# evanwang1990/FMwR

Hardware: AMD Instinct MI355X
Metric: training examples/sec, 10Mx1M sparse FM SGD (higher is better)
Workload: dtype f32

## Files before the change

### fmwr_amd/_lib.py

```python
import ctypes as C
import os

_PKG = os.path.dirname(os.path.abspath(__file__))
LIB_PATH = os.environ.get("FMX_LIB_PATH") or os.path.join(_PKG, "libfmx.so")

OK, ERR_INVALID, ERR_HIP, ERR_NOGPU, ERR_STATE = 0, 1, 2, 3, 4
TASK_CLASSIFICATION, TASK_REGRESSION, TASK_RANKING = 10, 20, 30
SOLVER_MCMC, SOLVER_ALS, SOLVER_SGD, SOLVER_FTRL, SOLVER_TDAP = 100, 200, 300, 500, 600
MODE_SEQUENTIAL, MODE_MINIBATCH = 0, 1
LINK_NONE, LINK_LOGISTIC, LINK_CLAMP, LINK_PROBIT = 0, 1, 2, 3
DIV_REL_SCORE, DIV_REL_MINMAX = 0, 1
SIM_COSINE, SIM_DOT = 0, 1
REDUCE_MEAN, REDUCE_SUM = 0, 1
COLUMNS_UNIFORM, COLUMNS_ZIPF = 1, 2
EVAL_LL, EVAL_AUC, EVAL_ACC, EVAL_RMSE, EVAL_MSE, EVAL_MAE = 0, 111, 222, 333, 444, 555
EVAL_PAIR_ACC, EVAL_BPR = 666, 777
KERNEL_ROWS_FORWARD, KERNEL_COLS_UPDATE, KERNEL_SCALAR, KERNEL_SEQ, KERNEL_ALS_SWEEP = 0, 1, 2, 3, 4

SYMBOLS = [
    "fmx_last_error", "fmx_device_count", "fmx_config_default", "fmx_engine_create", "fmx_engine_destroy", "fmx_set_params",
    "fmx_get_params", "fmx_engine_save", "fmx_engine_load", "fmx_matrix_from_rlist", "fmx_matrix_from_dgc", "fmx_matrix_from_csr", "fmx_matrix_synthetic", "fmx_matrix_synthetic_fields", "fmx_matrix_synthetic_iid", "fmx_matrix_synthetic_ragged", "fmx_matrix_synthetic_values", "fmx_train_stream", "fmx_matrix_set_labels", "fmx_matrix_set_fields", "fmx_matrix_destroy",
    "fmx_matrix_info", "fmx_matrix_export", "fmx_matrix_scales", "fmx_matrix_normalize", "fmx_predict", "fmx_train", "fmx_train_grid", "fmx_train_order", "fmx_num_batches",
    "fmx_step", "fmx_grad", "fmx_grad_buffer", "fmx_grad_elem_bytes", "fmx_grad_layout", "fmx_grad_begin", "fmx_grad_chunk", "fmx_apply_chunk", "fmx_apply", "fmx_sync", "fmx_stream", "fmx_predict_device",
    "fmx_als_plan_info", "fmx_als_tiled_info", "fmx_als_order_info", "fmx_als_carry_q", "fmx_als_vsweep", "fmx_mcmc_vsweep", "fmx_als_train", "fmx_mcmc_train", "fmx_mcmc_train_from", "fmx_mcmc_v_hyper", "fmx_evaluate", "fmx_train_tracked", "fmx_trace_size", "fmx_trace_get", "fmx_trace_params",
    "fmx_profile_enable", "fmx_profile_get", "fmx_profile_reset", "fmx_rows_tune_info", "fmx_matrix_rows_form", "fmx_measure_gather", "fmx_measure_gather_occ", "fmx_measure_gather_matrix", "fmx_rccl_selftest",
    "fmx_get_rows", "fmx_set_rows", "fmx_init_normal", "fmx_compact_info", "fmx_compact_count", "fmx_compact_reserve", "fmx_grad_compact", "fmx_compact_records", "fmx_apply_compact",
    "fmx_vsweep_device", "fmx_group_info", "fmx_source_open", "fmx_source_next", "fmx_source_close",
    "fmx_apply_compact_parts", "fmx_layout_info", "fmx_owner_configure", "fmx_owner_info", "fmx_rows_pack", "fmx_rows_unpack",
    "fmx_topk", "fmx_topk_device", "fmx_contrib", "fmx_contrib_device", "fmx_contrib_summary",
    "fmx_matrix_pairs", "fmx_matrix_pairs_hard",
    "fmx_heldout_rank", "fmx_heldout_rank_device", "fmx_heldout_metrics",
    "fmx_rank_lists", "fmx_rank_lists_device", "fmx_topk_lists", "fmx_topk_lists_device", "fmx_project", "fmx_project_device",
    "fmx_fold_in", "fmx_fold_in_pairs",
    "fmx_diversify", "fmx_diversify_device",
    "fmx_neighbors", "fmx_neighbors_device",
    "fmx_interactions", "fmx_interactions_device", "fmx_interactions_summary",
    "fmx_metrics", "fmx_metrics_device",
    "fmx_predict_calibrated", "fmx_predict_calibrated_device", "fmx_reliability", "fmx_reliability_device",
    "fmx_calibrate_platt", "fmx_calibrate_platt_device", "fmx_calibrate_isotonic", "fmx_calibrate_isotonic_device",
    "fmx_matrix_take", "fmx_matrix_take_device", "fmx_split_assign", "fmx_split_assign_device", "fmx_matrix_select", "fmx_matrix_select_device",
    "fmx_free_device", "fmx_matrix_split_entries", "fmx_row_permutation", "fmx_row_permutation_device",
]
SPLIT_ROWS, SPLIT_WITHIN_GROUPS, SPLIT_GROUPS = 0, 1, 2
SPLIT_ORDER_HASH, SPLIT_ORDER_TAIL = 0, 1
SPLIT_NO_PART = 0xFFFFFFFF
MET_VALUES, MET_COUNTS = 6, 4
MET_AUC, MET_LOGLOSS, MET_ACCURACY, MET_BRIER, MET_MEAN_PRED, MET_MEAN_LABEL = 0, 1, 2, 3, 4, 5
MET_MSE, MET_RMSE, MET_MAE, MET_MEAN_ERR = 0, 1, 2, 3
MET_ROWS, MET_POSITIVES, MET_PAIRS2, MET_CORRECT = 0, 1, 2, 3
CAL_NONE, CAL_PLATT, CAL_STEPS = 0, 1, 2
BINS_WIDTH, BINS_MASS = 0, 1
CAL_VALUES = 4
CAL_ECE, CAL_MCE, CAL_BRIER, CAL_LOGLOSS = 0, 1, 2, 3


TEST_HOOKS = ["fmx_debug_fail_next_plan_build", "fmx_debug_fail_next_comm_init", "fmx_debug_lose_next_seq_multiplier", "fmx_debug_stall_next_persistent_sweep",
              "fmx_debug_contrib_summary_chunk", "fmx_debug_foldin_slab", "fmx_debug_heldout_limits", "fmx_debug_pairs_hard_chunk", "fmx_debug_lists_limits", "fmx_debug_diversify_limits", "fmx_debug_neighbors_limits", "fmx_debug_interactions_limits", "fmx_debug_metrics_limits", "fmx_debug_take_limits", "fmx_debug_calibrate_limits", "fmx_debug_cols_launches",
              "fmx_debug_long_launches", "fmx_debug_rows_launches", "fmx_debug_rows_merged_launches",
              "fmx_debug_rows_sched_launches", "fmx_debug_rows_sched_id_limit", "fmx_debug_rows_sched_export"]


class Config(C.Structure):
    _fields_ = [
        ("struct_size", C.c_uint32), ("task", C.c_int32), ("solver", C.c_int32), ("num_factor", C.c_int32),
        ("keep_w0", C.c_int32), ("keep_w1", C.c_int32),
        ("l2_w0", C.c_double), ("l1_w1", C.c_double), ("l2_w1", C.c_double), ("l1_v", C.c_double), ("l2_v", C.c_double),
        ("learn_rate", C.c_double),
        ("alpha_w", C.c_double), ("alpha_v", C.c_double), ("beta_w", C.c_double), ("beta_v", C.c_double),
        ("random_step", C.c_int32), ("mode", C.c_int32), ("batch_rows", C.c_int64),
        ("min_target", C.c_double), ("max_target", C.c_double),
        ("device", C.c_int32), ("batch_reduce", C.c_int32), ("gamma", C.c_double), ("tile_rows", C.c_int64),
        ("state_fp64", C.c_int32), ("exchange_chunks", C.c_int32), ("n_gpus", C.c_int32), ("als_max_levels", C.c_int32), ("seq_reassociate", C.c_int32), ("gpus_share_device", C.c_int32),
    ]


class FieldsSpec(C.Structure):
    _fields_ = [("struct_size", C.c_uint32), ("n_dense", C.c_int32), ("n_fields", C.c_int32), ("reserved", C.c_int32),
                ("field_vocab", C.c_void_p), ("skew", C.c_double), ("seed", C.c_uint64)]


class TrackConfig(C.Structure):
    _fields_ = [("struct_size", C.c_uint32), ("metric", C.c_int32), ("step_size", C.c_int64), ("convergence", C.c_double),
                ("keep_params", C.c_int32), ("reserved", C.c_int32)]


class SplitSpec(C.Structure):
    _fields_ = [("struct_size", C.c_uint32), ("scope", C.c_int32), ("order", C.c_int32), ("n_folds", C.c_int32), ("hold_count", C.c_int64),
                ("hold_fraction", C.c_double), ("min_keep", C.c_int64), ("seed", C.c_uint64), ("salt", C.c_uint64)]


class Calibrator(C.Structure):
    _fields_ = [("struct_size", C.c_uint32), ("kind", C.c_int32), ("n_groups", C.c_int64), ("max_steps", C.c_int32), ("link", C.c_int32),
                ("platt", C.c_void_p), ("n_steps", C.c_void_p), ("thr", C.c_void_p), ("val", C.c_void_p)]


class FmxError(RuntimeError):
    def __init__(self, status, message):
        super().__init__(message)
        self.status = status


_lib = None


def lib():
    global _lib
    if _lib is None:
        if not os.path.exists(LIB_PATH):
            raise ImportError(f"{LIB_PATH} is missing: build the HIP library first (python -m fmwr_amd.build). "
                              "fmwr_amd has no CPU fallback.")
        L = C.CDLL(LIB_PATH)
        L.fmx_last_error.restype = C.c_char_p
        for name in SYMBOLS + TEST_HOOKS:
            if name != "fmx_last_error":
                getattr(L, name).restype = C.c_int
        L.fmx_matrix_pairs_hard.argtypes = [C.c_void_p, C.c_void_p, C.c_void_p, C.c_void_p, C.c_int32, C.c_int32, C.c_uint64, C.c_int64,
                                            C.POINTER(C.c_void_p)]
        L.fmx_fold_in.argtypes = [C.c_void_p, C.c_void_p, C.c_void_p, C.c_int64, C.c_double, C.c_double, C.c_int32, C.c_int32, C.c_void_p, C.c_void_p,
                                  C.c_void_p, C.c_void_p]
        L.fmx_fold_in_pairs.argtypes = L.fmx_fold_in.argtypes
        L.fmx_diversify.argtypes = [C.c_void_p, C.c_void_p, C.c_int64, C.c_int32, C.c_void_p, C.c_void_p, C.c_int32, C.c_double, C.c_int32, C.c_void_p,
                                    C.c_void_p, C.c_void_p]
        L.fmx_diversify_device.argtypes = L.fmx_diversify.argtypes
        L.fmx_neighbors.argtypes = [C.c_void_p, C.c_void_p, C.c_void_p, C.c_int32, C.c_int32, C.c_int32, C.c_void_p, C.c_void_p]
        L.fmx_neighbors_device.argtypes = [C.c_void_p, C.c_void_p, C.c_int64, C.c_int64, C.c_void_p, C.c_int32, C.c_int32, C.c_int32, C.c_void_p, C.c_void_p]
        L.fmx_debug_neighbors_limits.argtypes = [C.c_int64, C.c_int64]
        L.fmx_interactions.argtypes = [C.c_void_p, C.c_void_p, C.c_int32, C.c_void_p, C.c_void_p, C.c_void_p]
        L.fmx_interactions_device.argtypes = [C.c_void_p, C.c_void_p, C.c_int64, C.c_int64, C.c_int32, C.c_void_p, C.c_void_p, C.c_void_p]
        L.fmx_interactions_summary.argtypes = [C.c_void_p, C.c_void_p, C.c_void_p, C.c_int32, C.c_void_p, C.c_void_p, C.c_void_p]
        L.fmx_debug_interactions_limits.argtypes = [C.c_int32, C.c_int32, C.c_int64]
        L.fmx_metrics.argtypes = [C.c_void_p, C.c_void_p, C.c_void_p, C.c_int64, C.c_int, C.c_void_p, C.c_void_p]
        L.fmx_metrics_device.argtypes = [C.c_void_p, C.c_void_p, C.c_int64, C.c_int64, C.c_void_p, C.c_int64, C.c_int, C.c_void_p, C.c_void_p]
        L.fmx_debug_metrics_limits.argtypes = [C.c_int32, C.c_int32, C.c_int64]
        L.fmx_predict_calibrated.argtypes = [C.c_void_p, C.c_void_p, C.c_void_p, C.c_int64, C.POINTER(Calibrator), C.c_int, C.c_void_p]
        L.fmx_predict_calibrated_device.argtypes = [C.c_void_p, C.c_void_p, C.c_int64, C.c_int64, C.c_void_p, C.c_int64, C.POINTER(Calibrator), C.c_int, C.c_void_p]
        L.fmx_reliability.argtypes = [C.c_void_p, C.c_void_p, C.c_void_p, C.c_int64, C.c_int32, C.c_int32, C.POINTER(Calibrator), C.c_int] + [C.c_void_p] * 6
        L.fmx_reliability_device.argtypes = [C.c_void_p, C.c_void_p, C.c_int64, C.c_int64, C.c_void_p, C.c_int64, C.c_int32, C.c_int32, C.POINTER(Calibrator),
                                             C.c_int] + [C.c_void_p] * 6
        L.fmx_calibrate_platt.argtypes = [C.c_void_p, C.c_void_p, C.c_void_p, C.c_int64, C.c_double, C.c_int32, C.c_void_p, C.c_void_p, C.c_void_p]
        L.fmx_calibrate_platt_device.argtypes = [C.c_void_p, C.c_void_p, C.c_int64, C.c_int64, C.c_void_p, C.c_int64, C.c_double, C.c_int32, C.c_void_p, C.c_void_p,
                                                 C.c_void_p]
        L.fmx_calibrate_isotonic.argtypes = [C.c_void_p, C.c_void_p, C.c_void_p, C.c_int64, C.c_int32, C.c_void_p, C.c_void_p, C.c_void_p]
        L.fmx_calibrate_isotonic_device.argtypes = [C.c_void_p, C.c_void_p, C.c_int64, C.c_int64, C.c_void_p, C.c_int64, C.c_int32, C.c_void_p, C.c_void_p, C.c_void_p]
        L.fmx_debug_calibrate_limits.argtypes = [C.c_int64]
        L.fmx_matrix_take.argtypes = [C.c_void_p, C.c_void_p, C.c_int64, C.POINTER(C.c_void_p)]
        L.fmx_matrix_take_device.argtypes = L.fmx_matrix_take.argtypes
        L.fmx_split_assign.argtypes = [C.c_int, C.c_int64, C.c_void_p, C.c_int64, C.POINTER(SplitSpec), C.c_void_p]
        L.fmx_split_assign_device.argtypes = L.fmx_split_assign.argtypes
        L.fmx_matrix_select.argtypes = [C.c_void_p, C.c_void_p, C.c_uint32, C.c_int32, C.POINTER(C.c_void_p), C.c_void_p]
        L.fmx_matrix_select_device.argtypes = [C.c_void_p, C.c_void_p, C.c_uint32, C.c_int32, C.POINTER(C.c_void_p), C.POINTER(C.c_void_p)]
        L.fmx_free_device.argtypes = [C.c_void_p]
        L.fmx_matrix_split_entries.argtypes = [C.c_void_p, C.c_int32, C.c_int64, C.c_double, C.c_int64, C.c_uint64, C.c_uint64, C.POINTER(C.c_void_p),
                                               C.POINTER(C.c_void_p)]
        L.fmx_row_permutation.argtypes = [C.c_int, C.c_int64, C.c_uint64, C.c_uint64, C.c_void_p]
        L.fmx_row_permutation_device.argtypes = L.fmx_row_permutation.argtypes
        L.fmx_debug_take_limits.argtypes = [C.c_int32, C.c_int32, C.c_int64]
        _lib = L
    return _lib


def check(status):
    if status != OK:
        raise FmxError(status, lib().fmx_last_error().decode("utf-8", "replace"))


def default_config():
    cfg = Config()
    check(lib().fmx_config_default(C.byref(cfg)))
    return cfg
```

### fmwr_amd/csrc/fm_batch_kernels.hip

```cpp
#include <atomic>
#include <mutex>
#include <utility>
#include <vector>

#include "fmx_internal.h"
#include "fm_probit.h"
#include "fmx_test_hooks.h"

#ifndef FMX_U
#define FMX_U 4
#endif
#ifndef FMX_SPARSE_WAVES
#define FMX_SPARSE_WAVES 4
#endif
#ifndef FMX_DENSE_WAVES
#define FMX_DENSE_WAVES 4
#endif
#ifndef FMX_U_LARGE
#define FMX_U_LARGE 4
#endif
#ifndef FMX_U_SMALL
#define FMX_U_SMALL 8
#endif

// ... 331 lines not shown
  constexpr int PER = MERGE_STAGE / WG_THREADS;
  constexpr uint32_t DONE = 0xFFFFFFFFu;
  __shared__ uint32_t stage[MERGE_STAGE];
  __shared__ double red[TRAIN ? MERGE_RPW : 1];

  const int tid = threadIdx.x;
  const int gid = tid / LPR;
  const int lig = tid % LPR;
  const int64_t R0 = (int64_t)blockIdx.x * MERGE_RPW;
  const int64_t R1 = (R0 + MERGE_RPW < a.nrows) ? R0 + MERGE_RPW : a.nrows;
  const int64_t lo = a.row_ptr[a.r0 + R0];
  const int64_t hi = a.row_ptr[a.r0 + R1];
  const int cnt = (hi - lo < MERGE_STAGE) ? (int)(hi - lo) : MERGE_STAGE;
  uint32_t pe[MERGE_SLOTS];
#pragma unroll
  for (int s = 0; s < MERGE_SLOTS; ++s) {
    const int64_t row = R0 + s * NG + gid;
    const int64_t ra = row < a.nrows ? row : a.nrows, rb = row + 1 < a.nrows ? row + 1 : a.nrows;
    const int64_t ta = a.row_ptr[a.r0 + ra] - lo, tb = a.row_ptr[a.r0 + rb] - lo;
    pe[s] = (uint32_t)(ta < cnt ? ta : cnt) | ((uint32_t)(tb < cnt ? tb : cnt) << 16);
  }
  {
    uint32_t id[PER];
#pragma unroll
    for (int u = 0; u < PER; ++u) {
      const int i = tid + u * WG_THREADS;
      id[u] = i < cnt ? a.col[lo + i] : 0u;
    }
#pragma unroll
    for (int u = 0; u < PER; ++u) {
      const int i = tid + u * WG_THREADS;
      if (i < cnt) stage[i] = id[u];
    }
  }
  __syncthreads();

  const T* __restrict__ Vt = reinterpret_cast<const T*>(a.V) + lig * VEC;
  const T* __restrict__ wt = a.w ? reinterpret_cast<const T*>(a.w) : reinterpret_cast<const T*>(a.V);
  const bool k1 = h.k1 != 0;
  const int last = cnt > 0 ? cnt - 1 : 0;
  static_assert(MERGE_STAGE < (1 << 16), "positions are kept in 16 bits");
  uint32_t hd[MERGE_SLOTS];
  int left = 0;
#pragma unroll
  for (int s = 0; s < MERGE_SLOTS; ++s) {
    const int p0 = (int)(pe[s] & 0xFFFFu), p1 = (int)(pe[s] >> 16);
    const uint32_t v = stage[p0 < last ? p0 : last];
    hd[s] = p0 < p1 ? v : DONE;
    left += p1 - p0;
  }
  double sm[MERGE_SLOTS][VEC], qm[MERGE_SLOTS][VEC], lin[MERGE_SLOTS];
#pragma unroll
  for (int s = 0; s < MERGE_SLOTS; ++s) {
#pragma unroll
    for (int i = 0; i < VEC; ++i) { sm[s][i] = 0.0; qm[s][i] = 0.0; }
    lin[s] = h.k0 ? a.scal[SC_W0] : 0.0;
  }

  uint32_t safe = 0u;
  for (; left > 0; left -= U) {
    uint32_t eid[U];
    int esl[U];
#pragma unroll
    for (int u = 0; u < U; ++u) {
      uint32_t best = hd[0];
      int sel = 0;
#pragma unroll
      for (int s = 1; s < MERGE_SLOTS; ++s)
        if (hd[s] < best) { best = hd[s]; sel = s; }
      const bool live = best != DONE;
      eid[u] = live ? best : safe;
      esl[u] = live ? sel : MERGE_SLOTS;
      safe = eid[u];
      uint32_t nxt = 0u;
#pragma unroll
      for (int s = 0; s < MERGE_SLOTS; ++s)
        if (esl[u] == s) { pe[s] += 1u; nxt = pe[s]; }
      const int np = (int)(nxt & 0xFFFFu), ne = (int)(nxt >> 16);
      const uint32_t nx = stage[np < last ? np : last];
      const uint32_t nh = np < ne ? nx : DONE;
#pragma unroll
      for (int s = 0; s < MERGE_SLOTS; ++s)
        if (esl[u] == s) hd[s] = nh;
    }
    float4 vv[U];
    T wv[U];
#pragma unroll
    for (int u = 0; u < U; ++u) {
      vv[u] = gather_row(Vt + ((size_t)eid[u] << RowStride<T, LPR>::v(a.vsh)));
      wv[u] = wt[(size_t)eid[u] << RowStride<T, LPR>::w(a.wsh)];
    }
#pragma unroll
    for (int u = 0; u < U; ++u) {
      const double x = 1.0;
      const double wx = (double)wv[u] * x;
      double tmp[VEC], tsq[VEC];
      slice_get(vv[u], tmp);
#pragma unroll
      for (int i = 0; i < VEC; ++i) { tmp[i] = tmp[i] * x; tsq[i] = tmp[i] * tmp[i]; }
#pragma unroll
      for (int s = 0; s < MERGE_SLOTS; ++s) {
        if (esl[u] == s) {
          if (k1) lin[s] += wx;
#pragma unroll
          for (int i = 0; i < VEC; ++i) {
            sm[s][i] += tmp[i];
            if constexpr (U == 1) qm[s][i] += tsq[i]; else qm[s][i] += tmp[i] * tmp[i];
          }
        }
      }
    }
  }

  int eg = tid / LPR;
  asm volatile("" : "+v"(eg));
#pragma unroll
  for (int s = 0; s < MERGE_SLOTS; ++s) {
    const int64_t row = R0 + s * NG + eg;
    const bool have = row < a.nrows;
    double pair = 0.0;
#pragma unroll
    for (int i = 0; i < VEC; ++i) pair += 0.5 * (sm[s][i] * sm[s][i] - qm[s][i]);
#pragma unroll
    for (int off = LPR / 2; off > 0; off >>= 1) pair += __shfl_xor(pair, off);
    const double y_hat = lin[s] + pair;
    if constexpr (TRAIN) {
      double mult = 0.0;
      if (have) {
        mult = grad_mult(h, y_hat, a.y[a.r0 + row]);
        float4 srow = slice_make(sm[s], T());
        srow = embed_store<LPR>(srow, lig, (float)mult, a.embed);
        *reinterpret_cast<float4*>(reinterpret_cast<T*>(a.S) + (size_t)row * KP + lig * VEC) = srow;
        if (lig == 0) reinterpret_cast<T*>(a.amul)[row] = (T)mult;
      }
      if (lig == 0) red[s * NG + eg] = mult;
    } else {
      if (have && lig == 0 && a.yhat) a.yhat[row] = link_apply(h, y_hat, a.link, a.pn_y);
    }
  }
  if constexpr (TRAIN) {
    __syncthreads();
    if (tid % 64 == 0) {
      const int s = tid / 64;
      if (R0 + (int64_t)s * NG < a.nrows) {
        double g0 = 0.0, q0 = 0.0;
        for (int i = 0; i < NG; ++i) { const double m = red[s * NG + i]; g0 += m; q0 += m * m; }
        a.partials[2 * ((size_t)blockIdx.x * MERGE_SLOTS + s)] = g0;
        a.partials[2 * ((size_t)blockIdx.x * MERGE_SLOTS + s) + 1] = q0;
      }
    }
  }
}

template <bool UNIFORM, bool PIPE, bool DEAL = false>
__global__ __launch_bounds__(WG_THREADS, 4) void fm_rows_sched_k(RowsArgs a, Hyper h) {
  using T = float;
  constexpr int LPR = 4, VEC = 4, KP = LPR * VEC;
  constexpr int NG = WG_THREADS / LPR;
  constexpr int PER = MERGE_STAGE / WG_THREADS;
  static_assert(MERGE_STAGE == SCHED_STAGE_STEPS * NG && MERGE_SLOTS == 4, "the stage holds SCHED_STAGE_STEPS steps of one word per lane group");
  static_assert(UNIFORM || !PIPE, "only the unrolled walk has a round to request together");
  static_assert(!(UNIFORM && DEAL), "a DEAL schedule is walked as a MERGE one");
  __shared__ uint32_t stage[MERGE_STAGE];
  __shared__ double red[MERGE_RPW];
  __shared__ uint32_t places[DEAL ? NG : 1];

  const int tid = threadIdx.x;
  const int gid = tid / LPR;
  const int lig = tid % LPR;
  const int64_t R0 = (int64_t)blockIdx.x * MERGE_RPW;
  const uint32_t w_hi = a.sched_dir[blockIdx.x + 1];
  uint32_t w_lo = a.sched_dir[blockIdx.x];
  if constexpr (DEAL) {
    const bool hdr = w_hi - w_lo >= (uint32_t)NG;
    if (tid < NG) places[tid] = hdr ? a.sched[(size_t)w_lo + tid] : 0u;
    w_lo += hdr ? (uint32_t)NG : 0u;
  }
  const int cnt = (w_hi - w_lo < (uint32_t)MERGE_STAGE) ? (int)(w_hi - w_lo) : MERGE_STAGE;
  const int steps = UNIFORM ? (cnt / NG) & ~3 : cnt / NG;
  {
    uint32_t id[PER];
#pragma unroll
    for (int u = 0; u < PER; ++u) {
      const int i = tid + u * WG_THREADS;
      id[u] = i < cnt ? a.sched[(size_t)w_lo + i] : SCHED_BUBBLE;
    }
#pragma unroll
    for (int u = 0; u < PER; ++u) {
      const int i = tid + u * WG_THREADS;
      if (i < cnt) stage[i] = id[u];
    }
  }
  __syncthreads();

  const __amdgpu_buffer_rsrc_t v_rsrc = table_rsrc(a.V, a.sched_vbytes);
  const __amdgpu_buffer_rsrc_t w_rsrc = table_rsrc(a.w ? a.w : a.V, a.w ? a.sched_wbytes : a.sched_vbytes);
  const bool k1 = h.k1 != 0;
  const int vsh = RowStride<T, LPR>::v(a.vsh) + 2, wsh = RowStride<T, LPR>::w(a.wsh) + 2;
  const uint32_t lane_off = (uint32_t)(lig * VEC * sizeof(T));
  double sm[MERGE_SLOTS][VEC], qm[MERGE_SLOTS][VEC], lin[MERGE_SLOTS];
#pragma unroll
  for (int s = 0; s < MERGE_SLOTS; ++s) {
#pragma unroll
    for (int i = 0; i < VEC; ++i) { sm[s][i] = 0.0; qm[s][i] = 0.0; }
    lin[s] = h.k0 ? a.scal[SC_W0] : 0.0;
  }
  const uint32_t* __restrict__ mine = stage + gid;

  if constexpr (UNIFORM) {
    for (int t = 0; t < steps; t += MERGE_SLOTS) {
      uint32_t wd[MERGE_SLOTS];
#pragma unroll
      for (int j = 0; j < MERGE_SLOTS; ++j) wd[j] = mine[(t + j) * NG];
      float4 vv[MERGE_SLOTS];
      T wv[MERGE_SLOTS];
      if constexpr (PIPE) {
#pragma unroll
        for (int j = 0; j < MERGE_SLOTS; ++j) {
          const bool live = wd[j] != SCHED_BUBBLE;
          const uint32_t c = wd[j] & SCHED_MAX_P;
          vv[j] = buf_row(v_rsrc, live ? (c << vsh) + lane_off : BUF_SKIP, T());
          wv[j] = buf_elem(w_rsrc, live ? c << wsh : BUF_SKIP, T());
        }
      }
#pragma unroll
      for (int j = 0; j < MERGE_SLOTS; ++j) {
        if constexpr (!PIPE) {
          const bool live = wd[j] != SCHED_BUBBLE;
          const uint32_t c = wd[j] & SCHED_MAX_P;
          vv[j] = buf_row(v_rsrc, live ? (c << vsh) + lane_off : BUF_SKIP, T());
          wv[j] = buf_elem(w_rsrc, live ? c << wsh : BUF_SKIP, T());
          asm volatile("s_waitcnt vmcnt(0)" ::: "memory");
        }
        const double x = 1.0;
        const double wx = (double)wv[j] * x;
        double tmp[VEC], tsq[VEC];
        slice_get(vv[j], tmp);
#pragma unroll
        for (int i = 0; i < VEC; ++i) { tmp[i] = tmp[i] * x; tsq[i] = tmp[i] * tmp[i]; }
        if (k1) lin[j] += wx;
#pragma unroll
        for (int i = 0; i < VEC; ++i) { sm[j][i] += tmp[i]; qm[j][i] += tsq[i]; }
      }
    }
  } else {
    for (int t = 0; t < steps; ++t) {
      const uint32_t wd = mine[t * NG];
      const bool live = wd != SCHED_BUBBLE;
      const uint32_t c = wd & SCHED_MAX_P;
      const int esl = live ? (int)(wd >> 30) : MERGE_SLOTS;
      const float4 vv = buf_row(v_rsrc, live ? (c << vsh) + lane_off : BUF_SKIP, T());
      const T wv = buf_elem(w_rsrc, live ? c << wsh : BUF_SKIP, T());
      const double x = 1.0;
      const double wx = (double)wv * x;
      double tmp[VEC], tsq[VEC];
      slice_get(vv, tmp);
#pragma unroll
      for (int i = 0; i < VEC; ++i) { tmp[i] = tmp[i] * x; tsq[i] = tmp[i] * tmp[i]; }
#pragma unroll
      for (int s = 0; s < MERGE_SLOTS; ++s) {
        if (esl == s) {
          if (k1) lin[s] += wx;
#pragma unroll
          for (int i = 0; i < VEC; ++i) { sm[s][i] += tmp[i]; qm[s][i] += tsq[i]; }
        }
      }
    }
  }

  int eg = tid / LPR;
  asm volatile("" : "+v"(eg));
  uint32_t place = 0;
  if constexpr (DEAL) place = places[eg];
#pragma unroll
  for (int s = 0; s < MERGE_SLOTS; ++s) {
    const int at = DEAL ? (int)((place >> (8 * s)) & 255u) : s * NG + eg;
    const int64_t row = R0 + at;
    const bool have = row < a.nrows;
    double pair = 0.0;
#pragma unroll
    for (int i = 0; i < VEC; ++i) pair += 0.5 * (sm[s][i] * sm[s][i] - qm[s][i]);
#pragma unroll
    for (int off = LPR / 2; off > 0; off >>= 1) pair += __shfl_xor(pair, off);
    const double y_hat = lin[s] + pair;
    double mult = 0.0;
    if (have) {
      mult = grad_mult(h, y_hat, a.y[a.r0 + row]);
      float4 srow = slice_make(sm[s], T());
      srow = embed_store<LPR>(srow, lig, (float)mult, a.embed);
      *reinterpret_cast<float4*>(reinterpret_cast<T*>(a.S) + (size_t)row * KP + lig * VEC) = srow;
      if (lig == 0) reinterpret_cast<T*>(a.amul)[row] = (T)mult;
    }
    if (lig == 0) red[at] = mult;
  }
  __syncthreads();
  if (tid % 64 == 0) {
    const int s = tid / 64;
    if (R0 + (int64_t)s * NG < a.nrows) {
      double g0 = 0.0, q0 = 0.0;
      for (int i = 0; i < NG; ++i) { const double m = red[s * NG + i]; g0 += m; q0 += m * m; }
      a.partials[2 * ((size_t)blockIdx.x * MERGE_SLOTS + s)] = g0;
      a.partials[2 * ((size_t)blockIdx.x * MERGE_SLOTS + s) + 1] = q0;
    }
  }
}

template <typename T, int LPR, bool TRAIN>
__global__ __launch_bounds__(WG_THREADS) void fm_rows_forward_dyn_k(RowsArgs a, Hyper h) {
  using vec_t = typename Slice<T>::vec;
  constexpr int VEC = Slice<T>::N;
  constexpr int KP = LPR * VEC;
  constexpr int GROUPS = WG_THREADS / LPR;
  constexpr int RPW = 4 * GROUPS;
  constexpr int RU = FMX_U_LARGE;
  constexpr int PER = (RU + LPR - 1) / LPR;
  __shared__ int next_row;
  __shared__ double red[TRAIN ? RPW : 1];
  const int tid = threadIdx.x;
  const int grp = tid / LPR, lig = tid % LPR;
  const int lane0 = (tid & 63) - lig;
  const int64_t R0 = (int64_t)blockIdx.x * RPW;
  const int rows_here = (int)((R0 + RPW < a.nrows ? R0 + RPW : a.nrows) - R0);
  if (tid == 0) next_row = GROUPS;
  if (TRAIN) for (int i = tid; i < RPW; i += WG_THREADS) red[i] = 0.0;
  __syncthreads();
  const T* __restrict__ Vt = reinterpret_cast<const T*>(a.V) + lig * VEC;
  const T* __restrict__ wt = a.w ? reinterpret_cast<const T*>(a.w) : reinterpret_cast<const T*>(a.V);
  const bool k1 = h.k1 != 0;
  const int64_t last = a.row_ptr[a.r0 + R0 + rows_here] - 1;
  int r = grp;
  while (r < rows_here) {
    const int64_t ta = a.row_ptr[a.r0 + R0 + r], tb = a.row_ptr[a.r0 + R0 + r + 1];
    double s[VEC], q[VEC];
#pragma unroll
    for (int i = 0; i < VEC; ++i) { s[i] = 0.0; q[i] = 0.0; }
    double lin = h.k0 ? a.scal[SC_W0] : 0.0;
    auto load_round = [&](int64_t t, uint32_t* id, uint32_t* xb) {
#pragma unroll
      for (int v = 0; v < PER; ++v) {
        const int64_t at = t + lig + v * LPR;
        const int64_t ac = at <= last ? (at >= 0 ? at : 0) : (last >= 0 ? last : 0);
        id[v] = a.col[ac];
        xb[v] = a.unit ? 0x3f800000u : __float_as_uint(a.val[ac]);
      }
    };
    uint32_t cid[PER], cxb[PER], nid[PER], nxb[PER];
    load_round(ta, cid, cxb);
    for (int64_t t = ta; t < tb; t += RU) {
      load_round(t + RU, nid, nxb);
      uint2 en[RU];
#pragma unroll
      for (int u = 0; u < RU; ++u) {
        en[u].x = (uint32_t)__shfl((int)cid[u / LPR], lane0 + (u % LPR));
        en[u].y = (uint32_t)__shfl((int)cxb[u / LPR], lane0 + (u % LPR));
      }
#pragma unroll
      for (int u = 1; u < RU; ++u)
        if (t + u >= tb) en[u] = make_uint2(en[0].x, 0u);
      vec_t vv[RU];
      T wv[RU];
#pragma unroll
      for (int u = 0; u < RU; ++u) {
        vv[u] = gather_row(Vt + ((size_t)en[u].x << RowStride<T, LPR>::v(a.vsh)));
        wv[u] = wt[(size_t)en[u].x << RowStride<T, LPR>::w(a.wsh)];
        if (a.serial) asm volatile("s_waitcnt vmcnt(0)" ::: "memory");
      }
#pragma unroll
      for (int u = 0; u < RU; ++u) {
        const double x = (double)__uint_as_float(en[u].y);
        if (k1) lin += (double)wv[u] * x;
        double vf[VEC];
        slice_get(vv[u], vf);
#pragma unroll
        for (int i = 0; i < VEC; ++i) {
          const double tmp = vf[i] * x;
          s[i] += tmp;
          q[i] += tmp * tmp;
        }
      }
#pragma unroll
      for (int v = 0; v < PER; ++v) { cid[v] = nid[v]; cxb[v] = nxb[v]; }
    }
    double pair = 0.0;
#pragma unroll
    for (int i = 0; i < VEC; ++i) pair += 0.5 * (s[i] * s[i] - q[i]);
#pragma unroll
    for (int off = LPR / 2; off > 0; off >>= 1) pair += __shfl_xor(pair, off);
    const double y_hat = lin + pair;
    const int64_t row = R0 + r;
    if constexpr (TRAIN) {
      const double mult = grad_mult(h, y_hat, a.y[a.r0 + row]);
      vec_t srow = slice_make(s, T());
      if constexpr (sizeof(T) == 4) srow = embed_store<LPR>(srow, lig, (float)mult, a.embed);
      *reinterpret_cast<vec_t*>(reinterpret_cast<T*>(a.S) + (size_t)row * KP + lig * VEC) = srow;
      if (lig == 0) { reinterpret_cast<T*>(a.amul)[row] = (T)mult; red[r] = mult; }
    } else {
      if (lig == 0 && a.yhat) a.yhat[row] = link_apply(h, y_hat, a.link, a.pn_y);
      if constexpr (sizeof(T) == 8) {
        if (a.qout) {
          if (a.qout_t > 0) { a.qout[(size_t)(lig * VEC) * a.qout_t + row] = s[0]; a.qout[(size_t)(lig * VEC + 1) * a.qout_t + row] = s[1]; }
          else *reinterpret_cast<double2*>(a.qout + (size_t)row * KP + lig * VEC) = make_double2(s[0], s[1]);
        }
      } else if (a.qout) {
        double2* q2 = reinterpret_cast<double2*>(a.qout + (size_t)row * KP + lig * VEC);
        q2[0] = make_double2(s[0], s[1]);
        q2[1] = make_double2(s[2], s[3]);
      }
    }
    int nr = 0;
    if (lig == 0) nr = atomicAdd(&next_row, 1);
    r = __shfl(nr, lane0);
  }
  if constexpr (TRAIN) {
    __syncthreads();
    if (tid < RPW / GROUPS && tid * GROUPS < rows_here) {
      double g0 = 0.0, q0 = 0.0;
      for (int i = tid * GROUPS; i < (tid + 1) * GROUPS; ++i) { g0 += red[i]; q0 += red[i] * red[i]; }
      const size_t at = (size_t)blockIdx.x * (RPW / GROUPS) + tid;
// ... 254 lines not shown
    if (a.wg_threads == 64 && 64 / lpr >= 2) { count_rows_launch(counted, ROWS_NARROW1); return launch_rows_t<T, TRAIN, 64, 1, true>(e, a, kp); }
    count_rows_launch(counted, wide_form);
    return launch_rows_t<T, TRAIN, WG_THREADS, 1, true>(e, a, kp);
  }
  if (a.sort_rows && a.wg_threads != 64) { count_rows_launch(counted, ROWS_PULL); return launch_rows_dyn<T, TRAIN>(e, a, kp); }
  if (a.flat == 1 && a.wg_threads != 64) { count_rows_launch(counted, ROWS_FLAT); return launch_rows_flat<T, TRAIN>(e, a, kp); }
  if (a.wg_threads == 64) {
    count_rows_launch(counted, a.split == 4 ? ROWS_NARROW4 : ROWS_NARROW1);
    return a.split == 4 ? launch_rows_t<T, TRAIN, 64, 4>(e, a, kp) : launch_rows_t<T, TRAIN, 64, 1>(e, a, kp);
  }
  count_rows_launch(counted, wide_form);
  return launch_rows_t<T, TRAIN, WG_THREADS, 1>(e, a, kp);
}

static std::atomic<int64_t> g_rows_merged[2];
void debug_rows_merged_launches(int64_t out[2]) {
  for (int i = 0; i < 2; ++i) out[i] = g_rows_merged[i].load();
}
#ifndef FMX_ROWS_MERGE_U_DEFAULT
#define FMX_ROWS_MERGE_U_DEFAULT 1
#endif
static int rows_merge_mode() { static const int v = [] { const char* s = getenv("FMX_ROWS_MERGE"); return s ? atoi(s) : 1; }(); return v; }
static int rows_merge_u() {
  static const int v = [] { const char* s = getenv("FMX_ROWS_MERGE_U"); const int u = s ? atoi(s) : FMX_ROWS_MERGE_U_DEFAULT; return (u == 1 || u == 2) ? u : FMX_ROWS_MERGE_U_DEFAULT; }();
  return v;
}

template <bool TRAIN, int U>
static int64_t rows_merged_fill(const fmx_engine* e) {
  constexpr int MAX_DEV = 64;
  static std::atomic<int64_t> fill_dev[MAX_DEV];
  std::atomic<int64_t>& fill = fill_dev[(e->cfg.device >= 0 && e->cfg.device < MAX_DEV) ? e->cfg.device : 0];
  int64_t v = fill.load();
  if (v == 0) {
    hipDeviceProp_t pr{};
    const int cus = (hipGetDeviceProperties(&pr, e->cfg.device) == hipSuccess && pr.multiProcessorCount > 0) ? pr.multiProcessorCount : 256;
    int per = 0;
    if (hipOccupancyMaxActiveBlocksPerMultiprocessor(&per, fm_rows_merged_k<float, 4, TRAIN, U>, WG_THREADS, 0) != hipSuccess || per <= 0) per = 4;
    v = (int64_t)per * cus * MERGE_RPW;
    fill.store(v);
  }
  return v;
}

__global__ __launch_bounds__(WG_THREADS) void rows_block_max_k(const int64_t* __restrict__ row_ptr, int64_t r0, int64_t nrows, int64_t* __restrict__ out) {
  __shared__ int64_t part[WG_THREADS];
  const int64_t blocks = (nrows + MERGE_RPW - 1) / MERGE_RPW;
  int64_t m = 0;
  for (int64_t b = threadIdx.x; b < blocks; b += WG_THREADS) {
    const int64_t r1 = (b + 1) * MERGE_RPW < nrows ? (b + 1) * MERGE_RPW : nrows;
    const int64_t c = row_ptr[r0 + r1] - row_ptr[r0 + b * MERGE_RPW];
    m = c > m ? c : m;
  }
  part[threadIdx.x] = m;
  __syncthreads();
  if (threadIdx.x == 0) {
    for (int i = 1; i < WG_THREADS; ++i) m = part[i] > m ? part[i] : m;
    out[0] = m;
  }
}

static int rows_merged_fits(fmx_engine* e, const RowsArgs& a, bool* fits) {
  if ((int64_t)a.max_row_len * MERGE_RPW <= MERGE_STAGE) { *fits = true; return FMX_OK; }
  struct Key { uint64_t uid; int64_t r0, nrows; };
  static std::mutex mu;
  static std::vector<std::pair<Key, bool>> known;
  {
    std::lock_guard<std::mutex> g(mu);
    for (const auto& k : known)
      if (k.first.uid == a.mat_uid && k.first.r0 == a.r0 && k.first.nrows == a.nrows) { *fits = k.second; return FMX_OK; }
  }
  int64_t* d = nullptr;
  int64_t most = 0;
  FMX_HIP(hipMalloc(&d, sizeof(int64_t)));
  hipLaunchKernelGGL(rows_block_max_k, dim3(1), dim3(WG_THREADS), 0, e->stream, a.row_ptr, a.r0, a.nrows, d);
  hipError_t err = hipGetLastError();
  if (err == hipSuccess) err = hipMemcpyAsync(&most, d, sizeof(int64_t), hipMemcpyDeviceToHost, e->stream);
  if (err == hipSuccess) err = hipStreamSynchronize(e->stream);
  (void)hipFree(d);
  FMX_HIP(err);
  *fits = most <= MERGE_STAGE;
  std::lock_guard<std::mutex> g(mu);
  if (known.size() >= 4096) known.clear();
  known.push_back({Key{a.mat_uid, a.r0, a.nrows}, *fits});
  return FMX_OK;
}

template <bool TRAIN, int U>
static int launch_rows_merged_u(fmx_engine* e, const RowsArgs& a, int mode, bool* ran) {
  const size_t v_bytes = ((size_t)e->p << a.vsh) * sizeof(float);
  if (mode != 2 && (a.nrows < rows_merged_fill<TRAIN, U>(e) || a.col_skew != 1 || v_bytes <= MERGE_MIN_TABLE)) return FMX_OK;
  bool fits = false;
  FMX_TRY(rows_merged_fits(e, a, &fits));
  if (!fits) { g_rows_merged[1]++; return FMX_OK; }
  const int64_t grid = (a.nrows + MERGE_RPW - 1) / MERGE_RPW;
  FMX_CHECK(grid < (1LL << 31), FMX_ERR_INVALID, "rows_forward: grid too large (%lld)", (long long)grid);
  hipLaunchKernelGGL((fm_rows_merged_k<float, 4, TRAIN, U>), dim3((unsigned)grid), dim3(WG_THREADS), 0, e->stream, a, e->hyper);
  FMX_HIP(hipGetLastError());
  g_rows_merged[0]++;
  *ran = true;
  return FMX_OK;
}

template <bool TRAIN>
static int launch_rows_merged(fmx_engine* e, const RowsArgs& a, bool fp64_tables, bool* ran) {
  *ran = false;
  const int mode = rows_merge_mode();
  if (mode == 0 || fp64_tables || e->kp32 != 16 || !a.unit || a.qout || a.no_w || a.wg_threads == 64 || a.sort_rows || a.flat == 1) return FMX_OK;
  if (TRAIN && e->cfg.task == FMX_TASK_RANKING) return FMX_OK;
  if (a.nrows <= 0 || a.max_row_len <= 0 || a.mat_uid == 0) return FMX_OK;
  switch (rows_merge_u()) {
    case 2: return launch_rows_merged_u<TRAIN, 2>(e, a, mode, ran);
    default: return launch_rows_merged_u<TRAIN, 1>(e, a, mode, ran);
  }
}

#ifndef FMX_ROWS_SCHED_DEFAULT
#define FMX_ROWS_SCHED_DEFAULT 1
#endif
#ifndef FMX_ROWS_SCHED_POLICY_DEFAULT
#define FMX_ROWS_SCHED_POLICY_DEFAULT SCHED_DEAL
#endif
#ifndef FMX_ROWS_SCHED_RHO_DEFAULT
#define FMX_ROWS_SCHED_RHO_DEFAULT 1024
#endif
static std::atomic<int64_t> g_rows_sched[3];
void debug_rows_sched_launches(int64_t out[3]) {
  for (int i = 0; i < 3; ++i) out[i] = g_rows_sched[i].load();
}
void rows_sched_count_build() { g_rows_sched[2]++; }
static int rows_sched_mode() {
  static const int v = [] { const char* s = getenv("FMX_ROWS_SCHED"); return s ? atoi(s) : (getenv("FMX_ROWS_MERGE") ? 0 : FMX_ROWS_SCHED_DEFAULT); }();
  return v;
}
static int rows_sched_policy() {
  static const int v = [] {
    const char* s = getenv("FMX_ROWS_SCHED_POLICY");
    if (!s) return (int)FMX_ROWS_SCHED_POLICY_DEFAULT;
    return s[0] == 'm' ? (int)SCHED_MERGE : s[0] == 'f' ? (int)SCHED_FRONT : s[0] == 'r' ? (int)SCHED_ROUND : s[0] == 'd' ? (int)SCHED_DEAL : (int)FMX_ROWS_SCHED_POLICY_DEFAULT;
  }();
  return v;
}
static int rows_sched_rho_q() {
  static const int v = [] {
    const char* s = getenv("FMX_ROWS_SCHED_RHO");
    if (!s) return (int)FMX_ROWS_SCHED_RHO_DEFAULT;
    const double r = atof(s);
    return r <= 0.0 ? 0 : r >= 1.0 ? 1024 : (int)(r * 1024.0 + 0.5);
  }();
  return v;
}
static int rows_sched_u() { static const int v = [] { const char* s = getenv("FMX_ROWS_SCHED_U"); return (s && atoi(s) == 4) ? 4 : 1; }(); return v; }

bool rows_sched_wanted(fmx_engine* e, const RowsArgs& a, int* policy, int* rho_q) {
  const int mode = rows_sched_mode();
  if (mode == 0 || mb_wide(e) || e->kp32 != 16 || !a.unit || a.qout || a.no_w || a.wg_threads == 64 || a.sort_rows || a.flat == 1) return false;
  if (e->cfg.task == FMX_TASK_RANKING || a.nrows <= 0 || a.max_row_len <= 0 || a.mat_uid == 0 || !a.w) return false;
  const uint64_t v_bytes = (uint64_t)e->p * (uint64_t)a.vs * sizeof(float), w_bytes = (uint64_t)e->p * (uint64_t)a.ws * sizeof(float);
  if (v_bytes >= BUF_SKIP || w_bytes >= BUF_SKIP || e->p > SCHED_MAX_P) return false;
  if (mode != 2 && (a.nrows < rows_merged_fill<true, 1>(e) || a.col_skew != 1 || v_bytes <= MERGE_MIN_TABLE)) return false;
  *policy = rows_sched_policy();
  *rho_q = (*policy == SCHED_MERGE || *policy == SCHED_DEAL) ? 0 : rows_sched_rho_q();
  return true;
}

static int launch_rows_sched(fmx_engine* e, const RowsArgs& a_in, bool* ran) {
  *ran = false;
  if (a_in.sched_state == 0) return FMX_OK;
  int policy = 0, rho_q = 0;
  if (!rows_sched_wanted(e, a_in, &policy, &rho_q)) return FMX_OK;
  if (a_in.sched_state != 1 || !a_in.sched || !a_in.sched_dir) { g_rows_sched[1]++; return FMX_OK; }
  RowsArgs a = a_in;
  a.sched_vbytes = (uint32_t)((uint64_t)e->p * (uint64_t)a.vs * sizeof(float));
  a.sched_wbytes = (uint32_t)((((uint64_t)e->p - 1) * (uint64_t)a.ws + 1) * sizeof(float));
  const int64_t grid = (a.nrows + MERGE_RPW - 1) / MERGE_RPW;
  FMX_CHECK(grid < (1LL << 31), FMX_ERR_INVALID, "rows_forward: grid too large (%lld)", (long long)grid);
  if (a.sched_deal) hipLaunchKernelGGL((fm_rows_sched_k<false, false, true>), dim3((unsigned)grid), dim3(WG_THREADS), 0, e->stream, a, e->hyper);
  else if (!a.sched_uniform) hipLaunchKernelGGL((fm_rows_sched_k<false, false>), dim3((unsigned)grid), dim3(WG_THREADS), 0, e->stream, a, e->hyper);
  else if (rows_sched_u() == 4) hipLaunchKernelGGL((fm_rows_sched_k<true, true>), dim3((unsigned)grid), dim3(WG_THREADS), 0, e->stream, a, e->hyper);
  else hipLaunchKernelGGL((fm_rows_sched_k<true, false>), dim3((unsigned)grid), dim3(WG_THREADS), 0, e->stream, a, e->hyper);
  FMX_HIP(hipGetLastError());
  g_rows_sched[0]++;
  *ran = true;
  return FMX_OK;
}

int launch_rows_forward(fmx_engine* e, const RowsArgs& a_in, bool train, bool fp64_tables) {
  RowsArgs a = a_in;
  FMX_CHECK(a.vs >= (fp64_tables ? e->kp64 : e->kp32) && a.ws >= 1 && (a.vs & (a.vs - 1)) == 0 && (a.ws & (a.ws - 1)) == 0, FMX_ERR_STATE,
            "rows_forward: table strides not set (%d, %d)", a.vs, a.ws);
  {
    const int kp = fp64_tables ? e->kp64 : e->kp32;
    FMX_CHECK((!fp64_tables && kp <= WIR_MAX_KP) || (a.vs == kp && a.ws == 1), FMX_ERR_STATE, "rows_forward: strides (%d, %d) on a table of compiled strides (%d, 1)",
              a.vs, a.ws, kp);
  }
  a.vsh = __builtin_ctz((unsigned)a.vs); a.wsh = __builtin_ctz((unsigned)a.ws);
  static const bool embed_ok = [] { const char* v = getenv("FMX_EMBED_MULT"); return !(v && v[0] == '0'); }();
  static const int force = [] { const char* v = getenv("FMX_ROWS_SERIAL"); return v ? atoi(v) : -1; }();
  RowsTune& tu = e->rows_tune;
  auto pick = [&](const RowsArgs& r, int* serial, int* trial) -> int {
    *trial = -1;
    *serial = 1;
    if (force >= 0) { *serial = force; return FMX_OK; }
    const bool timed = r.wg_threads != 64 && r.nrows >= RowsTune::MIN_ROWS;
    const int64_t key = r.unit ? 1 : 0;
    if (timed && key != tu.key) {
      if (tu.events && tu.launches > 0 && tu.decided < 0) FMX_HIP(hipStreamSynchronize(e->stream));
      tu.key = key; tu.decided = -1; tu.launches = 0;
    }
    if (tu.decided >= 0) { *serial = tu.decided; return FMX_OK; }
    if (!timed) return FMX_OK;
    if (!tu.events) {
      bool ok = true;
      for (auto& ev : tu.ev) ok = ok && hipEventCreate(&ev) == hipSuccess;
      FMX_CHECK(ok, FMX_ERR_HIP, "rows_forward: could not create the tuning events");
      tu.events = true;
    }
    if (tu.launches >= RowsTune::TRIALS) {
      tu.decided = 1;
      return FMX_OK;
    }
    *trial = tu.launches++;
    *serial = *trial % 2 == 0 ? 1 : 0;
    FMX_HIP(hipEventRecord(tu.ev[2 * *trial], e->stream));
    return FMX_OK;
  };
  auto done = [&](int trial) -> int {
    if (trial < 0) return FMX_OK;
    FMX_HIP(hipEventRecord(tu.ev[2 * trial + 1], e->stream));
    if (tu.launches >= RowsTune::TRIALS && tu.decided < 0) {
      FMX_HIP(hipEventSynchronize(tu.ev[2 * trial + 1]));
      double ms[2] = {0.0, 0.0};
      for (int i = 2; i < RowsTune::TRIALS; ++i) {
        float t = 0.f;
        FMX_HIP(hipEventElapsedTime(&t, tu.ev[2 * i], tu.ev[2 * i + 1]));
        ms[i % 2 == 0 ? 1 : 0] += t;
      }
      tu.ms[0] = ms[0]; tu.ms[1] = ms[1];
      tu.decided = ms[1] <= ms[0] ? 1 : 0;
    }
    return FMX_OK;
  };
  a.embed = (train && embed_ok) ? embed_mode(e->k, fp64_tables ? e->kp64 : e->kp32, !fp64_tables) : EMBED_NONE;
  prof_begin(e, FMX_KERNEL_ROWS_FORWARD);
  int st = FMX_OK;
  bool merged = false;
  if (train) {
    st = launch_rows_sched(e, a, &merged);
    if (st == FMX_OK && !merged) st = launch_rows_merged<true>(e, a, fp64_tables, &merged);
    if (st == FMX_OK && !merged) {
      int trial;
      FMX_TRY(pick(a, &a.serial, &trial));
      st = fp64_tables ? launch_rows_w<double, true>(e, a, e->kp64) : launch_rows_w<float, true>(e, a, e->kp32);
      { const int st2 = done(trial); if (st == FMX_OK) st = st2; }
    }
  } else {
    const int64_t SLAB = 1 << 18;
    const int kp = fp64_tables ? e->kp64 : e->kp32;
    for (int64_t off = 0; off < a.nrows && st == FMX_OK; off += SLAB) {
      RowsArgs s = a;
      s.r0 = a.r0 + off;
      s.nrows = a.nrows - off < SLAB ? a.nrows - off : SLAB;
      if (a.yhat) s.yhat = a.yhat + off;
      if (a.qout) s.qout = a.qout_t > 0 ? a.qout + off : a.qout + (size_t)off * kp;
      s.wg_threads = a.fixed_schedule ? WG_THREADS : rows_wg_threads(a.nrows, kp / (fp64_tables ? 2 : 4));
      s.split = a.fixed_schedule ? 1 : rows_split(a.nrows, kp / (fp64_tables ? 2 : 4));
      st = launch_rows_merged<false>(e, s, fp64_tables, &merged);
      if (st != FMX_OK || merged) continue;
      int trial;
      FMX_TRY(pick(s, &s.serial, &trial));
      st = fp64_tables ? launch_rows_w<double, false>(e, s, kp) : launch_rows_w<float, false>(e, s, kp);
      { const int st2 = done(trial); if (st == FMX_OK) st = st2; }
    }
  }
  prof_end(e);
  return st;
}

template <typename ST>
__device__ __forceinline__ void tail_put_rows(ST* gtail, double rows) {
  const double hi = floor(rows / 4096.0);
  gtail[2] = (ST)hi;
  gtail[3] = (ST)(rows - hi * 4096.0);
}
template <typename ST>
__device__ __forceinline__ double tail_get_rows(const ST* gtail) { return (double)gtail[2] * 4096.0 + (double)gtail[3]; }

template <typename ST>
__device__ __forceinline__ void scalar_update(const double* __restrict__ partials, int64_t n_partials, const double* sin,
                                              double* sout, ST* gtail, const Hyper& h, double rows, int mode,
                                              double* sg, double* sq) {
  const int phase = (mode == SCALAR_PUBLISH) ? 1 : (mode == SCALAR_FROM_TAIL) ? 2 : 0;
  double g0 = 0.0, q0 = 0.0;
  if (phase != 2) {
    for (int64_t i = threadIdx.x; i < n_partials; i += WG_THREADS) { g0 += partials[2 * i]; q0 += partials[2 * i + 1]; }
  }
  sg[threadIdx.x] = g0; sq[threadIdx.x] = q0;
  __syncthreads();
  for (int off = WG_THREADS / 2; off > 0; off >>= 1) {
    if ((int)threadIdx.x < off) { sg[threadIdx.x] += sg[threadIdx.x + off]; sq[threadIdx.x] += sq[threadIdx.x + off]; }
    __syncthreads();
  }
  if (threadIdx.x != 0) return;
  g0 = sg[0]; q0 = sq[0];
  if (phase == 1) { gtail[0] = (ST)g0; gtail[1] = (ST)q0; tail_put_rows(gtail, rows); return; }
  if (phase == 2) { g0 = gtail[0]; q0 = gtail[1]; if (rows <= 0.0) rows = tail_get_rows(gtail); }
  for (int i = 0; i < SC_COUNT; ++i) sout[i] = sin[i];
  if (h.task == FMX_TASK_RANKING) {
    sout[SC_G0] = 0.0; sout[SC_Q0] = 0.0;
    if (h.kind == UPD_SGD_L1) {
      const double steps = (h.mean && rows > 0.0) ? 1.0 : rows;
      sout[SC_UW] = sin[SC_UW] + steps * (h.lr * h.regw);
      sout[SC_UV] = sin[SC_UV] + steps * (h.lr * h.regv);
    }
    return;
  }
  sout[SC_G0] = g0; sout[SC_Q0] = q0;
  if (h.mean && rows > 0.0) {
    g0 /= rows;
    q0 = g0 * g0;
    rows = 1.0;
  }
  const double w0 = sin[SC_W0];
  if (h.kind == UPD_TDAP) {
    double u = sin[SC_N0], nu = sin[SC_T_NU], dl = sin[SC_T_DELTA], hh = sin[SC_T_H], z0 = sin[SC_Z0];
    if (h.k0) {
      const double u_new = u + q0;
      nu += g0;
      const double sigma = (sqrt(u_new) - sqrt(u)) / h.alpha_w;
      const double age = rows == 1.0 ? h.egamma : exp(-h.gamma * rows);
      dl = age * (dl + sigma);
      hh = age * (hh + sigma * w0);
      u = u_new;
      z0 = nu - hh;
// ... 1148 lines not shown
```

### fmwr_amd/csrc/fm_group.hip

```cpp
#include <dlfcn.h>

#include <atomic>

#include <hip/hip_runtime.h>

#include "fmx_internal.h"

namespace fmx {

typedef void* rcclComm_t;
struct Rccl {
  void* lib = nullptr;
  int (*CommInitAll)(rcclComm_t*, int, const int*) = nullptr;
  int (*CommDestroy)(rcclComm_t) = nullptr;
  int (*AllReduce)(const void*, void*, size_t, int, int, rcclComm_t, hipStream_t) = nullptr;
  int (*AllGather)(const void*, void*, size_t, int, rcclComm_t, hipStream_t) = nullptr;
  int (*GroupStart)() = nullptr;
  int (*GroupEnd)() = nullptr;
  const char* (*GetErrorString)(int) = nullptr;
};
constexpr int RCCL_SUM = 0, RCCL_FLOAT32 = 7, RCCL_FLOAT64 = 8;

static Rccl* rccl() {
  static Rccl r;
  static bool tried = false;
  if (tried) return r.lib ? &r : nullptr;
  tried = true;
  for (const char* name : {"librccl.so.1", "librccl.so", "/opt/rocm/lib/librccl.so.1"}) {
    r.lib = dlopen(name, RTLD_NOW | RTLD_GLOBAL);
    if (r.lib) break;
  }
  if (!r.lib) return nullptr;
  r.CommInitAll = (decltype(r.CommInitAll))dlsym(r.lib, "ncclCommInitAll");
  r.CommDestroy = (decltype(r.CommDestroy))dlsym(r.lib, "ncclCommDestroy");
  r.AllReduce = (decltype(r.AllReduce))dlsym(r.lib, "ncclAllReduce");
  r.AllGather = (decltype(r.AllGather))dlsym(r.lib, "ncclAllGather");
  r.GroupStart = (decltype(r.GroupStart))dlsym(r.lib, "ncclGroupStart");
  r.GroupEnd = (decltype(r.GroupEnd))dlsym(r.lib, "ncclGroupEnd");
  r.GetErrorString = (decltype(r.GetErrorString))dlsym(r.lib, "ncclGetErrorString");
  if (!r.CommInitAll || !r.CommDestroy || !r.AllReduce || !r.AllGather || !r.GroupStart || !r.GroupEnd) { dlclose(r.lib); r.lib = nullptr; return nullptr; }
  return &r;
}

#define FMX_RCCL(call)                                                                                               \
  do {                                                                                                               \
    const int _r = (call);                                                                                           \
    if (_r != 0) {                                                                                                   \
      Rccl* _l = rccl();                                                                                             \
      fmx::set_error("%s failed: %s", #call, _l && _l->GetErrorString ? _l->GetErrorString(_r) : "rccl error");       \
      return FMX_ERR_HIP;                                                                                            \
    }                                                                                                                \
  } while (0)

constexpr int GROUP_MAX = 16;
struct BufList { void* b[GROUP_MAX]; int n; };

template <typename ST>
__global__ void sum_buffers_k(BufList bl, int64_t count) {
  const int64_t i = (int64_t)blockIdx.x * blockDim.x + threadIdx.x;
  if (i >= count) return;
  ST acc = reinterpret_cast<const ST*>(bl.b[0])[i];
  for (int r = 1; r < bl.n; ++r) acc = acc + reinterpret_cast<const ST*>(bl.b[r])[i];
  for (int r = 0; r < bl.n; ++r) reinterpret_cast<ST*>(bl.b[r])[i] = acc;
}

__global__ void rebase_rows_k(const int64_t* __restrict__ src, int64_t r0, int64_t n, int64_t base, int64_t* __restrict__ dst) {
  const int64_t i = (int64_t)blockIdx.x * blockDim.x + threadIdx.x;
  if (i <= n) dst[i] = src[r0 + i] - base;
}

struct Group {
  int n = 0;
  std::vector<fmx_engine*> rep;
  std::vector<int> dev;
  bool shared = false;
  std::vector<rcclComm_t> comm;
  hipStream_t xs = nullptr;
  std::vector<hipEvent_t> ready;
  hipEvent_t summed = nullptr;
  uint64_t src_uid = 0;
  uint64_t src_values = 0;
  std::vector<fmx_matrix*> shard;
  std::vector<void*> gath;
  int64_t gath_records = 0;
  bool busy = false;
  struct OwnerBuf {
    void *req = nullptr, *rows_out = nullptr, *rows_in = nullptr, *parts = nullptr;
    int64_t req_cap = 0, out_cap = 0, in_cap = 0, parts_cap = 0;
  };
  std::vector<OwnerBuf> ox;
  std::vector<hipEvent_t> ev_ids, ev_packed, ev_grad, ev_done;
  int peer_pairs = 0, peer_direct = 0;
  bool owners_on = false;
  bool owner_dirty = false;
};

bool group_outside(const fmx_engine* e) { return e->group != nullptr && !e->group->busy; }

static void free_shards(Group* g) {
  for (size_t r = 0; r < g->shard.size(); ++r)
    if (g->shard[r]) { (void)hipSetDevice(g->dev[r]); fmx_matrix_destroy(g->shard[r]); }
  g->shard.clear();
  g->src_uid = 0;
}

void group_destroy(fmx_engine* e) {
  Group* g = e->group;
  if (!g) return;
  free_shards(g);
  for (size_t r = 0; r < g->gath.size(); ++r) if (g->gath[r]) { (void)hipSetDevice(g->dev[r]); (void)hipFree(g->gath[r]); }
  for (size_t r = 0; r < g->ox.size(); ++r) {
    (void)hipSetDevice(g->dev[r]);
    (void)hipFree(g->ox[r].req); (void)hipFree(g->ox[r].rows_out); (void)hipFree(g->ox[r].rows_in); (void)hipFree(g->ox[r].parts);
  }
  for (auto* v : {&g->ev_ids, &g->ev_packed, &g->ev_grad, &g->ev_done})
    for (size_t r = 0; r < v->size(); ++r) if ((*v)[r]) { (void)hipSetDevice(g->dev[r]); (void)hipEventDestroy((*v)[r]); }
  Rccl* l = rccl();
  for (rcclComm_t c : g->comm) if (c && l) (void)l->CommDestroy(c);
  (void)hipSetDevice(e->cfg.device);
  for (hipEvent_t ev : g->ready) if (ev) (void)hipEventDestroy(ev);
  if (g->summed) (void)hipEventDestroy(g->summed);
  if (g->xs) (void)hipStreamDestroy(g->xs);
  for (int r = 1; r < g->n; ++r) fmx_engine_destroy(g->rep[(size_t)r]);
  delete g;
  e->group = nullptr;
}

static std::atomic<int> g_fail_next_comm_init{0};
void debug_fail_next_comm_init() { g_fail_next_comm_init.store(1); }

int group_create(fmx_engine* e) {
  const int n = e->cfg.n_gpus;
  FMX_CHECK(n >= 2 && n <= GROUP_MAX, FMX_ERR_INVALID, "n_gpus must be in 1..%d", GROUP_MAX);
  FMX_CHECK(e->cfg.mode == FMX_MODE_MINIBATCH, FMX_ERR_INVALID,
            "n_gpus > 1 needs FMX_MODE_MINIBATCH: the reference's per-example algorithm does not shard (every example depends on the one before)");
  FMX_CHECK(e->cfg.solver == FMX_SOLVER_SGD || e->cfg.solver == FMX_SOLVER_FTRL || e->cfg.solver == FMX_SOLVER_TDAP, FMX_ERR_INVALID,
            "n_gpus > 1 trains SGD / FTRL / TDAP engines (the ALS / MCMC sweeps run as replicas only)");
  Group* g = new Group();
  e->group = g;
  g->n = n;
  g->shared = e->cfg.gpus_share_device != 0;
  g->rep.assign((size_t)n, nullptr);
  g->rep[0] = e;
  int count = 0;
  FMX_HIP(hipGetDeviceCount(&count));
  for (int r = 0; r < n; ++r) g->dev.push_back(g->shared ? e->cfg.device : e->cfg.device + r);
  FMX_CHECK(g->dev.back() < count, FMX_ERR_INVALID, "n_gpus = %d starting at device %d, but only %d devices are visible", n, e->cfg.device, count);
  for (int r = 1; r < n; ++r) {
    fmx_config c = e->cfg;
    c.n_gpus = 1;
    c.device = g->dev[(size_t)r];
    FMX_TRY(fmx_engine_create(&c, e->p, &g->rep[(size_t)r]));
  }
  g->ready.assign((size_t)n, nullptr);
  if (g_fail_next_comm_init.exchange(0) > 0) {
    set_error("ncclCommInitAll failed on device %d (forced: fmx_debug_fail_next_comm_init)", g->dev[(size_t)n - 1]);
    return FMX_ERR_HIP;
  }
  if (g->shared) {
    FMX_HIP(hipSetDevice(e->cfg.device));
    FMX_HIP(hipStreamCreateWithFlags(&g->xs, hipStreamNonBlocking));
    FMX_HIP(hipEventCreateWithFlags(&g->summed, hipEventDisableTiming));
    for (int r = 0; r < n; ++r) FMX_HIP(hipEventCreateWithFlags(&g->ready[(size_t)r], hipEventDisableTiming));
  } else {
    Rccl* l = rccl();
    FMX_CHECK(l != nullptr, FMX_ERR_STATE, "n_gpus > 1 on distinct devices needs librccl.so (not found by dlopen)");
    g->comm.assign((size_t)n, nullptr);
    FMX_RCCL(l->CommInitAll(g->comm.data(), n, g->dev.data()));
    for (int a = 0; a < n; ++a) {
      FMX_HIP(hipSetDevice(g->dev[(size_t)a]));
      for (int b = 0; b < n; ++b) {
        if (a == b) continue;
        ++g->peer_pairs;
        int can = 0;
        if (hipDeviceCanAccessPeer(&can, g->dev[(size_t)a], g->dev[(size_t)b]) != hipSuccess) { (void)hipGetLastError(); can = 0; }
        if (!can) continue;
        const hipError_t pe = hipDeviceEnablePeerAccess(g->dev[(size_t)b], 0);
        if (pe == hipSuccess || pe == hipErrorPeerAccessAlreadyEnabled) ++g->peer_direct;
        (void)hipGetLastError();
      }
    }
  }
  FMX_HIP(hipSetDevice(e->cfg.device));
  return FMX_OK;
}

int group_load(fmx_engine* e, const char* path) {
  Group* g = e->group;
  for (int r = 1; r < g->n; ++r) FMX_TRY(fmx_engine_load(g->rep[(size_t)r], path));
  g->owner_dirty = false;
  return use_device(e->cfg.device);
}

int group_set_params(fmx_engine* e, double w0, const double* w, const double* v) {
  (void)w; (void)v;
  Group* g = e->group;
  std::vector<std::pair<void*, size_t>> src;
  engine_tables(e, &src, true);
  FMX_HIP(hipSetDevice(e->cfg.device));
  FMX_HIP(hipStreamSynchronize(e->stream));
  for (int r = 1; r < g->n; ++r) {
    FMX_TRY(fmx_set_params(g->rep[(size_t)r], w0, nullptr, nullptr));
    std::vector<std::pair<void*, size_t>> dst;
    engine_tables(g->rep[(size_t)r], &dst, true);
    FMX_CHECK(dst.size() == src.size(), FMX_ERR_STATE, "replica %d has another table layout", r);
    for (size_t t = 0; t < src.size(); ++t) {
      FMX_CHECK(dst[t].second == src[t].second, FMX_ERR_STATE, "replica %d has another table layout", r);
      const size_t bytes = src[t].second * (size_t)e->p;
      if (g->dev[(size_t)r] == g->dev[0]) FMX_HIP(hipMemcpy(dst[t].first, src[t].first, bytes, hipMemcpyDeviceToDevice));
      else FMX_HIP(hipMemcpyPeer(dst[t].first, g->dev[(size_t)r], src[t].first, g->dev[0], bytes));
    }
  }
  FMX_HIP(hipDeviceSynchronize());
  g->owner_dirty = false;
  return use_device(e->cfg.device);
}

int group_init_normal(fmx_engine* e, uint64_t seed, double mean, double stdev) {
  Group* g = e->group;
  for (int r = 1; r < g->n; ++r) FMX_TRY(fmx_init_normal(g->rep[(size_t)r], seed, mean, stdev));
  return use_device(e->cfg.device);
}

int group_set_rows(fmx_engine* e, const uint32_t* ids, int64_t n, const double* w, const double* v) {
  Group* g = e->group;
  for (int r = 1; r < g->n; ++r) FMX_TRY(fmx_set_rows(g->rep[(size_t)r], ids, n, w, v));
  return use_device(e->cfg.device);
}

static int cut_shard(const fmx_matrix* src, int64_t r0, int64_t r1, int dev, fmx_matrix** out) {
  FMX_HIP(hipSetDevice(src->device));
  int64_t ends[2] = {0, 0};
  FMX_HIP(hipMemcpy(&ends[0], src->row_ptr + r0, sizeof(int64_t), hipMemcpyDeviceToHost));
  FMX_HIP(hipMemcpy(&ends[1], src->row_ptr + r1, sizeof(int64_t), hipMemcpyDeviceToHost));
  const int64_t base = ends[0], cnt = ends[1] - ends[0], n = r1 - r0;
  fmx_matrix* m = nullptr;
  FMX_TRY(alloc_matrix(dev, n, src->p, cnt, src->has_labels != 0, &m));
  auto body = [&]() -> int {
    FMX_HIP(hipSetDevice(dev));
    if (dev == src->device) {
      hipLaunchKernelGGL(rebase_rows_k, dim3((unsigned)((n + 1 + 255) / 256)), dim3(256), 0, nullptr, src->row_ptr, r0, n, base, m->row_ptr);
    } else {
      FMX_HIP(hipMemcpyPeer(m->row_ptr, dev, src->row_ptr + r0, src->device, ((size_t)n + 1) * sizeof(int64_t)));
      hipLaunchKernelGGL(rebase_rows_k, dim3((unsigned)((n + 1 + 255) / 256)), dim3(256), 0, nullptr, m->row_ptr, (int64_t)0, n, base, m->row_ptr);
    }
    if (cnt > 0) {
      FMX_HIP(hipMemcpyPeer(m->col, dev, src->col + base, src->device, (size_t)cnt * sizeof(uint32_t)));
      FMX_HIP(hipMemcpyPeer(m->val, dev, src->val + base, src->device, (size_t)cnt * sizeof(float)));
    }
    if (n > 0) FMX_HIP(hipMemcpyPeer(m->y, dev, src->y + r0, src->device, (size_t)n * sizeof(float)));
// ... 615 lines not shown
```

### fmwr_amd/csrc/fmx_api.hip

```cpp
#include <algorithm>
#include <cmath>
#include <cstdlib>
#include <cstring>
#include <ctime>
#include <atomic>
#include <memory>

#include "fmx_internal.h"
#include "fmx_test_hooks.h"
#include "fm_probit.h"

namespace fmx {

static thread_local std::string g_error;

void set_error(const char* fmt, ...) {
  char buf[1024];
  va_list ap;
  va_start(ap, fmt);
  vsnprintf(buf, sizeof(buf), fmt, ap);
  va_end(ap);
  g_error = buf;
}

void prof_begin(fmx_engine* e, int kernel) {
  e->prof_open = 0;
  if (!e->profile) return;
  if ((e->prof_seen[kernel]++ % e->profile) != 0) return;
  hipEvent_t a, b;
  if (hipEventCreate(&a) != hipSuccess || hipEventCreate(&b) != hipSuccess) return;
  (void)hipEventRecord(a, e->stream);
  e->prof_pending.push_back({kernel, {a, b}});
  e->prof_open = 1;
}

void prof_end(fmx_engine* e) {
  if (!e->prof_open || e->prof_pending.empty()) return;
  e->prof_open = 0;
  (void)hipEventRecord(e->prof_pending.back().second.second, e->stream);
}

static int prof_collect(fmx_engine* e) {
  if (e->prof_pending.empty()) return FMX_OK;
  FMX_HIP(hipStreamSynchronize(e->stream));
  for (auto& pr : e->prof_pending) {
    float ms = 0.f;
    if (hipEventElapsedTime(&ms, pr.second.first, pr.second.second) == hipSuccess) {
      e->prof_ms[pr.first] += ms;
      e->prof_n[pr.first] += 1;
    }
    (void)hipEventDestroy(pr.second.first);
    (void)hipEventDestroy(pr.second.second);
  }
  e->prof_pending.clear();
  return FMX_OK;
}

int use_device(int device) {
  int count = 0;
  hipError_t err = hipGetDeviceCount(&count);
  if (err != hipSuccess || count <= 0) {
    set_error("no HIP device available (%s); libfmx has no CPU fallback", err == hipSuccess ? "device count 0" : hipGetErrorString(err));
    return FMX_ERR_NOGPU;
  }
  FMX_CHECK(device >= 0 && device < count, FMX_ERR_INVALID, "device %d out of range (0..%d)", device, count - 1);
  FMX_HIP(hipSetDevice(device));
  return FMX_OK;
}

int seq_abort_check(fmx_engine* e) {
  if (!e->cfg.seq_reassociate && !getenv("FMX_SEQ_REASSOC")) return FMX_OK;
  double flag = 0.0;
  FMX_HIP(hipMemcpy(&flag, e->scal + SC_SEQ_ABORT, sizeof(double), hipMemcpyDeviceToHost));
  FMX_CHECK(flag == 0.0, FMX_ERR_HIP, "the reassociated sequential learner gave up waiting inside a launch (its workgroup's waves did not all run?): the parameters are not a valid state");
  return FMX_OK;
}

template <typename T>
static int dev_alloc_zero(T** ptr, size_t count) {
  const size_t bytes = (count ? count : 1) * sizeof(T);
  FMX_HIP(hipMalloc(ptr, bytes));
  FMX_HIP(hipMemset(*ptr, 0, bytes));
  return FMX_OK;
}

static int make_hyper(const fmx_config& c, Hyper* h) {
  h->task = c.task;
  h->k0 = c.keep_w0 != 0;
  h->k1 = c.keep_w1 != 0;
  h->lr = c.learn_rate;
  h->reg0 = c.l2_w0;
  h->l1w = c.l1_w1; h->l1v = c.l1_v; h->l2w = c.l2_w1; h->l2v = c.l2_v;
  h->alpha_w = c.alpha_w; h->alpha_v = c.alpha_v; h->beta_w = c.beta_w; h->beta_v = c.beta_v;
  h->min_t = c.min_target; h->max_t = c.max_target;
  h->mean = (c.batch_reduce == FMX_REDUCE_MEAN);
  h->egamma = std::exp(-c.gamma);
  h->gamma = c.gamma;
  if (c.solver == FMX_SOLVER_FTRL || c.solver == FMX_SOLVER_TDAP) {
    h->kind = c.solver == FMX_SOLVER_FTRL ? UPD_FTRL : UPD_TDAP;
    h->regw = 0; h->regv = 0;
  } else {
    bool l1 = false;
    if (c.l1_w1 > 0 || c.l1_v > 0) {
      l1 = true;
      h->regw = c.l1_w1; h->regv = c.l1_v;
    } else {
      h->regw = c.l2_w1; h->regv = c.l2_v;
    }
    if (c.task == FMX_TASK_REGRESSION) l1 = false;
    h->kind = l1 ? UPD_SGD_L1 : UPD_SGD_L2;
  }
  h->decay_w = 1.0 - h->lr * h->regw;
  h->decay_v = 1.0 - h->lr * h->regv;
  h->log_decay_w = h->decay_w > 0 ? std::log(h->decay_w) : 0.0;
  h->log_decay_v = h->decay_v > 0 ? std::log(h->decay_v) : 0.0;
  return FMX_OK;
}

static bool seq_mode(const fmx_engine* e) { return e->cfg.mode == FMX_MODE_SEQUENTIAL; }
static bool ranking(const fmx_engine* e) { return e->cfg.task == FMX_TASK_RANKING; }

static int check_pairs(const fmx_engine* e, const fmx_matrix* m, int64_t rows, const char* what) {
  if (!ranking(e)) return FMX_OK;
  FMX_CHECK(m->n % 2 == 0, FMX_ERR_INVALID, "a ranking engine trains on pair matrices (rows 2t, 2t + 1): this matrix has an odd row count (%lld)", (long long)m->n);
  FMX_CHECK(rows % 2 == 0, FMX_ERR_INVALID, "a ranking engine needs an even %s (got %lld): a step may not split a pair", what, (long long)rows);
  return FMX_OK;
}

static int reset_optimizer_state(fmx_engine* e) {
  const size_t p = e->p;
  double zeros[SC_COUNT] = {0};
  double w0 = 0;
  FMX_HIP(hipMemcpy(&w0, e->scal + SC_W0, sizeof(double), hipMemcpyDeviceToHost));
  zeros[SC_W0] = w0;
  FMX_HIP(hipMemcpy(e->scal, zeros, sizeof(zeros), hipMemcpyHostToDevice));
  if (e->sV) FMX_HIP(hipMemset(e->sV, 0, p * e->kp32 * sizeof(float)));
  if (e->sw) FMX_HIP(hipMemset(e->sw, 0, p * sizeof(float)));
  if (e->nV) FMX_HIP(hipMemset(e->nV, 0, p * e->kp32 * sizeof(float)));
  if (e->nw) FMX_HIP(hipMemset(e->nw, 0, p * sizeof(float)));
  for (float* t : {e->t1V, e->t2V, e->t3V}) if (t) FMX_HIP(hipMemset(t, 0, p * e->kp32 * sizeof(float)));
  for (float* t : {e->t1w, e->t2w, e->t3w}) if (t) FMX_HIP(hipMemset(t, 0, p * sizeof(float)));
  if (e->dsV) FMX_HIP(hipMemset(e->dsV, 0, p * e->kp64 * sizeof(double)));
  if (e->dsw) FMX_HIP(hipMemset(e->dsw, 0, p * sizeof(double)));
  if (e->dnV) FMX_HIP(hipMemset(e->dnV, 0, p * e->kp64 * sizeof(double)));
  if (e->dnw) FMX_HIP(hipMemset(e->dnw, 0, p * sizeof(double)));
  for (double* t : {e->dt1V, e->dt2V, e->dt3V}) if (t) FMX_HIP(hipMemset(t, 0, p * e->kp64 * sizeof(double)));
  for (double* t : {e->dt1w, e->dt2w, e->dt3w}) if (t) FMX_HIP(hipMemset(t, 0, p * sizeof(double)));
  return FMX_OK;
}

static int ensure_workspace(fmx_engine* e, int64_t s_rows, int64_t step_rows, int64_t tiles_per_step) {
  const int rpw = WG_THREADS / mb_lpr(e);
  const int64_t partials = (step_rows + rpw - 1) / rpw + (tiles_per_step > 0 ? tiles_per_step : 1) + 8 + 4096;
  if (s_rows <= e->ws_rows && partials <= e->ws_partials) return FMX_OK;
  FMX_HIP(hipStreamSynchronize(e->stream));
  (void)hipFree(e->S); (void)hipFree(e->amul); (void)hipFree(e->partials);
  e->S = nullptr; e->amul = nullptr; e->partials = nullptr; e->ws_rows = 0; e->ws_partials = 0;
  FMX_HIP(hipMalloc(&e->S, (size_t)s_rows * mb_kp(e) * mb_elem(e)));
  FMX_HIP(hipMalloc(&e->amul, (size_t)s_rows * mb_elem(e)));
  FMX_HIP(hipMalloc(&e->partials, (size_t)partials * 2 * sizeof(double)));
  e->ws_rows = s_rows;
  e->ws_partials = partials;
  return FMX_OK;
}

static int ensure_gbuf(fmx_engine* e) {
  if (e->gbuf) return FMX_OK;
  const bool has_q = exchange_has_q(e);
  const int64_t chunks = e->cfg.exchange_chunks > 1 ? e->cfg.exchange_chunks : 1;
  const int64_t per = ((int64_t)e->p + chunks - 1) / chunks;
  e->gb_feats = chunks > 1 ? (per + 63) / 64 * 64 : ((int64_t)e->p + 3) / 4 * 4;
  e->gb_blocks = ((int64_t)e->p + e->gb_feats - 1) / e->gb_feats;
  e->gb_block_elems = e->gb_feats * mb_kp(e) * (has_q ? 2 : 1) + e->gb_feats * (has_q ? 3 : 2);
  e->gbuf_floats = e->gb_blocks * e->gb_block_elems + 4;
  FMX_HIP(hipMalloc(&e->gbuf, (size_t)e->gbuf_floats * mb_elem(e)));
  FMX_HIP(hipMemset(e->gbuf, 0, (size_t)e->gbuf_floats * mb_elem(e)));
  FMX_HIP(hipDeviceSynchronize());
  return FMX_OK;
}

static uint32_t random_select(int n) {
  if (n == 1) return 1;
  return (uint32_t)((rand() / ((double)RAND_MAX + 1)) * n + 1);
}

struct VisitOrder {
  int64_t n;
  int step;
  uint64_t i = 0;
  bool in_pass = false;
  int idle = 0;
  VisitOrder(int64_t n_, int step_) : n(n_), step(step_) {}
  bool pending = false;
  bool next(int64_t count, std::vector<int64_t>* out) {
    out->clear();
    out->reserve((size_t)count);
    size_t pass_start = 0;
    while ((int64_t)out->size() < count) {
      if (!in_pass) { i = random_select(step); in_pass = true; pending = false; pass_start = out->size(); }
      else if (pending) { i += random_select(step); pending = false; }
      if (i < (uint64_t)n) {
        out->push_back((int64_t)i);
        pending = true;
        idle = 0;
      } else {
        in_pass = false;
        if (out->size() == pass_start && ++idle > 1000) return false;
      }
    }
    return true;
  }
};

void free_matrix(fmx_matrix* m) {
  if (!m) return;
  (void)hipFree(m->row_ptr); (void)hipFree(m->col); (void)hipFree(m->val); (void)hipFree(m->y);
  drop_plans(m);
  (void)hipFree(m->col_ptr); (void)hipFree(m->crow); (void)hipFree(m->cval); (void)hipFree(m->als_feats); (void)hipFree(m->als_heavy); (void)hipFree(m->als_level_ptr_dev); (void)hipFree(m->als_rank);
  (void)hipFree(m->als_vh); (void)hipFree(m->als_vh_seg0); (void)hipFree(m->als_vseg_feat); (void)hipFree(m->als_vseg_b); (void)hipFree(m->als_vseg_e); (void)hipFree(m->als_vh_work);
  als_tiled_free(m);
  delete m;
}

int alloc_matrix(int device, int64_t n, uint32_t p, int64_t nnz, bool labels, fmx_matrix** out) {
  FMX_CHECK(out != nullptr, FMX_ERR_INVALID, "out is NULL");
  *out = nullptr;
  FMX_CHECK(n >= 0 && nnz >= 0, FMX_ERR_INVALID, "negative size");
  FMX_TRY(use_device(device));
  std::unique_ptr<fmx_matrix, void (*)(fmx_matrix*)> m(new fmx_matrix(), free_matrix);
  static std::atomic<uint64_t> next_uid{1};
  m->uid = next_uid.fetch_add(1);
  m->device = device; m->n = n; m->p = p; m->nnz = nnz; m->has_labels = labels;
  FMX_HIP(hipMalloc(&m->row_ptr, ((size_t)n + 1) * sizeof(int64_t)));
  FMX_HIP(hipMalloc(&m->col, ((size_t)nnz + 1) * sizeof(uint32_t)));
  FMX_HIP(hipMalloc(&m->val, ((size_t)nnz + 1) * sizeof(float)));
  FMX_HIP(hipMalloc(&m->y, ((size_t)n + 1) * sizeof(float)));
  FMX_HIP(hipMemset(m->y, 0, ((size_t)n + 1) * sizeof(float)));
  *out = m.release();
  return FMX_OK;
}

int check_pair(const fmx_engine* e, const fmx_matrix* m) {
  FMX_CHECK(e && m, FMX_ERR_INVALID, "NULL handle");
  FMX_CHECK((uint64_t)m->p == e->p, FMX_ERR_INVALID, "number of input's features is not correct...");
  FMX_CHECK(m->device == e->cfg.device, FMX_ERR_INVALID, "matrix lives on device %d, engine on %d", m->device, e->cfg.device);
  return FMX_OK;
}

int forward_rows(fmx_engine* e, const fmx_matrix* m, int64_t r0, int64_t r1, double* d_out, int link) {
  FMX_CHECK(link >= FMX_LINK_NONE && link <= FMX_LINK_PROBIT, FMX_ERR_INVALID, "unknown link %d", link);
  if (link == FMX_LINK_PROBIT) FMX_TRY(ensure_probit(e));
  RowsArgs a{};
  a.row_ptr = m->row_ptr; a.col = m->col; a.val = m->val; a.y = nullptr;
  a.r0 = r0; a.nrows = r1 - r0;
  if (wide_state(e)) { a.V = e->dV; a.w = e->dw; a.vs = e->kp64; a.ws = 1; }
  else { a.V = e->V; a.w = mb_wbase(e); a.vs = e->vstride32; a.ws = mb_wstride(e); }
  a.scal = e->scal;
  a.yhat = d_out;
  a.link = link;
  a.pn_y = e->probit;
  a.unit = m->unit_values;
  a.sort_rows = rows_ragged(m);
  a.flat = rows_flat(m); a.nmat = m->n;
  a.mat_uid = m->uid; a.max_row_len = m->max_row_len;
  for (const auto& pl : m->plans) { const int s = rows_col_skew(m, pl); a.col_skew = s > a.col_skew ? s : a.col_skew; }
  FMX_TRY(launch_rows_forward(e, a, false, wide_state(e)));
  return FMX_OK;
}

int ensure_probit(fmx_engine* e) {
  if (e->probit) return FMX_OK;
  std::vector<double> t((size_t)PN_POINTS + 1 + DP_POINTS + 1);
  for (int i = 0; i < PN_POINTS; ++i) t[(size_t)i] = 0.5 * std::erfc(-pn_x(i) / std::sqrt(2.0));
  t[PN_POINTS] = t[PN_POINTS - 1];
  double* dp = t.data() + PN_POINTS + 1;
  for (int i = 0; i < DP_POINTS; ++i) {
    const double x = dp_x(i);
    const double r = std::exp(-0.5 * x * x) / std::sqrt(2.0 * 3.14159265358979323846) / (1.0 - 0.5 * std::erfc(-x / std::sqrt(2.0)));
    dp[i] = std::round(r * 1e12) / 1e12;
  }
  dp[DP_POINTS] = dp[DP_POINTS - 1];
  FMX_HIP(hipMalloc(&e->probit, t.size() * sizeof(double)));
  FMX_HIP(hipMemcpy(e->probit, t.data(), t.size() * sizeof(double), hipMemcpyHostToDevice));
  return FMX_OK;
}

static int64_t effective_tile_rows(const fmx_engine* e) {
  const int64_t want = e->cfg.tile_rows > 0 ? e->cfg.tile_rows : (e->kp32 >= 16 ? 524288 : 262144);
  if (e->cfg.batch_rows <= want) return e->cfg.batch_rows;
  const int64_t tiles = (e->cfg.batch_rows + want - 1) / want;
  const int64_t rows = (e->cfg.batch_rows + tiles - 1) / tiles;
  return (ranking(e) && rows % 2 != 0) ? rows + 1 : rows;
}

struct TileRun {
  int64_t tile;
  int64_t r0;
  int64_t nrows;
};

static int step_tiles(fmx_engine* e, fmx_matrix* m, int64_t batch, int64_t rows_limit, std::vector<TileRun>* out, int64_t* step_rows) {
  FMX_CHECK(!seq_mode(e), FMX_ERR_STATE, "step interface needs FMX_MODE_MINIBATCH");
  FMX_CHECK(m->has_labels || ranking(e), FMX_ERR_STATE, "there are no labels in data");
  FMX_TRY(check_pairs(e, m, rows_limit, "rows_limit"));
  const int64_t tile = effective_tile_rows(e);
  FMX_TRY(build_batch_csc(m, e->cfg.batch_rows, tile, e->stream));
// ... 237 lines not shown
  if (tiles.empty()) tiles.push_back({m->step_first_tile[(size_t)batch], 0, 0});
  const auto& pl = m->plans[(size_t)tiles[0].tile];
  FMX_CHECK(pl.feat != nullptr, FMX_ERR_STATE, "the compact exchange needs sparse tiles (fewer entries than features per tile); use fmx_grad for dense ones");
  FMX_TRY(ensure_compact(e, (int64_t)pl.n_lists > 0 ? (int64_t)pl.n_lists : 1));
  int64_t np = 0;
  FMX_TRY(rows_phase(e, m, tiles[0], step_rows, 0, &np));
  ColsArgs c{};
  FMX_TRY(cols_args(e, m, tiles[0], true, &c));
  c.store_compact = 1;
  c.compact_tail = 1;
  c.scalar = SCALAR_PUBLISH;
  c.n_partials = np;
  c.global_rows = (double)step_rows;
  if (e->owner_parts > 1) {
    FMX_TRY(ensure_owner_plan(e, m, tiles[0].tile));
    c.rec_pos = m->plans[(size_t)tiles[0].tile].own_pos;
  }
  LongArgs la{};
  FMX_TRY(long_args(e, m, tiles[0].tile, &la, &c));
  e->crec_count = pl.dcounts;
  e->crec_n = (int64_t)pl.n_lists;
  return launch_cols_update(e, c, la);
}

int group_grad_empty(fmx_engine* e, fmx_matrix* m, int64_t batch) { return run_step(e, m, batch, 0, false, true); }
int group_grad_compact(fmx_engine* e, fmx_matrix* m, int64_t batch, int64_t rows) { return grad_compact(e, m, batch, rows, rows <= 0); }

}

using namespace fmx;

extern "C" {

const char* fmx_last_error(void) { return g_error.c_str(); }

int fmx_device_count(int32_t* count) {
  FMX_CHECK(count != nullptr, FMX_ERR_INVALID, "count is NULL");
  int c = 0;
  const hipError_t err = hipGetDeviceCount(&c);
  *count = (err == hipSuccess) ? c : 0;
  if (err != hipSuccess || c <= 0) { set_error("no HIP device available (%s); libfmx has no CPU fallback", err == hipSuccess ? "device count 0" : hipGetErrorString(err)); return FMX_ERR_NOGPU; }
  return FMX_OK;
}

int fmx_config_default(fmx_config* cfg) {
  FMX_CHECK(cfg != nullptr, FMX_ERR_INVALID, "cfg is NULL");
  memset(cfg, 0, sizeof(*cfg));
  cfg->struct_size = sizeof(fmx_config);
  cfg->task = FMX_TASK_CLASSIFICATION;
  cfg->solver = FMX_SOLVER_SGD;
  cfg->num_factor = 2;
  cfg->keep_w0 = 1; cfg->keep_w1 = 1;
  cfg->learn_rate = 0.01;
  cfg->alpha_w = 0.1; cfg->alpha_v = 0.1; cfg->beta_w = 1.0; cfg->beta_v = 1.0;
  cfg->random_step = 1;
  cfg->mode = FMX_MODE_SEQUENTIAL;
  cfg->batch_rows = 65536;
  cfg->min_target = -1.0; cfg->max_target = 1.0;
  cfg->device = 0;
  cfg->batch_reduce = FMX_REDUCE_MEAN;
  cfg->gamma = 1e-4;
  cfg->n_gpus = 1;
  return FMX_OK;
}

int fmx_engine_create(const fmx_config* cfg, uint64_t num_features, fmx_engine** out) {
  FMX_CHECK(out != nullptr, FMX_ERR_INVALID, "out is NULL");
  *out = nullptr;
  FMX_CHECK(cfg != nullptr, FMX_ERR_INVALID, "cfg is NULL");
  FMX_CHECK(cfg->struct_size == sizeof(fmx_config), FMX_ERR_INVALID, "fmx_config size mismatch (%u vs %zu): header/library skew",
            cfg->struct_size, sizeof(fmx_config));
  FMX_CHECK(cfg->task == FMX_TASK_CLASSIFICATION || cfg->task == FMX_TASK_REGRESSION || cfg->task == FMX_TASK_RANKING, FMX_ERR_INVALID, "unknown task...");
  if (cfg->task == FMX_TASK_RANKING) {
    FMX_CHECK(cfg->mode == FMX_MODE_MINIBATCH && (cfg->solver == FMX_SOLVER_SGD || cfg->solver == FMX_SOLVER_FTRL), FMX_ERR_INVALID,
              "FMX_TASK_RANKING runs in FMX_MODE_MINIBATCH with FMX_SOLVER_SGD or FMX_SOLVER_FTRL only (got mode %d, solver %d)", cfg->mode, cfg->solver);
    FMX_CHECK(cfg->batch_rows % 2 == 0 && cfg->tile_rows % 2 == 0, FMX_ERR_INVALID,
              "FMX_TASK_RANKING needs an even batch_rows and an even (or 0) tile_rows: a step or tile may not split a pair (got %lld, %lld)",
              (long long)cfg->batch_rows, (long long)cfg->tile_rows);
  }
  FMX_CHECK(cfg->solver == FMX_SOLVER_SGD || cfg->solver == FMX_SOLVER_FTRL || cfg->solver == FMX_SOLVER_ALS || cfg->solver == FMX_SOLVER_TDAP ||
                cfg->solver == FMX_SOLVER_MCMC,
            FMX_ERR_INVALID, "Unknown solver...");
  FMX_CHECK(cfg->num_factor >= 0 && cfg->num_factor <= 128, FMX_ERR_INVALID, "factor.number must be in 0..128 (got %d)", cfg->num_factor);
  FMX_CHECK(cfg->mode == FMX_MODE_SEQUENTIAL || cfg->mode == FMX_MODE_MINIBATCH, FMX_ERR_INVALID, "unknown mode %d", cfg->mode);
  FMX_CHECK(cfg->random_step >= 1, FMX_ERR_INVALID, "random_step must be >= 1");
  FMX_CHECK(cfg->n_gpus >= 0, FMX_ERR_INVALID, "n_gpus must be >= 0");
  FMX_CHECK(cfg->als_max_levels >= -2, FMX_ERR_INVALID, "als_max_levels must be >= 0, or -1 / -2 (the coloured orders)");
  FMX_CHECK(cfg->batch_reduce == FMX_REDUCE_MEAN || cfg->batch_reduce == FMX_REDUCE_SUM, FMX_ERR_INVALID, "unknown batch_reduce %d", cfg->batch_reduce);
  FMX_CHECK(num_features > 0 && num_features < (1ull << 32), FMX_ERR_INVALID, "number of features must be in 1..2^32-1");
  if (cfg->mode == FMX_MODE_MINIBATCH) FMX_CHECK(cfg->batch_rows >= 1 && cfg->tile_rows >= 0, FMX_ERR_INVALID, "batch_rows must be >= 1 and tile_rows >= 0");
  FMX_TRY(use_device(cfg->device));

  std::unique_ptr<fmx_engine, int (*)(fmx_engine*)> e(new fmx_engine(), fmx_engine_destroy);
  e->cfg = *cfg;
  e->p = num_features;
  e->k = cfg->num_factor;
  e->kp32 = pad_factor(e->k, 4);
  e->kp64 = pad_factor(e->k, 2);
  FMX_TRY(make_hyper(*cfg, &e->hyper));
  FMX_HIP(hipStreamCreateWithFlags(&e->stream, hipStreamNonBlocking));
  FMX_TRY(dev_alloc_zero(&e->scal_base, (size_t)2 * SC_COUNT));
  e->scal = e->scal_base;
  e->scal_next = e->scal_base + SC_COUNT;
  const size_t p = (size_t)e->p;
  if (cfg->mode == FMX_MODE_MINIBATCH && !cfg->state_fp64) {
    {
      const char* v = getenv("FMX_W_IN_ROW");
      const bool want = v ? v[0] == '1' : num_features >= 3000000ull;
      e->w_in_row = (want && e->kp32 <= WIR_MAX_KP && e->k > 0) ? 1 : 0;
      e->vstride32 = e->w_in_row ? 2 * e->kp32 : e->kp32;
    }
    FMX_TRY(dev_alloc_zero(&e->V, p * e->vstride32));
    if (!e->w_in_row) FMX_TRY(dev_alloc_zero(&e->w, p));
    if (e->hyper.kind != UPD_SGD_L2) { FMX_TRY(dev_alloc_zero(&e->sV, p * e->kp32)); FMX_TRY(dev_alloc_zero(&e->sw, p)); }
    if (e->hyper.kind == UPD_FTRL || e->hyper.kind == UPD_TDAP) { FMX_TRY(dev_alloc_zero(&e->nV, p * e->kp32)); FMX_TRY(dev_alloc_zero(&e->nw, p)); }
    if (e->hyper.kind == UPD_TDAP) {
      FMX_TRY(dev_alloc_zero(&e->t1V, p * e->kp32)); FMX_TRY(dev_alloc_zero(&e->t1w, p));
      FMX_TRY(dev_alloc_zero(&e->t2V, p * e->kp32)); FMX_TRY(dev_alloc_zero(&e->t2w, p));
      FMX_TRY(dev_alloc_zero(&e->t3V, p * e->kp32)); FMX_TRY(dev_alloc_zero(&e->t3w, p));
    }
  } else {
    FMX_TRY(dev_alloc_zero(&e->dV, p * e->kp64));
    FMX_TRY(dev_alloc_zero(&e->dw, p));
    if (e->hyper.kind != UPD_SGD_L2) { FMX_TRY(dev_alloc_zero(&e->dsV, p * e->kp64)); FMX_TRY(dev_alloc_zero(&e->dsw, p)); }
    if (e->hyper.kind == UPD_FTRL || e->hyper.kind == UPD_TDAP) { FMX_TRY(dev_alloc_zero(&e->dnV, p * e->kp64)); FMX_TRY(dev_alloc_zero(&e->dnw, p)); }
    if (e->hyper.kind == UPD_TDAP) {
      FMX_TRY(dev_alloc_zero(&e->dt1V, p * e->kp64)); FMX_TRY(dev_alloc_zero(&e->dt1w, p));
      FMX_TRY(dev_alloc_zero(&e->dt2V, p * e->kp64)); FMX_TRY(dev_alloc_zero(&e->dt2w, p));
      FMX_TRY(dev_alloc_zero(&e->dt3V, p * e->kp64)); FMX_TRY(dev_alloc_zero(&e->dt3w, p));
    }
  }
  FMX_HIP(hipDeviceSynchronize());
  if (cfg->n_gpus > 1) FMX_TRY(group_create(e.get()));
  *out = e.release();
  return FMX_OK;
}

int fmx_engine_destroy(fmx_engine* e) {
  if (!e) return FMX_OK;
  group_destroy(e);
  (void)hipSetDevice(e->cfg.device);
  if (e->stream) (void)hipStreamSynchronize(e->stream);
  for (auto& pr : e->prof_pending) { (void)hipEventDestroy(pr.second.first); (void)hipEventDestroy(pr.second.second); }
  if (e->rows_tune.events) for (auto& ev : e->rows_tune.ev) (void)hipEventDestroy(ev);
  (void)hipFree(e->scal_base);
  (void)hipFree(e->V); (void)hipFree(e->w); (void)hipFree(e->sV); (void)hipFree(e->sw); (void)hipFree(e->nV); (void)hipFree(e->nw);
  (void)hipFree(e->t1V); (void)hipFree(e->t1w); (void)hipFree(e->t2V); (void)hipFree(e->t2w); (void)hipFree(e->t3V); (void)hipFree(e->t3w);
  (void)hipFree(e->dV); (void)hipFree(e->dw); (void)hipFree(e->dsV); (void)hipFree(e->dsw); (void)hipFree(e->dnV); (void)hipFree(e->dnw);
  (void)hipFree(e->dt1V); (void)hipFree(e->dt1w); (void)hipFree(e->dt2V); (void)hipFree(e->dt2w); (void)hipFree(e->dt3V); (void)hipFree(e->dt3w);
  (void)hipFree(e->seq_b); (void)hipFree(e->seq_len); (void)hipFree(e->seq_y);
  (void)hipFree(e->seq_packed); (void)hipFree(e->seq_conf); (void)hipFree(e->seq_keys); (void)hipFree(e->seq_sort_tmp);
  (void)hipFree(e->long_partial); (void)hipFree(e->probit);
  (void)hipFree(e->S); (void)hipFree(e->amul); (void)hipFree(e->partials); (void)hipFree(e->gbuf);
  (void)hipFree(e->crec); (void)hipFree(e->ctail); merge_ws_free(e->merge); (void)hipFree(e->als_qe_new); (void)hipFree(e->als_Q); (void)hipFree(e->als_qe); (void)hipFree(e->als_dyn); (void)hipFree(e->als_backup); (void)hipFree(e->als_tile_ws); (void)hipFree(e->als_lo[0]); (void)hipFree(e->als_lo[1]); (void)hipFree(e->als_hash_word); (void)hipFree(e->als_lam_mu); (void)hipFree(e->als_persist_ctl); (void)hipFree(e->als_rec);
  als_graph_free(e->als_graph_w); als_graph_free(e->als_graph_v);
  if (e->side_fork) (void)hipEventDestroy(e->side_fork);
  if (e->side_join) (void)hipEventDestroy(e->side_join);
  if (e->side) (void)hipStreamDestroy(e->side);
  if (e->stream) (void)hipStreamDestroy(e->stream);
  delete e;
  return FMX_OK;
}

int fmx_set_params(fmx_engine* e, double w0, const double* w, const double* v) {
  FMX_CHECK(e != nullptr, FMX_ERR_INVALID, "NULL engine");
  FMX_TRY(use_device(e->cfg.device));
  FMX_HIP(hipStreamSynchronize(e->stream));
  FMX_HIP(hipMemcpy(e->scal + SC_W0, &w0, sizeof(double), hipMemcpyHostToDevice));
  e->als_q_invalidate();
  FMX_TRY(params_to_device(e, w, v));
  e->trace_iters.clear(); e->trace_evals.clear(); e->trace_params.clear();
  FMX_TRY(reset_optimizer_state(e));
  FMX_HIP(hipDeviceSynchronize());
  if (e->group) FMX_TRY(group_set_params(e, w0, w, v));
  return FMX_OK;
}

int fmx_get_params(fmx_engine* e, double* w0, double* w, double* v) {
  FMX_CHECK(e != nullptr, FMX_ERR_INVALID, "NULL engine");
  FMX_TRY(use_device(e->cfg.device));
  FMX_HIP(hipStreamSynchronize(e->stream));
  FMX_TRY(seq_abort_check(e));
  if (w0) FMX_HIP(hipMemcpy(w0, e->scal + SC_W0, sizeof(double), hipMemcpyDeviceToHost));
  FMX_TRY(params_from_device(e, w, v));
  return FMX_OK;
}

int fmx_init_normal(fmx_engine* e, uint64_t seed, double mean, double stdev) {
  FMX_CHECK(e != nullptr, FMX_ERR_INVALID, "NULL engine");
  FMX_TRY(use_device(e->cfg.device));
  FMX_TRY(fmx_set_params(e, 0.0, nullptr, nullptr));
  FMX_TRY(init_normal(e, seed, mean, stdev));
  FMX_HIP(hipStreamSynchronize(e->stream));
  if (e->group) FMX_TRY(group_init_normal(e, seed, mean, stdev));
  return FMX_OK;
}

static int rows_io(fmx_engine* e, const uint32_t* ids, int64_t n, double* w, double* v, bool set) {
  FMX_CHECK(e != nullptr && n >= 0 && (n == 0 || ids), FMX_ERR_INVALID, "bad argument");
  for (int64_t i = 0; i < n; ++i) FMX_CHECK((uint64_t)ids[i] < e->p, FMX_ERR_INVALID, "feature id %u out of range", ids[i]);
  FMX_TRY(use_device(e->cfg.device));
  if (n == 0) return FMX_OK;
  uint32_t* d_ids = nullptr; double *d_w = nullptr, *d_v = nullptr;
  const size_t kk = (size_t)(e->k > 0 ? e->k : 1);
  int st = FMX_OK;
  auto body = [&]() -> int {
    FMX_HIP(hipMalloc(&d_ids, (size_t)n * sizeof(uint32_t)));
    FMX_HIP(hipMalloc(&d_w, (size_t)n * sizeof(double)));
    FMX_HIP(hipMalloc(&d_v, (size_t)n * kk * sizeof(double)));
    FMX_HIP(hipMemcpy(d_ids, ids, (size_t)n * sizeof(uint32_t), hipMemcpyHostToDevice));
    if (set) {
      FMX_TRY(rows_copy(e, d_ids, n, d_w, d_v, false));
      FMX_HIP(hipStreamSynchronize(e->stream));
      if (w) FMX_HIP(hipMemcpy(d_w, w, (size_t)n * sizeof(double), hipMemcpyHostToDevice));
      if (v && e->k > 0) FMX_HIP(hipMemcpy(d_v, v, (size_t)n * kk * sizeof(double), hipMemcpyHostToDevice));
    }
    FMX_TRY(rows_copy(e, d_ids, n, d_w, d_v, set));
    FMX_HIP(hipStreamSynchronize(e->stream));
    if (!set) {
      if (w) FMX_HIP(hipMemcpy(w, d_w, (size_t)n * sizeof(double), hipMemcpyDeviceToHost));
      if (v && e->k > 0) FMX_HIP(hipMemcpy(v, d_v, (size_t)n * kk * sizeof(double), hipMemcpyDeviceToHost));
    }
    return FMX_OK;
  };
  st = body();
  (void)hipFree(d_ids); (void)hipFree(d_w); (void)hipFree(d_v);
  return st;
}

int fmx_get_rows(fmx_engine* e, const uint32_t* ids, int64_t n, double* w, double* v) { return rows_io(e, ids, n, w, v, false); }
int fmx_set_rows(fmx_engine* e, const uint32_t* ids, int64_t n, const double* w, const double* v) {
  if (e) e->als_q_invalidate();
  FMX_TRY(rows_io(e, ids, n, const_cast<double*>(w), const_cast<double*>(v), true));
  if (e->group) FMX_TRY(group_set_rows(e, ids, n, w, v));
  return FMX_OK;
}

namespace fmx {

struct CkptHeader {
  char magic[4];
  uint32_t version;
  uint64_t p;
  int32_t k, kp, mode, kind;
  uint32_t scalars;
  uint32_t reserved[7];
};
static_assert(sizeof(CkptHeader) == 64, "checkpoint header is 64 bytes");

static void ckpt_tables(fmx_engine* e, std::vector<std::pair<void*, size_t>>* out) {
  const size_t p = (size_t)e->p;
  auto add = [&](void* ptr, size_t bytes) { if (ptr) out->push_back({ptr, bytes}); };
  add(e->V, p * (e->vstride32 ? e->vstride32 : e->kp32) * sizeof(float)); add(e->w, p * sizeof(float));
  add(e->sV, p * e->kp32 * sizeof(float)); add(e->sw, p * sizeof(float));
  add(e->nV, p * e->kp32 * sizeof(float)); add(e->nw, p * sizeof(float));
  add(e->t1V, p * e->kp32 * sizeof(float)); add(e->t1w, p * sizeof(float));
  add(e->t2V, p * e->kp32 * sizeof(float)); add(e->t2w, p * sizeof(float));
  add(e->t3V, p * e->kp32 * sizeof(float)); add(e->t3w, p * sizeof(float));
  add(e->dV, p * e->kp64 * sizeof(double)); add(e->dw, p * sizeof(double));
  add(e->dsV, p * e->kp64 * sizeof(double)); add(e->dsw, p * sizeof(double));
  add(e->dnV, p * e->kp64 * sizeof(double)); add(e->dnw, p * sizeof(double));
  add(e->dt1V, p * e->kp64 * sizeof(double)); add(e->dt1w, p * sizeof(double));
  add(e->dt2V, p * e->kp64 * sizeof(double)); add(e->dt2w, p * sizeof(double));
  add(e->dt3V, p * e->kp64 * sizeof(double)); add(e->dt3w, p * sizeof(double));
}

extern "C++" void engine_tables(fmx_engine* e, std::vector<std::pair<void*, size_t>>* out, bool params_only) {
  std::vector<std::pair<void*, size_t>> all;
  ckpt_tables(e, &all);
  for (auto& t : all) {
    const bool param = t.first == (void*)e->V || t.first == (void*)e->w || t.first == (void*)e->dV || t.first == (void*)e->dw;
    if (!params_only || param) out->push_back({t.first, t.second / (size_t)(e->p ? e->p : 1)});
  }
}

static CkptHeader ckpt_header(const fmx_engine* e) {
  CkptHeader h{};
  memcpy(h.magic, "FMX1", 4);
  h.version = 1; h.p = e->p; h.k = e->k; h.kp = wide_state(e) ? e->kp64 : e->kp32; h.mode = e->cfg.mode; h.kind = e->hyper.kind;
  h.scalars = SC_COUNT;
  h.reserved[0] = mb_wide(e) ? 1u : 0u;
  h.reserved[1] = 0u;
  return h;
}

constexpr size_t CKPT_PIECE = 1u << 18;
static bool ckpt_save_params32(fmx_engine* e, FILE* f) {
  const size_t p = (size_t)e->p, kp = (size_t)e->kp32, ds = (size_t)e->vstride32;
  std::vector<float> dev(CKPT_PIECE * ds), rows(CKPT_PIECE * kp), w(p);
  for (size_t j0 = 0; j0 < p; j0 += CKPT_PIECE) {
    const size_t c = p - j0 < CKPT_PIECE ? p - j0 : CKPT_PIECE;
    if (hipMemcpy(dev.data(), e->V + j0 * ds, c * ds * sizeof(float), hipMemcpyDeviceToHost) != hipSuccess) return false;
    for (size_t j = 0; j < c; ++j) {
      memcpy(&rows[j * kp], &dev[j * ds], kp * sizeof(float));
      w[j0 + j] = dev[j * ds + kp];
    }
    if (fwrite(rows.data(), sizeof(float), c * kp, f) != c * kp) return false;
  }
  return fwrite(w.data(), sizeof(float), p, f) == p;
}
static bool ckpt_load_params32(fmx_engine* e, FILE* f, bool file_wir) {
  const size_t p = (size_t)e->p, kp = (size_t)e->kp32, ds = (size_t)e->vstride32, fs = file_wir ? 2 * kp : kp;
  std::vector<float> dev(CKPT_PIECE * ds), rows(CKPT_PIECE * fs), w(p, 0.f);
  if (!file_wir && e->w_in_row) {
    const long at = ftell(f);
    if (at < 0 || fseek(f, (long)(p * kp * sizeof(float)), SEEK_CUR) != 0 || fread(w.data(), sizeof(float), p, f) != p || fseek(f, at, SEEK_SET) != 0) return false;
// ... 1027 lines not shown
  const size_t bytes = (size_t)m->n * sizeof(double);
  const size_t zbytes = (size_t)e->k * (size_t)e->p * sizeof(double);
  FMX_HIP(hipMalloc(&d_err, bytes));
  if (std_normals && hipMalloc(&d_z, zbytes) != hipSuccess) {
    (void)hipFree(d_err);
    set_error("out of device memory");
    return FMX_ERR_HIP;
  }
  int st = FMX_OK;
  if (hipMemcpy(d_err, error, bytes, hipMemcpyHostToDevice) != hipSuccess) { set_error("upload of the residual failed"); st = FMX_ERR_HIP; }
  if (st == FMX_OK && std_normals && hipMemcpy(d_z, std_normals, zbytes, hipMemcpyHostToDevice) != hipSuccess) { set_error("upload of the normal draws failed"); st = FMX_ERR_HIP; }
  if (st == FMX_OK) st = launch_als_vsweep_device(e, m, d_err, alpha, v_lambda, v_mu, d_z);
  if (st == FMX_OK && hipMemcpy(error, d_err, bytes, hipMemcpyDeviceToHost) != hipSuccess) { set_error("download of the residual failed"); st = FMX_ERR_HIP; }
  (void)hipFree(d_err); (void)hipFree(d_z);
  return st;
}

int fmx_als_vsweep(fmx_engine* e, fmx_matrix* m, double* error, double alpha, const double* v_lambda, const double* v_mu) {
  return vsweep_impl(e, m, error, alpha, v_lambda, v_mu, nullptr);
}

int fmx_mcmc_vsweep(fmx_engine* e, fmx_matrix* m, double* error, double alpha, const double* v_lambda, const double* v_mu,
                    const double* std_normals) {
  FMX_CHECK(std_normals != nullptr, FMX_ERR_INVALID, "std_normals is NULL (use fmx_als_vsweep for the ALS form)");
  return vsweep_impl(e, m, error, alpha, v_lambda, v_mu, std_normals);
}

int fmx_vsweep_device(fmx_engine* e, fmx_matrix* m, void* dev_error_f64, double alpha, const double* v_lambda, const double* v_mu, const void* dev_std_normals_f64) {
  FMX_TRY(check_pair(e, m));
  FMX_CHECK(seq_mode(e), FMX_ERR_STATE, "the ALS sweep runs on the fp64 tables: create the engine with FMX_MODE_SEQUENTIAL");
  FMX_CHECK(dev_error_f64 != nullptr || m->n == 0, FMX_ERR_INVALID, "dev_error_f64 is NULL");
  FMX_TRY(use_device(e->cfg.device));
  if (m->n == 0 || e->k == 0) return FMX_OK;
  return launch_als_vsweep_device(e, m, (double*)dev_error_f64, alpha, v_lambda, v_mu, (const double*)dev_std_normals_f64);
}

int fmx_als_plan_info(fmx_engine* e, fmx_matrix* m, int64_t* levels, int64_t* largest_level, int32_t* approximate, int32_t* level_of_feature) {
  FMX_TRY(check_pair(e, m));
  FMX_CHECK(seq_mode(e), FMX_ERR_STATE, "the ALS sweeps run on the fp64 tables: create the engine with FMX_MODE_SEQUENTIAL");
  FMX_TRY(use_device(e->cfg.device));
  return als_plan_info(e, m, levels, largest_level, approximate, level_of_feature);
}

int fmx_als_tiled_info(fmx_engine* e, fmx_matrix* m, int32_t* levels_tiled, int64_t* tile_rows, int32_t* n_tiles) {
  FMX_TRY(check_pair(e, m));
  FMX_CHECK(seq_mode(e), FMX_ERR_STATE, "the ALS sweeps run on the fp64 tables: create the engine with FMX_MODE_SEQUENTIAL");
  FMX_TRY(use_device(e->cfg.device));
  FMX_TRY(als_plan_info(e, m, nullptr, nullptr, nullptr, nullptr));
  return als_tiled_info(m, levels_tiled, tile_rows, n_tiles);
}

int fmx_als_order_info(fmx_engine* e, fmx_matrix* m, int32_t* level_order) {
  FMX_TRY(check_pair(e, m));
  FMX_CHECK(seq_mode(e), FMX_ERR_STATE, "the ALS sweeps run on the fp64 tables: create the engine with FMX_MODE_SEQUENTIAL");
  FMX_CHECK(level_order != nullptr, FMX_ERR_INVALID, "NULL argument");
  FMX_TRY(use_device(e->cfg.device));
  FMX_TRY(als_plan_info(e, m, nullptr, nullptr, nullptr, nullptr));
  *level_order = als_order_form(m);
  return FMX_OK;
}

int fmx_als_carry_q(fmx_engine* e, int32_t on) {
  FMX_CHECK(e != nullptr, FMX_ERR_INVALID, "NULL engine");
  e->als_carry_q = on ? 1 : 0;
  e->als_q_have = 0;
  return FMX_OK;
}

int fmx_als_train(fmx_engine* e, fmx_matrix* m, int32_t max_iter, int32_t with_v) {
  FMX_TRY(check_pair(e, m));
  FMX_CHECK(seq_mode(e), FMX_ERR_STATE, "ALS runs on the fp64 tables: create the engine with FMX_MODE_SEQUENTIAL");
  FMX_CHECK(max_iter >= 0, FMX_ERR_INVALID, "max_iter must be >= 0");
  FMX_CHECK(m->has_labels, FMX_ERR_STATE, "there are no labels in data");
  FMX_TRY(use_device(e->cfg.device));
  if (m->n == 0 || max_iter == 0) return FMX_OK;
  return launch_als_train(e, m, max_iter, with_v);
}

int fmx_mcmc_train(fmx_engine* e, fmx_matrix* m, int32_t max_iter, const double* std_gammas, const double* std_normals, double* state_out) {
  FMX_TRY(check_pair(e, m));
  FMX_CHECK(seq_mode(e), FMX_ERR_STATE, "MCMC runs on the fp64 tables: create the engine with FMX_MODE_SEQUENTIAL");
  FMX_CHECK(max_iter >= 0, FMX_ERR_INVALID, "max_iter must be >= 0");
  FMX_CHECK(m->has_labels, FMX_ERR_STATE, "there are no labels in data");
  FMX_CHECK(max_iter == 0 || (std_gammas != nullptr && std_normals != nullptr), FMX_ERR_INVALID, "the pre-drawn variates are NULL");
  FMX_TRY(use_device(e->cfg.device));
  if (m->n == 0 || max_iter == 0) return FMX_OK;
  return launch_mcmc_train(e, m, max_iter, std_gammas, std_normals, state_out);
}

int fmx_mcmc_train_from(fmx_engine* e, fmx_matrix* m, int32_t max_iter, const double* std_gammas, const double* std_normals, double* state_io) {
  FMX_TRY(check_pair(e, m));
  FMX_CHECK(seq_mode(e), FMX_ERR_STATE, "MCMC runs on the fp64 tables: create the engine with FMX_MODE_SEQUENTIAL");
  FMX_CHECK(state_io != nullptr, FMX_ERR_INVALID, "state_io is NULL (use fmx_mcmc_train to start a chain)");
  FMX_CHECK(max_iter >= 0, FMX_ERR_INVALID, "max_iter must be >= 0");
  FMX_CHECK(m->has_labels, FMX_ERR_STATE, "there are no labels in data");
  FMX_CHECK(max_iter == 0 || (std_gammas != nullptr && std_normals != nullptr), FMX_ERR_INVALID, "the pre-drawn variates are NULL");
  FMX_TRY(use_device(e->cfg.device));
  if (m->n == 0 || max_iter == 0) return FMX_OK;
  const double in[3] = {state_io[0], state_io[1], state_io[2]};
  return launch_mcmc_train(e, m, max_iter, std_gammas, std_normals, state_io, in);
}

int fmx_mcmc_v_hyper(fmx_engine* e, const double* std_gammas, const double* std_normals, double* v_lambda, double* v_mu, int32_t sample) {
  FMX_CHECK(e != nullptr && v_lambda != nullptr && v_mu != nullptr, FMX_ERR_INVALID, "NULL argument");
  FMX_CHECK(seq_mode(e), FMX_ERR_STATE, "MCMC / ALS run on the fp64 tables: create the engine with FMX_MODE_SEQUENTIAL");
  FMX_CHECK(!sample || (std_gammas != nullptr && std_normals != nullptr), FMX_ERR_INVALID, "the pre-drawn variates are NULL");
  FMX_TRY(use_device(e->cfg.device));
  return launch_mcmc_v_hyper(e, std_gammas, std_normals, v_lambda, v_mu, sample);
}

int fmx_rccl_selftest(int32_t n, double* max_err) { return group_rccl_selftest(n, max_err); }

int fmx_debug_fail_next_plan_build(void) { debug_fail_next_plan_build(); return FMX_OK; }
int fmx_debug_fail_next_comm_init(void) { debug_fail_next_comm_init(); return FMX_OK; }
int fmx_debug_lose_next_seq_multiplier(void) { debug_lose_next_seq_multiplier(); return FMX_OK; }
int fmx_debug_stall_next_persistent_sweep(void) { debug_stall_next_persistent_sweep(); return FMX_OK; }
int fmx_debug_contrib_summary_chunk(int64_t entries) { debug_contrib_summary_chunk(entries); return FMX_OK; }
int fmx_debug_foldin_slab(int64_t rows, int64_t groups) { debug_foldin_slab(rows, groups); return FMX_OK; }
int fmx_debug_heldout_limits(int32_t window, int64_t chunk) { debug_heldout_limits(window, chunk); return FMX_OK; }
int fmx_debug_pairs_hard_chunk(int64_t contexts) { debug_pairs_hard_chunk(contexts); return FMX_OK; }
int fmx_debug_lists_limits(int32_t lds_entries, int64_t chunk) { debug_lists_limits(lds_entries, chunk); return FMX_OK; }
int fmx_debug_diversify_limits(int32_t lds_rows, int64_t chunk) { debug_diversify_limits(lds_rows, chunk); return FMX_OK; }
int fmx_debug_neighbors_limits(int64_t slice_items, int64_t chunk_rows) { debug_neighbors_limits(slice_items, chunk_rows); return FMX_OK; }
int fmx_debug_interactions_limits(int32_t wave_entries, int32_t tile_entries, int64_t summary_rows_per_group) {
  debug_interactions_limits(wave_entries, tile_entries, summary_rows_per_group);
  return FMX_OK;
}
int fmx_debug_metrics_limits(int32_t wave_rows, int32_t lds_rows, int64_t chunk_rows) { debug_metrics_limits(wave_rows, lds_rows, chunk_rows); return FMX_OK; }
int fmx_debug_calibrate_limits(int64_t chunk_rows) { debug_calibrate_limits(chunk_rows); return FMX_OK; }
int fmx_debug_take_limits(int32_t fixed_entries, int32_t group_entries, int64_t rows_per_launch) {
  debug_take_limits(fixed_entries, group_entries, rows_per_launch);
  return FMX_OK;
}
int fmx_debug_long_launches(int64_t* out) {
  FMX_CHECK(out != nullptr, FMX_ERR_INVALID, "out is NULL");
  debug_long_launches(out);
  return FMX_OK;
}
int fmx_debug_rows_launches(int64_t* out) {
  FMX_CHECK(out != nullptr, FMX_ERR_INVALID, "out is NULL");
  debug_rows_launches(out);
  return FMX_OK;
}
int fmx_debug_rows_merged_launches(int64_t* out) {
  FMX_CHECK(out != nullptr, FMX_ERR_INVALID, "out is NULL");
  debug_rows_merged_launches(out);
  return FMX_OK;
}
int fmx_debug_rows_sched_launches(int64_t* out) {
  FMX_CHECK(out != nullptr, FMX_ERR_INVALID, "out is NULL");
  debug_rows_sched_launches(out);
  return FMX_OK;
}
int fmx_debug_rows_sched_id_limit(uint32_t limit) { debug_rows_sched_id_limit(limit); return FMX_OK; }
int fmx_debug_rows_sched_export(const fmx_matrix* m, int64_t tile, int64_t block, uint32_t* out, int64_t cap_words, int64_t* steps, int64_t* info) {
  FMX_CHECK(m != nullptr, FMX_ERR_INVALID, "NULL matrix");
  if (info) { info[0] = (int64_t)m->rows_sched.bytes; info[1] = (int64_t)(m->rows_sched.build_ms * 1e3); info[2] = m->rows_sched.policy; info[3] = m->rows_sched.rho_q; }
  return debug_rows_sched_export(m, tile, block, out, cap_words, steps);
}
int fmx_group_info(fmx_engine* e, int32_t* n_replicas, int32_t* share_device, int32_t* peer_pairs, int32_t* peer_pairs_direct, int32_t* sparse_exchange) {
  FMX_CHECK(e != nullptr, FMX_ERR_INVALID, "NULL engine");
  return group_info(e, n_replicas, share_device, peer_pairs, peer_pairs_direct, sparse_exchange);
}

int fmx_profile_enable(fmx_engine* e, int on) {
  FMX_CHECK(e != nullptr, FMX_ERR_INVALID, "NULL engine");
  FMX_TRY(prof_collect(e));
  e->profile = on > 0 ? on : 0;
  for (int i = 0; i < FMX_KERNEL_COUNT; ++i) e->prof_seen[i] = 0;
  return FMX_OK;
}

int fmx_profile_get(fmx_engine* e, int kernel, double* total_ms, int64_t* launches) {
  FMX_CHECK(e != nullptr && kernel >= 0 && kernel < FMX_KERNEL_COUNT, FMX_ERR_INVALID, "bad kernel id");
  FMX_TRY(prof_collect(e));
  if (total_ms) *total_ms = e->prof_ms[kernel];
  if (launches) *launches = e->prof_n[kernel];
  return FMX_OK;
}

int fmx_rows_tune_info(fmx_engine* e, int32_t* serial, double* ms_serial, double* ms_pipelined) {
  FMX_CHECK(e != nullptr, FMX_ERR_INVALID, "NULL engine");
  if (serial) *serial = e->rows_tune.decided;
  if (ms_serial) *ms_serial = e->rows_tune.ms[1];
  if (ms_pipelined) *ms_pipelined = e->rows_tune.ms[0];
  return FMX_OK;
}

int fmx_matrix_rows_form(const fmx_matrix* m, int32_t* form) {
  FMX_CHECK(m != nullptr && form != nullptr, FMX_ERR_INVALID, "NULL matrix or output");
  *form = rows_ragged(m) ? 2 : (rows_flat(m) ? 1 : 0);
  return FMX_OK;
}

int fmx_layout_info(fmx_engine* e, int32_t* v_row_stride, int32_t* w_in_row) {
  FMX_CHECK(e != nullptr, FMX_ERR_INVALID, "NULL engine");
  if (v_row_stride) *v_row_stride = wide_state(e) ? e->kp64 : e->vstride32;
  if (w_in_row) *w_in_row = (!wide_state(e) && e->w_in_row) ? 1 : 0;
  return FMX_OK;
}

int fmx_profile_reset(fmx_engine* e) {
  FMX_CHECK(e != nullptr, FMX_ERR_INVALID, "NULL engine");
  FMX_TRY(prof_collect(e));
  for (int i = 0; i < FMX_KERNEL_COUNT; ++i) { e->prof_ms[i] = 0; e->prof_n[i] = 0; }
  return FMX_OK;
}

}
```

### fmwr_amd/csrc/fmx_internal.h

```cpp
#pragma once
#include <hip/hip_runtime.h>

#include <cstdarg>
#include <cstdint>
#include <cstdio>
#include <cstdlib>
#include <functional>
#include <string>
#include <utility>
#include <vector>

#include "../../include/fmx.h"

namespace fmx {

void set_error(const char* fmt, ...);

#define FMX_HIP(call)                                                                         \
  do {                                                                                        \
    hipError_t _e = (call);                                                                   \
    if (_e != hipSuccess) {                                                                   \
      fmx::set_error("%s failed: %s (%s:%d)", #call, hipGetErrorString(_e), __FILE__, __LINE__); \
      return FMX_ERR_HIP;                                                                     \
    }                                                                                         \
// ... 63 lines not shown

namespace fmx { struct MergeWs; struct Group; }

struct fmx_matrix {
  uint64_t uid = 0;
  int device = 0;
  int64_t n = 0;
  uint32_t p = 0;
  int64_t nnz = 0;
  int64_t* row_ptr = nullptr;
  uint32_t* col = nullptr;
  float* val = nullptr;
  float* y = nullptr;
  int has_labels = 0;
  int rows_sorted = 0;
  int fixed_row_len = 0;
  int unit_values = 0;
  int dense_prefix = 0;
  std::vector<uint32_t> field_base;
  int max_row_len = 0;
  int64_t batch_rows = 0;
  int64_t tile_rows = 0;
  int64_t n_batches = 0;
  std::vector<int64_t> step_first_tile;
  struct TilePlan {
    int64_t r0 = 0, nrows = 0;
    int64_t base = 0, cnt = 0;
    uint32_t* off = nullptr;
    uint32_t* feat = nullptr;
    uint32_t* soff = nullptr;
    uint32_t* row0 = nullptr;
    uint32_t* val0 = nullptr;
    uint32_t n_lists = 0;
    uint32_t cap_lists = 0;
    uint32_t* lfeat = nullptr;
    uint32_t* lpos = nullptr;
    uint32_t* lseg_ptr = nullptr;
    uint32_t* seg_list = nullptr;
    uint32_t* seg_begin = nullptr;
    uint32_t* seg_end = nullptr;
    uint32_t n_long = 0, n_seg = 0, cap_long = 0, cap_seg = 0;
    uint32_t* dcounts = nullptr;
    void* pool = nullptr;
    int off_in_pool = 0;
    int own_n = 0;
    uint32_t* own_pos = nullptr;
    uint32_t* own_ids = nullptr;
    uint32_t* own_counts = nullptr;
    int64_t own_counts_h[17] = {0};
    void* own_pool = nullptr;
    uint32_t own_cap = 0;
  };
  std::vector<TilePlan> plans;
  uint64_t value_generation = 0;
  uint64_t plan_generation = 0;
  int64_t max_long_seg = 0;
  int64_t max_tile_cnt = 0;
  uint32_t* brow = nullptr;
  float* bval = nullptr;
  struct RowsSched {
    uint32_t* words = nullptr;
    uint32_t* dir = nullptr;
    std::vector<int64_t> tile_words;
    std::vector<int64_t> tile_dir;
    int policy = -1, rho_q = 0;
    uint64_t generation = 0;
    int tried = 0;
    size_t bytes = 0;
    double build_ms = 0.0;
  } rows_sched;
  int refilled_in_place = 0;
  int64_t* col_ptr = nullptr;
  uint32_t* crow = nullptr;
  float* cval = nullptr;
  uint32_t* als_feats = nullptr;
  std::vector<int64_t> als_level_ptr;
  uint32_t* als_heavy = nullptr;
  std::vector<int64_t> als_heavy_ptr;
  uint32_t* als_vh = nullptr;
  uint32_t* als_vh_seg0 = nullptr;
  uint32_t* als_vseg_feat = nullptr;
  int64_t* als_vseg_b = nullptr;
  int64_t* als_vseg_e = nullptr;
  double* als_vh_work = nullptr;
  int64_t als_n_vh = 0, als_n_vseg = 0;
  std::vector<int64_t> als_vh_ptr, als_vseg_ptr;
  std::vector<int32_t> als_level_of;
  int als_approx = 0;
  int als_coloured = 0;
  std::vector<int64_t> als_level_maxlen;
  int als_force_exact = 0;
  int als_plan_cap = -1;
  int64_t* als_level_ptr_dev = nullptr;
  uint16_t* als_rank = nullptr;
  int als_rank_state = 0;
  void* als_tiled = nullptr;
  int als_tiled_tried = 0;
};

struct RowsTune {
  static constexpr int TRIALS = 14;
  static constexpr int64_t MIN_ROWS = 65536;
  int decided = -1;
  int launches = 0;
  int64_t key = -1;
  hipEvent_t ev[2 * TRIALS] = {};
  bool events = false;
  double ms[2] = {0, 0};
};

struct fmx_engine {
  fmx_config cfg{};
  fmx::Hyper hyper{};
  uint64_t p = 0;
  int k = 0;
  int kp32 = 0;
  int vstride32 = 0;
  int w_in_row = 0;
  int kp64 = 0;
  hipStream_t stream = nullptr;
  hipStream_t side = nullptr;
  hipEvent_t side_fork = nullptr, side_join = nullptr;
  double* scal = nullptr;
  double* scal_next = nullptr;
  double* scal_base = nullptr;
  float *V = nullptr, *w = nullptr;
  float *sV = nullptr, *sw = nullptr;
  float *nV = nullptr, *nw = nullptr;
  float *t1V = nullptr, *t1w = nullptr;
  float *t2V = nullptr, *t2w = nullptr;
  float *t3V = nullptr, *t3w = nullptr;
  double *dV = nullptr, *dw = nullptr;
  double *dsV = nullptr, *dsw = nullptr;
  double *dnV = nullptr, *dnw = nullptr;
  double *dt1V = nullptr, *dt1w = nullptr;
  double *dt2V = nullptr, *dt2w = nullptr;
  double *dt3V = nullptr, *dt3w = nullptr;
  int64_t* seq_b = nullptr;
  int* seq_len = nullptr;
  float* seq_y = nullptr;
  int64_t seq_cap = 0;
  void* seq_packed = nullptr;
  int32_t* seq_conf = nullptr;
  uint32_t* seq_keys = nullptr;
  void* seq_sort_tmp = nullptr;
  size_t seq_sort_tmp_bytes = 0;
  int64_t seq_wcap = 0;
  int64_t ws_rows = 0;
  int64_t tile_rows = 0;
  void* S = nullptr;
  void* amul = nullptr;
  double* partials = nullptr;
  int64_t ws_partials = 0;
  double* probit = nullptr;
  double* long_partial = nullptr;
  int64_t long_partial_cap = 0;
  void* crec = nullptr;
  int64_t crec_cap = 0;
  int rec_elems = 0;
  void* ctail = nullptr;
  uint32_t* crec_count = nullptr;
  int64_t crec_n = 0;
  int owner_parts = 0;
  int owner_rank = 0;
  fmx::MergeWs* merge = nullptr;
  void* als_qe_new = nullptr;
  int64_t als_qe_new_rows = 0;
  double* als_Q = nullptr;
  size_t als_Q_elems = 0;
  void* als_qe = nullptr;
  int64_t als_qe_rows = 0;
  void* als_dyn = nullptr;
  void* als_tile_ws = nullptr;
  size_t als_tile_ws_bytes = 0;
  void* als_lo[2] = {nullptr, nullptr};
  int64_t als_lo_rows = 0;
  int als_lo_cur = 0;
  int als_q_level0 = 0;
  int als_carry_q = 0;
  int als_q_have = 0, als_q_age = 0;
  uint64_t als_q_trusted = 0;
  uint64_t als_q_hash = 0, als_q_plan = 0;
  void* als_hash_word = nullptr;
  double* als_lam_mu = nullptr;
  void als_q_invalidate() { als_q_have = 0; als_q_trusted = 0; }
  uint32_t* als_rec = nullptr;
  int64_t als_rec_rows = 0;
  unsigned int* als_persist_ctl = nullptr;
  const double* als_qnext = nullptr;
  int als_vf_slot = -1, als_vf_buf = 0;
  void *als_graph_w = nullptr, *als_graph_v = nullptr;
  double* als_backup = nullptr;
  size_t als_backup_elems = 0;
  fmx::Group* group = nullptr;
  void* gbuf = nullptr;
  int64_t gbuf_floats = 0;
  int64_t gb_feats = 0, gb_blocks = 0, gb_block_elems = 0;
  struct OpenTile { int64_t tile, r0, nrows, s_row0; };
  std::vector<OpenTile> open_tiles;
  int64_t open_rows = 0;
  int64_t open_partials = 0;
  fmx_matrix* open_matrix = nullptr;
  uint64_t open_generation = 0;
  struct Snapshot { double w0; std::vector<double> w, v; };
  std::vector<int64_t> trace_iters;
  std::vector<double> trace_evals;
  std::vector<Snapshot> trace_params;
  int profile = 0;
  int64_t prof_seen[FMX_KERNEL_COUNT] = {0};
  int prof_open = 0;
  double prof_ms[FMX_KERNEL_COUNT] = {0};
  int64_t prof_n[FMX_KERNEL_COUNT] = {0};
  std::vector<std::pair<int, std::pair<hipEvent_t, hipEvent_t>>> prof_pending;
  RowsTune rows_tune;
};

namespace fmx {

inline bool mb_wide(const fmx_engine* e) { return e->cfg.mode == FMX_MODE_MINIBATCH && e->cfg.state_fp64 != 0; }
inline bool wide_state(const fmx_engine* e) { return e->cfg.mode == FMX_MODE_SEQUENTIAL || e->cfg.state_fp64 != 0; }
inline int mb_kp(const fmx_engine* e) { return mb_wide(e) ? e->kp64 : e->kp32; }
inline int mb_lpr(const fmx_engine* e) { return mb_wide(e) ? e->kp64 / 2 : e->kp32 / 4; }
inline size_t mb_elem(const fmx_engine* e) { return mb_wide(e) ? sizeof(double) : sizeof(float); }
inline int mb_vstride(const fmx_engine* e) { return mb_wide(e) ? e->kp64 : e->vstride32; }
inline void* mb_vbase(const fmx_engine* e) { return mb_wide(e) ? (void*)e->dV : (void*)e->V; }
inline void* mb_wbase(const fmx_engine* e) { return mb_wide(e) ? (void*)e->dw : (e->w_in_row ? (void*)(e->V + e->kp32) : (void*)e->w); }
inline int mb_wstride(const fmx_engine* e) { return (!mb_wide(e) && e->w_in_row) ? e->vstride32 : 1; }
inline bool exchange_has_q(const fmx_engine* e) { return (e->hyper.kind == UPD_FTRL || e->hyper.kind == UPD_TDAP) && !e->hyper.mean; }

struct RowsArgs {
  const int64_t* row_ptr;
  const uint32_t* col;
  const float* val;
  const float* y;
  int64_t r0;
  int64_t nrows;
  const void* V;
  const void* w;
  int vs, ws;
  int vsh, wsh;
  const double* scal;
  void* S;
  void* amul;
  double* partials;
  double* yhat;
  double* qout;
  int64_t qout_t;
  const double* pn_y;
  int link;
  int unit;
  int no_w;
  int embed;
  int wg_threads;
  int split;
  int serial;
  int flat;
  int64_t nmat;
  int sort_rows;
  uint64_t mat_uid;
  int max_row_len;
  int col_skew;
  const uint32_t* sched;
  const uint32_t* sched_dir;
  int sched_state;
  uint32_t sched_vbytes, sched_wbytes;
  int sched_uniform;
  int sched_deal;
  int fixed_schedule;
};
constexpr size_t FMX_SERIAL_TABLE_MAX = 1ull << 30;
inline int rows_wg_threads(int64_t step_rows, int lpr) { return step_rows * lpr < 512LL * WG_THREADS ? 64 : WG_THREADS; }
inline int rows_split(int64_t step_rows, int lpr) { return (lpr <= 16 && step_rows * lpr < 1024LL * 64) ? 4 : 1; }
inline int rows_ragged(const fmx_matrix* m) {
  const char* s = getenv("FMX_ROWS_PULL");
  return (s && s[0] == '1' && m->fixed_row_len == 0 && m->n > 0) ? 1 : 0;
}
inline int rows_flat(const fmx_matrix* m) {
  if (m->fixed_row_len != 0 || m->n <= 0 || m->nnz <= 0) return 0;
  if ((int64_t)m->max_row_len * WG_THREADS >= (1LL << 31)) return 0;
  const char* s = getenv("FMX_ROWS_FLAT");
  return (s && s[0] == '1') ? 1 : 0;
}
inline int64_t rows_flat_blocks(int64_t r0, int64_t nrows, int g) { return nrows > 0 ? (r0 + nrows - 1) / g - r0 / g + 1 : 0; }
inline int rows_col_skew(const fmx_matrix* m, const fmx_matrix::TilePlan& pl) {
  const uint64_t lists = pl.feat ? pl.n_lists : m->p;
  if (lists == 0 || pl.n_long == 0) return 1;
  return ((uint64_t)pl.cnt <= 32ull * lists && (uint64_t)pl.n_long * 1024ull >= lists) ? 2 : 1;
}
int launch_rows_forward(fmx_engine* e, const RowsArgs& a, bool train, bool fp64_tables);
enum RowsSchedPolicy : int { SCHED_MERGE = 0, SCHED_FRONT = 1, SCHED_ROUND = 2, SCHED_DEAL = 3 };
constexpr int SCHED_STAGE_STEPS = 144;
constexpr uint32_t SCHED_BUBBLE = 0xFFFFFFFFu;
constexpr uint32_t SCHED_MAX_P = (1u << 30) - 1;
bool rows_sched_wanted(fmx_engine* e, const RowsArgs& a, int* policy, int* rho_q);
void rows_sched_count_build();
void debug_rows_sched_launches(int64_t out[3]);
int rows_sched_build(fmx_matrix* m, int policy, int rho_q, hipStream_t stream);
void rows_sched_free(fmx_matrix* m);
void debug_rows_sched_id_limit(uint32_t limit);
int debug_rows_sched_export(const fmx_matrix* m, int64_t tile, int64_t block, uint32_t* out, int64_t cap_words, int64_t* steps);
int ensure_probit(fmx_engine* e);
int topk_run(fmx_engine* e, const fmx_matrix* C, int64_t r0, int64_t r1, const fmx_matrix* I, const fmx_matrix* X, int K, int link, int64_t* d_index,
             double* d_score);
int heldout_run(fmx_engine* e, const fmx_matrix* C, int64_t r0, int64_t r1, const fmx_matrix* I, const fmx_matrix* H, const fmx_matrix* X, int64_t* d_rank,
                double* d_score, const int32_t* ks, int n_ks, double* pc);
int heldout_means(fmx_engine* e, const double* pc, int64_t n, int cols, double* out, int64_t* counted);
void debug_heldout_limits(int window, int64_t chunk);
int lists_run(fmx_engine* e, const fmx_matrix* C, int64_t r0, int64_t r1, const fmx_matrix* I, const fmx_matrix* Lm, int link, int K, double* d_score,
              int64_t* d_pos, int64_t* d_index, double* d_tscore);
int project_run(fmx_engine* e, const fmx_matrix* m, int64_t r0, int64_t r1, bool with_w0, double* d_base, double* d_s);
void debug_lists_limits(int lds_entries, int64_t chunk);
int diversify_run(fmx_engine* e, const fmx_matrix* I, int64_t n, int P, const int64_t* index, const double* score, int K, double lambda, int relevance,
                  int64_t* oi, double* os, double* om, bool host);
void debug_diversify_limits(int lds_rows, int64_t chunk);
int neighbors_run(fmx_engine* e, const fmx_matrix* Q, int64_t r0, int64_t r1, const fmx_matrix* I, int K, int metric, bool skip_self, int64_t* d_index,
                  double* d_score);
void debug_neighbors_limits(int64_t slice_items, int64_t chunk_rows);
int contrib_run(fmx_engine* e, const fmx_matrix* m, int64_t r0, int64_t r1, double* d_out);
int pairs_build(const fmx_matrix* C, const fmx_matrix* I, const fmx_matrix* X, int n_neg, uint64_t seed, int64_t epoch, fmx_matrix** out,
                fmx_engine* e = nullptr, int n_cand = 1);
void debug_pairs_hard_chunk(int64_t contexts);
int contrib_summary_run(fmx_engine* e, const fmx_matrix* m, double* sum, double* abs_sum, int64_t* count);
int foldin_run(fmx_engine* e, const fmx_matrix* m, const uint32_t* ids, int64_t n_ids, double lw, double lv, int n_newton, bool pairs,
               std::vector<double>* theta, std::vector<int64_t>* rows, std::vector<int32_t>* status);
void debug_foldin_slab(int64_t rows, int64_t groups);
void debug_contrib_summary_chunk(int64_t entries);
struct InterLimits {
  int wave_entries = 0;
  int tile_entries = 0;
  int64_t summary_rows = 0;
};
InterLimits interactions_take_limits();
int interactions_run(fmx_engine* e, const fmx_matrix* m, int64_t r0, int64_t r1, int top_m, const InterLimits& lim, int64_t* d_a, int64_t* d_b, double* d_v);
int interactions_summary_run(fmx_engine* e, const fmx_matrix* m, const uint32_t* groups, int G, const InterLimits& lim, double* sum, double* abs_sum,
                             int64_t* count);
void debug_interactions_limits(int wave_entries, int tile_entries, int64_t summary_rows);
struct MetLimits {
  int wave_rows = 0;
  int lds_rows = 0;
  int64_t chunk_rows = 0;
};
MetLimits metrics_limits();
int metrics_run(fmx_engine* e, const fmx_matrix* m, int64_t r0, int64_t r1, const uint32_t* d_group, int64_t G, int link, const MetLimits& lim, double* d_value,
                int64_t* d_count);
void debug_metrics_limits(int wave_rows, int lds_rows, int64_t chunk_rows);
int predict_calibrated_run(fmx_engine* e, const fmx_matrix* m, int64_t r0, int64_t r1, const uint32_t* d_group, int64_t G, const fmx_calibrator* cal, int link,
                           double* d_out);
int reliability_run(fmx_engine* e, const fmx_matrix* m, int64_t r0, int64_t r1, const uint32_t* d_group, int64_t G, int B, int binning, const fmx_calibrator* cal,
                    int link, int64_t* d_count, double* d_sum_p, double* d_lo_z, double* d_hi_z, int64_t* d_nan_rows, double* d_value);
int platt_run(fmx_engine* e, const fmx_matrix* m, int64_t r0, int64_t r1, const uint32_t* d_group, int64_t G, double lambda, int n_newton, double* d_ab,
              int64_t* d_rows, int32_t* d_status);
int isotonic_run(fmx_engine* e, const fmx_matrix* m, int64_t r0, int64_t r1, const uint32_t* d_group, int64_t G, int B, int32_t* d_n_steps, double* d_thr,
                 double* d_val);
void debug_calibrate_limits(int64_t chunk_rows);
void debug_take_limits(int fixed_entries, int group_entries, int64_t rows_per_launch);
void debug_long_launches(int64_t out[2]);
void debug_rows_launches(int64_t out[6]);
void debug_rows_merged_launches(int64_t out[2]);

enum ScalarMode : int { SCALAR_NONE = 0, SCALAR_FUSED = 1, SCALAR_PUBLISH = 2, SCALAR_FROM_TAIL = 3 };

struct ColsArgs {
  const uint32_t* bptr;
  const uint32_t* brow;
  const float* bval;
  uint32_t rows_active;
  uint32_t long_min;
  const uint32_t* tfeat;
  const uint32_t* toff;
  uint32_t n_tfeat;
  const uint32_t* trow0;
  const uint32_t* tval0;
  int inline0;
  int walk;
  int load_gbuf;
  int store_gbuf;
  int apply;
  int scalar;
  int64_t n_partials;
  double global_rows;
  uint32_t f0, f1;
  int64_t s_row0;
  int store_compact;
  const uint32_t* rec_pos;
  int compact_tail;
  int unit;
  int direct;
  int64_t list_entries;
  int embed;
  int buf_gather;
};
struct LongArgs {
  const uint32_t* lfeat;
  const uint32_t* lpos;
  const uint32_t* lseg_ptr;
  const uint32_t* seg_feat;
  const uint32_t* seg_begin;
  const uint32_t* seg_end;
  double* partial;
  int64_t n_long, n_seg;
};
inline uint32_t list_long_min() {
  static const uint32_t v = [] { const char* s = getenv("FMX_LONG_MIN"); const long x = s ? atol(s) : 0; return x > 0 ? (uint32_t)x : 64u; }();
  return v;
}
constexpr int WIR_MAX_KP = 16;
constexpr uint32_t LIST_SEG = 1024;
int launch_cols_update(fmx_engine* e, const ColsArgs& a, const LongArgs& la);
constexpr int REC_PARTS_MAX = 64;
struct RecParts { int n; int64_t prefix[REC_PARTS_MAX + 1]; int64_t start[REC_PARTS_MAX]; };
int launch_record_keys(fmx_engine* e, const void* recs, const RecParts& parts, int64_t total, uint32_t* keys, uint32_t* pos);
int launch_apply_records(fmx_engine* e, const void* recs, const uint32_t* pos, const uint32_t* roff, const uint32_t* rfeat, const uint32_t* d_n,
                         int64_t max_lists, int64_t global_rows);
struct MergeWs;
int merge_records(fmx_engine* e, const void* recs, const int64_t* counts, const int64_t* starts, int n_parts, int64_t stride, int64_t* total_out);
void merge_ws_free(MergeWs* w);
void merge_result(const fmx_engine* e, const uint32_t** pos, const uint32_t** roff, const uint32_t** rfeat, const uint32_t** d_n);

int launch_seq_learn(fmx_engine* e, const fmx_matrix* m, const int64_t* d_order, int64_t count);
int launch_seq_learn_grid(fmx_engine* const* es, int n, const fmx_matrix* m, const int64_t* d_order, int64_t count);

struct PlanWorkspace {
  int64_t max_cnt = 0;
  uint32_t p = 0;
  int bits = 0;
  uint32_t* keys_out = nullptr;
  uint64_t *vals_in = nullptr, *vals_out = nullptr;
  void* sort_temp = nullptr;
  size_t sort_bytes = 0;
  uint8_t* flags = nullptr;
  uint32_t* nseg = nullptr;
  uint32_t* blk = nullptr;
  void* prim_temp = nullptr;
  size_t prim_bytes = 0;
  uint32_t *fq_counts = nullptr, *fq_totals = nullptr;
  int reserve(int64_t cnt, uint32_t p, hipStream_t stream);
  PlanWorkspace() = default;
  PlanWorkspace(const PlanWorkspace&) = delete;
  PlanWorkspace& operator=(const PlanWorkspace&) = delete;
  ~PlanWorkspace();
};
int plan_alloc(fmx_matrix::TilePlan& t, uint32_t p, int64_t cap_cnt, bool dense);
void plan_free(fmx_matrix::TilePlan& t);
int plan_build(fmx_matrix::TilePlan& t, PlanWorkspace& ws, uint32_t p, const int64_t* row_ptr, const uint32_t* col, const float* val,
               uint32_t* brow, float* bval, hipStream_t stream, int unit_values, int fixed_row_len, int dense_prefix = 0,
               const std::vector<uint32_t>* field_base = nullptr, bool presplit = false);
bool plan_fields_split_applies(const PlanWorkspace& ws, int unit_values, int fixed_row_len, int dense_prefix, const std::vector<uint32_t>* field_base);
void plan_set_counts(fmx_matrix::TilePlan& t, uint32_t p, const uint32_t* h);
int plan_ensure_dense(fmx_matrix* m, int64_t tile, hipStream_t stream);
struct OwnerWorkspace {
  uint32_t cap = 0;
  uint32_t *keys_in = nullptr, *keys_out = nullptr, *idx_in = nullptr, *idx_out = nullptr;
  void* temp = nullptr;
  size_t temp_bytes = 0;
  int reserve(uint32_t n, hipStream_t stream);
  OwnerWorkspace() = default;
  OwnerWorkspace(const OwnerWorkspace&) = delete;
  OwnerWorkspace& operator=(const OwnerWorkspace&) = delete;
  ~OwnerWorkspace();
};
int plan_owner_alloc(fmx_matrix::TilePlan& t, uint32_t cap_lists);
int plan_owner_build(fmx_matrix::TilePlan& t, OwnerWorkspace& ws, int n_owners, uint32_t n_sort, hipStream_t stream);
int rows_pack(fmx_engine* e, const uint32_t* d_ids, int64_t n, void* d_rows, bool unpack);
void drop_plans(fmx_matrix* m);
int build_batch_csc(fmx_matrix* m, int64_t batch_rows, int64_t tile_rows, hipStream_t stream);
void debug_fail_next_plan_build();
void debug_lose_next_seq_multiplier();
void debug_stall_next_persistent_sweep();
int build_full_csc(fmx_matrix* m, hipStream_t stream);
int generate_synthetic(fmx_matrix* m, int32_t nnz_per_row, uint64_t seed, int64_t row_offset);
int generate_synthetic_async(fmx_matrix* m, int64_t n, int32_t z, uint64_t seed, int64_t row_offset, hipStream_t stream);
void strata_bounds(uint32_t p, int32_t z, std::vector<uint32_t>* out);
int generate_ragged(int device, int64_t n, uint32_t p, double mean, int lo, int hi, uint64_t seed, int64_t row_offset, fmx_matrix** out);
int matrix_values_uniform(fmx_matrix* m, uint64_t seed, int64_t row_offset);
int generate_iid_async(fmx_matrix* m, int64_t n, int32_t z, uint64_t seed, int64_t row_offset, int kind, double s_exp, hipStream_t stream);
constexpr int FMX_MAX_FIELDS = 64;
struct FieldSpec {
  int n_dense, n_fields;
  double skew;
  uint32_t base[FMX_MAX_FIELDS], vocab[FMX_MAX_FIELDS];
};
int generate_fields_async(fmx_matrix* m, int64_t n, const FieldSpec& fs, uint64_t seed, int64_t row_offset, hipStream_t stream);
int generate_fields_split_async(fmx_matrix* m, int64_t n, const FieldSpec& fs, uint64_t seed, int64_t row_offset, hipStream_t stream, uint32_t* keys_sorted, uint32_t* brow,
                                float* bval, uint32_t* keys_in);
int check_rows_sorted(fmx_matrix* m);
int params_to_device(fmx_engine* e, const double* w, const double* v);
int params_from_device(fmx_engine* e, double* w, double* v);
int ingest_host_arrays(fmx_matrix* m, const void* values, bool values_f64, const void* cols, bool cols_signed, const int32_t* row_size, const int64_t* row_ptr,
                       const void* labels, bool labels_f64, uint64_t bad[2], int64_t* total);
int matrix_set_fields(fmx_matrix* m, int n_dense, int n_fields, const uint32_t* base);
int init_normal(fmx_engine* e, uint64_t seed, double mean, double stdev);
int rows_copy(fmx_engine* e, const uint32_t* d_ids, int64_t n, double* d_w, double* d_v, bool set);
int matrix_scales(fmx_matrix* m, const uint8_t* h_listed, double* h_mean, double* h_std);
int matrix_normalize(fmx_matrix* m, const double* h_mean, const double* h_std);

int launch_als_train(fmx_engine* e, fmx_matrix* m, int max_iter, int with_v);
int als_plan_info(fmx_engine* e, fmx_matrix* m, int64_t* levels, int64_t* largest, int32_t* approx, int32_t* level_of);
int launch_mcmc_train(fmx_engine* e, fmx_matrix* m, int max_iter, const double* h_gammas, const double* h_normals, double* h_state, const double* h_state_in = nullptr);
int launch_mcmc_v_hyper(fmx_engine* e, const double* h_gammas, const double* h_normals, double* v_lambda, double* v_mu, int sample);
int launch_als_vsweep(fmx_engine* e, fmx_matrix* m, double* d_error, double* d_q, double alpha, const double* h_lambda, const double* h_mu,
                      const double* d_znorm);
void als_graph_free(void* g);
struct SweepDyn {
  int f, pad;
  double alpha, lambda, mu;
  const double* znorm;
};
int als_tiled_build(fmx_matrix* m, hipStream_t stream);
void als_tiled_free(fmx_matrix* m);
int als_tiled_info(const fmx_matrix* m, int32_t* levels_tiled, int64_t* tile_rows, int32_t* n_tiles);
template <bool W>
int als_tiled_level(fmx_engine* e, fmx_matrix* m, int level, bool last, double2* d_qe, const SweepDyn* dyn, bool* done);
bool als_order_ready(const fmx_matrix* m);
int als_order_levels(const fmx_matrix* m);
int als_order_enter(fmx_engine* e, fmx_matrix* m, const double2* d_qe, const double* d_Q0, bool* ok);
int als_order_level(fmx_engine* e, fmx_matrix* m, int slot, const SweepDyn* dyn, const double* d_qnext, double* d_qprev_out = nullptr);
int als_order_prepare(fmx_engine* e, fmx_matrix* m, const uint32_t** colP, const float** valP, const uint32_t** row0);
int als_order_exit(fmx_engine* e, fmx_matrix* m, double2* d_qe, double* d_qlast_out = nullptr);
uint64_t als_order_plan_uid(const fmx_matrix* m);
int als_order_w_sweep(fmx_engine* e, fmx_matrix* m, double2* d_qe, const SweepDyn* dyn, bool* done);
struct AlsBlocksIn {
  int64_t n; int n_slots;
  const uint32_t *lvl0, *cnt;
  const uint32_t* h_feats;
  const uint32_t* d_feats;
  int unit;
};
int als_blocks_build(fmx_matrix* m, const AlsBlocksIn& in, void** out, hipStream_t stream);
void als_blocks_free(void* b);
int als_blocks_info(const void* b, int32_t* block_rows, int32_t* blocks_level0);
int als_blocks_enter(fmx_engine* e, const void* b, const double2* d_qe, const double* d_Q0, double2* dst);
int als_blocks_level(fmx_engine* e, const void* b, int s, const double2* src, double2* dst, const uint32_t* d_feats, const SweepDyn* dyn, const double* d_qin, double* d_qprev_out, bool w_sweep = false);
uint64_t als_blocks_uid(const void* b);
int als_vhash(fmx_engine* e, uint64_t* out);
void als_blocks_csr(const void* b, const uint32_t** colP, const float** valP, const uint32_t** row0);
int als_blocks_exit(fmx_engine* e, const void* b, const double2* src, double2* d_qe, double* d_qlast_out, bool e_only = false);
int als_order_form(const fmx_matrix* m);
int launch_als_vsweep_device(fmx_engine* e, fmx_matrix* m, double* d_error, double alpha, const double* h_lambda, const double* h_mu, const double* d_znorm);

int evaluate_device(fmx_engine* e, const double* d_yhat, const float* d_y, int64_t n, int metric, double* result);

int group_create(fmx_engine* e);
void group_destroy(fmx_engine* e);
int group_set_params(fmx_engine* e, double w0, const double* w, const double* v);
int group_init_normal(fmx_engine* e, uint64_t seed, double mean, double stdev);
int group_set_rows(fmx_engine* e, const uint32_t* ids, int64_t n, const double* w, const double* v);
bool group_outside(const fmx_engine* e);
int group_load(fmx_engine* e, const char* path);
using GroupStepHook = std::function<int(int64_t first, int64_t last, bool* stop)>;
int group_train(fmx_engine* e, fmx_matrix* m, int64_t max_iter, int64_t* examples_done, const GroupStepHook* after_step = nullptr);
int group_train_stream(fmx_engine* e, const fmx_fields_spec* spec, int32_t nnz_per_row, uint64_t seed, int64_t row_offset, int64_t total_rows,
                       int64_t* examples_done, double* ingest_wait_s);
void free_matrix(fmx_matrix* m);
void engine_tables(fmx_engine* e, std::vector<std::pair<void*, size_t>>* out, bool params_only);
int group_make_replicated(fmx_engine* e);
int group_grad_empty(fmx_engine* e, fmx_matrix* m, int64_t batch);
int group_grad_compact(fmx_engine* e, fmx_matrix* m, int64_t batch, int64_t rows);
int group_rccl_selftest(int n, double* max_err);
int group_info(const fmx_engine* e, int32_t* n, int32_t* shared, int32_t* peer_pairs, int32_t* peer_direct, int32_t* sparse_exchange);
void debug_fail_next_comm_init();
int use_device(int device);
int seq_abort_check(fmx_engine* e);
int check_pair(const fmx_engine* e, const fmx_matrix* m);
int alloc_matrix(int device, int64_t n, uint32_t p, int64_t nnz, bool labels, fmx_matrix** out);
int forward_rows(fmx_engine* e, const fmx_matrix* m, int64_t r0, int64_t r1, double* d_out, int link);

void prof_begin(fmx_engine* e, int kernel);
void prof_end(fmx_engine* e);

}
```

### fmwr_amd/csrc/fmx_test_hooks.h

```cpp
#ifndef FMX_TEST_HOOKS_H_
#define FMX_TEST_HOOKS_H_
#include <stdint.h>
#ifdef __cplusplus
extern "C" {
#endif
int fmx_debug_fail_next_plan_build(void);
int fmx_debug_fail_next_comm_init(void);
int fmx_debug_lose_next_seq_multiplier(void);
int fmx_debug_stall_next_persistent_sweep(void);
int fmx_debug_contrib_summary_chunk(int64_t entries);
int fmx_debug_foldin_slab(int64_t rows, int64_t groups);
int fmx_debug_heldout_limits(int32_t window, int64_t chunk);
int fmx_debug_pairs_hard_chunk(int64_t contexts);
int fmx_debug_lists_limits(int32_t lds_entries, int64_t chunk);
int fmx_debug_diversify_limits(int32_t lds_rows, int64_t chunk);
int fmx_debug_neighbors_limits(int64_t slice_items, int64_t chunk_rows);
int fmx_debug_interactions_limits(int32_t wave_entries, int32_t tile_entries, int64_t summary_rows_per_group);
int fmx_debug_metrics_limits(int32_t wave_rows, int32_t lds_rows, int64_t chunk_rows);
int fmx_debug_take_limits(int32_t fixed_entries, int32_t group_entries, int64_t rows_per_launch);
int fmx_debug_calibrate_limits(int64_t chunk_rows);
int fmx_debug_cols_launches(int64_t* out);
int fmx_debug_long_launches(int64_t* out);
int fmx_debug_rows_launches(int64_t* out );
int fmx_debug_rows_merged_launches(int64_t* out );
int fmx_debug_rows_sched_launches(int64_t* out );
int fmx_debug_rows_sched_id_limit(uint32_t limit);
int fmx_debug_rows_sched_export(const fmx_matrix* m, int64_t tile, int64_t block, uint32_t* out, int64_t cap_words, int64_t* steps, int64_t* info );
#ifdef __cplusplus
}
#endif
#endif
```

Before: 1.072 billion.

## Pace workgroups per XCD so they walk schedule steps in lockstep for cache reuse

Adds a pacing mechanism to the MERGE/DEAL scheduled rows kernel. Every few steps each workgroup bumps a per-XCD atomic counter and compares its progress to the group average. Workgroups that run ahead sleep with s_sleep, so waves on the same XCD touch the same V/w cache lines at about the same time and reuse them in L2. It is on by default when the grid fits in resident occupancy. The cost is atomic traffic, idle sleep cycles and extra kernel variants, plus optional trace instrumentation.

Measured after the change: 1.091 billion, median of 6. 1.02x the previous value.

```diff
diff --git a/fmwr_amd/_lib.py b/fmwr_amd/_lib.py
--- a/fmwr_amd/_lib.py
+++ b/fmwr_amd/_lib.py
@@ -57,7 +57,8 @@
 TEST_HOOKS = ["fmx_debug_fail_next_plan_build", "fmx_debug_fail_next_comm_init", "fmx_debug_lose_next_seq_multiplier", "fmx_debug_stall_next_persistent_sweep",
               "fmx_debug_contrib_summary_chunk", "fmx_debug_foldin_slab", "fmx_debug_heldout_limits", "fmx_debug_pairs_hard_chunk", "fmx_debug_lists_limits", "fmx_debug_diversify_limits", "fmx_debug_neighbors_limits", "fmx_debug_interactions_limits", "fmx_debug_metrics_limits", "fmx_debug_take_limits", "fmx_debug_calibrate_limits", "fmx_debug_cols_launches",
               "fmx_debug_long_launches", "fmx_debug_rows_launches", "fmx_debug_rows_merged_launches",
-              "fmx_debug_rows_sched_launches", "fmx_debug_rows_sched_id_limit", "fmx_debug_rows_sched_export"]
+              "fmx_debug_rows_sched_launches", "fmx_debug_rows_sched_id_limit", "fmx_debug_rows_sched_export",
+              "fmx_debug_rows_pace_launches", "fmx_debug_rows_pace_counters", "fmx_debug_rows_pace_counters_of", "fmx_debug_rows_pace_poison", "fmx_debug_rows_pace_trace"]
 
 
 class Config(C.Structure):
diff --git a/fmwr_amd/csrc/fm_batch_kernels.hip b/fmwr_amd/csrc/fm_batch_kernels.hip
--- a/fmwr_amd/csrc/fm_batch_kernels.hip
+++ b/fmwr_amd/csrc/fm_batch_kernels.hip
@@ -507,7 +507,37 @@
   }
 }
 
-template <bool UNIFORM, bool PIPE, bool DEAL = false>
+#ifndef FMX_ROWS_PACE_EVERY
+#define FMX_ROWS_PACE_EVERY 24
+#endif
+#ifndef FMX_ROWS_PACE_LEAD
+#define FMX_ROWS_PACE_LEAD 2
+#endif
+#ifndef FMX_ROWS_PACE_SLEEP
+#define FMX_ROWS_PACE_SLEEP 30
+#endif
+constexpr int PACE_MAX_CHECKINS = (SCHED_STAGE_STEPS - 1) / FMX_ROWS_PACE_EVERY;
+constexpr int64_t PACE_STEP_CYCLES = 2120;
+static_assert((int64_t)PACE_MAX_CHECKINS * 3 * FMX_ROWS_PACE_SLEEP * 64 * 10 <= SCHED_STAGE_STEPS * PACE_STEP_CYCLES, "check-ins x the longest sleep: at most a tenth of the longest block's walk");
+static_assert((int64_t)((120 - 1) / FMX_ROWS_PACE_EVERY) * 3 * FMX_ROWS_PACE_SLEEP * 64 * 10 <= 120 * PACE_STEP_CYCLES, "the same for the headline's 120-step blocks");
+
+__device__ __forceinline__ void pace_sleep(int units) {
+  switch (units) {
+    case 5: __builtin_amdgcn_s_sleep(5); break;
+    case 10: __builtin_amdgcn_s_sleep(10); break;
+    case 15: __builtin_amdgcn_s_sleep(15); break;
+    case 20: __builtin_amdgcn_s_sleep(20); break;
+    case 30: __builtin_amdgcn_s_sleep(30); break;
+    case 40: __builtin_amdgcn_s_sleep(40); break;
+    case 60: __builtin_amdgcn_s_sleep(60); break;
+    case 80: __builtin_amdgcn_s_sleep(80); break;
+    case 90: __builtin_amdgcn_s_sleep(90); break;
+    case 120: __builtin_amdgcn_s_sleep(120); break;
+    default: break;
+  }
+}
+
+template <bool UNIFORM, bool PIPE, bool DEAL = false, bool PACE = false, bool TRACE = false>
 __global__ __launch_bounds__(WG_THREADS, 4) void fm_rows_sched_k(RowsArgs a, Hyper h) {
   using T = float;
   constexpr int LPR = 4, VEC = 4, KP = LPR * VEC;
@@ -516,14 +546,17 @@
   static_assert(MERGE_STAGE == SCHED_STAGE_STEPS * NG && MERGE_SLOTS == 4, "the stage holds SCHED_STAGE_STEPS steps of one word per lane group");
   static_assert(UNIFORM || !PIPE, "only the unrolled walk has a round to request together");
   static_assert(!(UNIFORM && DEAL), "a DEAL schedule is walked as a MERGE one");
+  static_assert(!(UNIFORM && (PACE || TRACE)), "the pace and its trace belong to the MERGE and DEAL walks");
   __shared__ uint32_t stage[MERGE_STAGE];
   __shared__ double red[MERGE_RPW];
   __shared__ uint32_t places[DEAL ? NG : 1];
+  __shared__ uint32_t pace_box;
 
   const int tid = threadIdx.x;
   const int gid = tid / LPR;
   const int lig = tid % LPR;
   const int64_t R0 = (int64_t)blockIdx.x * MERGE_RPW;
+  if constexpr (PACE) { if (tid == 0) pace_box = 0u; }
   const uint32_t w_hi = a.sched_dir[blockIdx.x + 1];
   uint32_t w_lo = a.sched_dir[blockIdx.x];
   if constexpr (DEAL) {
@@ -599,7 +632,24 @@
       }
     }
   } else {
+    uint32_t* pace_ctr = nullptr;
+    int64_t pace_groups = 0;
+    int pace_at = 0, pace_k = 0, pace_slept = 0;
+    uint32_t pace_seen = 0;
+    if constexpr (PACE) {
+      const uint32_t lab = blockIdx.x & 7u;
+      pace_ctr = a.pace + (size_t)(a.pace_set * 8 + (int)lab) * PACE_LINE;
+      pace_groups = (int64_t)(a.pace_div + (lab < a.pace_rem ? 1u : 0u));
+      pace_at = a.pace_every;
+      if (blockIdx.x == 0 && tid < 8 && a.pace_zero)
+        __hip_atomic_store(a.pace + (size_t)((a.pace_set ^ 1) * 8 + tid) * PACE_LINE, 0u, __ATOMIC_RELAXED, __HIP_MEMORY_SCOPE_AGENT);
+    }
+    uint64_t* trace = nullptr;
+    if constexpr (TRACE) trace = a.pace_trace + ((size_t)blockIdx.x * (WG_THREADS / 64) + tid / 64) * PACE_TRACE_WORDS;
     for (int t = 0; t < steps; ++t) {
+      if constexpr (TRACE) {
+        if ((t & 15) == 0 && (tid & 63) == 0) trace[1 + (t >> 4)] = __builtin_amdgcn_s_memrealtime();
+      }
       const uint32_t wd = mine[t * NG];
       const bool live = wd != SCHED_BUBBLE;
       const uint32_t c = wd & SCHED_MAX_P;
@@ -619,6 +669,28 @@
 #pragma unroll
           for (int i = 0; i < VEC; ++i) { sm[s][i] += tmp[i]; qm[s][i] += tsq[i]; }
         }
+      }
+      if constexpr (PACE) {
+        if (t == pace_at) {
+          ++pace_k;
+          if (tid == 64 * (pace_k & 3)) pace_seen = __hip_atomic_fetch_add(pace_ctr, a.pace_inc, __ATOMIC_RELAXED, __HIP_MEMORY_SCOPE_AGENT);
+        } else if (t == pace_at + 1) {
+          if (tid == 64 * (pace_k & 3))
+            __hip_atomic_store(&pace_box, (uint32_t)pace_k << 24 | (pace_seen < 0xFFFFFFu ? pace_seen : 0xFFFFFFu), __ATOMIC_RELAXED, __HIP_MEMORY_SCOPE_WORKGROUP);
+          const uint32_t box = (uint32_t)__builtin_amdgcn_readfirstlane((int)__hip_atomic_load(&pace_box, __ATOMIC_RELAXED, __HIP_MEMORY_SCOPE_WORKGROUP));
+          const int64_t k = (int64_t)(box >> 24), seen = (int64_t)(box & 0xFFFFFFu);
+          const int64_t lead2 = 2 * (int64_t)a.pace_every * (k * pace_groups - seen) - (int64_t)(a.pace_every - 1) * pace_groups;
+          const int64_t thr2 = 2 * (int64_t)a.pace_lead * pace_groups;
+          const int level = k == 0 ? 0 : lead2 > 3 * thr2 ? 3 : lead2 > 2 * thr2 ? 2 : lead2 > thr2 ? 1 : 0;
+          if (level) { pace_sleep(level * a.pace_sleep); pace_slept += 1 + (level << 16); }
+          pace_at += a.pace_every;
+        }
+      }
+    }
+    if constexpr (TRACE) {
+      if ((tid & 63) == 0) {
+        trace[1 + ((steps + 15) >> 4)] = __builtin_amdgcn_s_memrealtime();
+        trace[0] = (uint64_t)(__builtin_amdgcn_s_getreg((31 << 11) | 20) & 15u) | (uint64_t)steps << 8 | (uint64_t)pace_slept << 32;
       }
     }
   }
@@ -1179,6 +1251,47 @@
 }
 static int rows_sched_u() { static const int v = [] { const char* s = getenv("FMX_ROWS_SCHED_U"); return (s && atoi(s) == 4) ? 4 : 1; }(); return v; }
 
+#ifndef FMX_ROWS_PACE_DEFAULT
+#define FMX_ROWS_PACE_DEFAULT 1
+#endif
+static std::atomic<int64_t> g_rows_pace[2];
+void debug_rows_pace_launches(int64_t out[2]) {
+  for (int i = 0; i < 2; ++i) out[i] = g_rows_pace[i].load();
+}
+static int rows_pace_mode() {
+  static const int v = [] { const char* s = getenv("FMX_ROWS_PACE"); const int m = s ? atoi(s) : FMX_ROWS_PACE_DEFAULT; return (m >= 0 && m <= 2) ? m : FMX_ROWS_PACE_DEFAULT; }();
+  return v;
+}
+static bool rows_pace_trace_on() { static const bool v = [] { const char* s = getenv("FMX_ROWS_PACE_TRACE"); return s && s[0] == '1'; }(); return v; }
+struct PaceTune { int every, lead, sleep; };
+static const PaceTune& rows_pace_tune() {
+  static const PaceTune v = [] {
+    PaceTune t{FMX_ROWS_PACE_EVERY, FMX_ROWS_PACE_LEAD, FMX_ROWS_PACE_SLEEP};
+    int ev = 0, ld = 0, sl = 0;
+    const char* s = getenv("FMX_ROWS_PACE_TUNE");
+    if (s && sscanf(s, "%d,%d,%d", &ev, &ld, &sl) == 3 && ev >= 2 && ev <= 64 && ld >= 0 && ld <= 64 && (sl == 5 || sl == 10 || sl == 20 || sl == 30 || sl == 40)) t = PaceTune{ev, ld, sl};
+    return t;
+  }();
+  return v;
+}
+int debug_rows_pace_counters(fmx_engine* e, uint32_t out[16]) {
+  for (int i = 0; i < 16; ++i) out[i] = 0;
+  if (!e->rows_pace) return FMX_OK;
+  std::vector<uint32_t> all(PACE_WORDS);
+  FMX_HIP(hipStreamSynchronize(e->stream));
+  FMX_HIP(hipMemcpy(all.data(), e->rows_pace, PACE_WORDS * sizeof(uint32_t), hipMemcpyDeviceToHost));
+  for (int i = 0; i < 16; ++i) out[i] = all[(size_t)i * PACE_LINE];
+  return FMX_OK;
+}
+int debug_rows_pace_trace(fmx_engine* e, uint64_t* out, int64_t cap_words, int64_t* waves) {
+  *waves = e->rows_pace_trace ? e->rows_pace_trace_waves : 0;
+  if (*waves == 0 || !out) return FMX_OK;
+  FMX_CHECK(cap_words >= *waves * PACE_TRACE_WORDS, FMX_ERR_INVALID, "rows_pace_trace: %lld words for %lld waves", (long long)cap_words, (long long)*waves);
+  FMX_HIP(hipStreamSynchronize(e->stream));
+  FMX_HIP(hipMemcpy(out, e->rows_pace_trace, (size_t)*waves * PACE_TRACE_WORDS * sizeof(uint64_t), hipMemcpyDeviceToHost));
+  return FMX_OK;
+}
+
 bool rows_sched_wanted(fmx_engine* e, const RowsArgs& a, int* policy, int* rho_q) {
   const int mode = rows_sched_mode();
   if (mode == 0 || mb_wide(e) || e->kp32 != 16 || !a.unit || a.qout || a.no_w || a.wg_threads == 64 || a.sort_rows || a.flat == 1) return false;
@@ -1202,11 +1315,67 @@
   a.sched_wbytes = (uint32_t)((((uint64_t)e->p - 1) * (uint64_t)a.ws + 1) * sizeof(float));
   const int64_t grid = (a.nrows + MERGE_RPW - 1) / MERGE_RPW;
   FMX_CHECK(grid < (1LL << 31), FMX_ERR_INVALID, "rows_forward: grid too large (%lld)", (long long)grid);
-  if (a.sched_deal) hipLaunchKernelGGL((fm_rows_sched_k<false, false, true>), dim3((unsigned)grid), dim3(WG_THREADS), 0, e->stream, a, e->hyper);
-  else if (!a.sched_uniform) hipLaunchKernelGGL((fm_rows_sched_k<false, false>), dim3((unsigned)grid), dim3(WG_THREADS), 0, e->stream, a, e->hyper);
-  else if (rows_sched_u() == 4) hipLaunchKernelGGL((fm_rows_sched_k<true, true>), dim3((unsigned)grid), dim3(WG_THREADS), 0, e->stream, a, e->hyper);
+  if (!a.sched_uniform) {
+    const int mode = rows_pace_mode();
+    const bool traced = rows_pace_trace_on();
+    using SchedKernel = void (*)(RowsArgs, Hyper);
+    static const SchedKernel instance[2][2][2] = {
+        {{fm_rows_sched_k<false, false, false, false, false>, fm_rows_sched_k<false, false, false, false, true>},
+         {fm_rows_sched_k<false, false, false, true, false>, fm_rows_sched_k<false, false, false, true, true>}},
+        {{fm_rows_sched_k<false, false, true, false, false>, fm_rows_sched_k<false, false, true, false, true>},
+         {fm_rows_sched_k<false, false, true, true, false>, fm_rows_sched_k<false, false, true, true, true>}}};
+    const int deal = a.sched_deal ? 1 : 0;
+    bool paced = false;
+    if (mode != 0 && e->rows_pace) {
+      constexpr int MAX_DEV = 64;
+      static std::atomic<int64_t> resident_dev[MAX_DEV][2][2];
+      std::atomic<int64_t>& resident = resident_dev[(e->cfg.device >= 0 && e->cfg.device < MAX_DEV) ? e->cfg.device : 0][deal][traced ? 1 : 0];
+      int64_t r = resident.load();
+      if (r == 0) {
+        hipDeviceProp_t pr{};
+        int per = 0;
+        if (hipGetDeviceProperties(&pr, e->cfg.device) == hipSuccess && pr.multiProcessorCount > 0 &&
+            hipOccupancyMaxActiveBlocksPerMultiprocessor(&per, instance[deal][1][traced ? 1 : 0], WG_THREADS, 0) == hipSuccess && per > 0)
+          r = (int64_t)per * pr.multiProcessorCount;
+        else r = -1;
+        resident.store(r);
+      }
+      paced = r > 0 && grid <= r;
+    }
+    if (paced) {
+      const PaceTune& pt = rows_pace_tune();
+      a.pace = e->rows_pace;
+      a.pace_set = (int)(e->rows_pace_launches & 1);
+      a.pace_zero = e->rows_pace_poisoned ? 0 : 1;
+      a.pace_inc = e->rows_pace_poisoned ? 0u : 1u;
+      a.pace_div = (uint32_t)(grid / 8); a.pace_rem = (uint32_t)(grid % 8);
+      a.pace_every = pt.every; a.pace_lead = pt.lead; a.pace_sleep = pt.sleep;
+      if (e->rows_pace_poisoned) FMX_HIP(hipMemsetD32Async((hipDeviceptr_t)e->rows_pace, (int)e->rows_pace_poison, PACE_WORDS, e->stream));
+    }
+    if (traced) {
+      const int64_t waves = grid * (WG_THREADS / 64);
+      if (waves > e->rows_pace_trace_cap) {
+        FMX_HIP(hipStreamSynchronize(e->stream));
+        (void)hipFree(e->rows_pace_trace); e->rows_pace_trace = nullptr; e->rows_pace_trace_cap = 0;
+        FMX_HIP(hipMalloc(&e->rows_pace_trace, (size_t)waves * PACE_TRACE_WORDS * sizeof(uint64_t)));
+        e->rows_pace_trace_cap = waves;
+      }
+      FMX_HIP(hipMemsetAsync(e->rows_pace_trace, 0, (size_t)waves * PACE_TRACE_WORDS * sizeof(uint64_t), e->stream));
+      e->rows_pace_trace_waves = waves;
+      a.pace_trace = e->rows_pace_trace;
+    }
+    hipLaunchKernelGGL(instance[deal][paced ? 1 : 0][traced ? 1 : 0], dim3((unsigned)grid), dim3(WG_THREADS), 0, e->stream, a, e->hyper);
+    FMX_HIP(hipGetLastError());
+    if (paced) ++e->rows_pace_launches;
+    g_rows_pace[paced ? 0 : 1]++;
+    g_rows_sched[0]++;
+    *ran = true;
+    return FMX_OK;
+  }
+  if (rows_sched_u() == 4) hipLaunchKernelGGL((fm_rows_sched_k<true, true>), dim3((unsigned)grid), dim3(WG_THREADS), 0, e->stream, a, e->hyper);
   else hipLaunchKernelGGL((fm_rows_sched_k<true, false>), dim3((unsigned)grid), dim3(WG_THREADS), 0, e->stream, a, e->hyper);
   FMX_HIP(hipGetLastError());
+  g_rows_pace[1]++;
   g_rows_sched[0]++;
   *ran = true;
   return FMX_OK;
diff --git a/fmwr_amd/csrc/fm_group.hip b/fmwr_amd/csrc/fm_group.hip
--- a/fmwr_amd/csrc/fm_group.hip
+++ b/fmwr_amd/csrc/fm_group.hip
@@ -96,6 +96,11 @@
 };
 
 bool group_outside(const fmx_engine* e) { return e->group != nullptr && !e->group->busy; }
+
+fmx_engine* group_replica(fmx_engine* e, int r) {
+  if (!e->group) return r == 0 ? e : nullptr;
+  return (r >= 0 && r < e->group->n) ? e->group->rep[(size_t)r] : nullptr;
+}
 
 static void free_shards(Group* g) {
   for (size_t r = 0; r < g->shard.size(); ++r)
diff --git a/fmwr_amd/csrc/fmx_api.hip b/fmwr_amd/csrc/fmx_api.hip
--- a/fmwr_amd/csrc/fmx_api.hip
+++ b/fmwr_amd/csrc/fmx_api.hip
@@ -152,6 +152,10 @@
 static int ensure_workspace(fmx_engine* e, int64_t s_rows, int64_t step_rows, int64_t tiles_per_step) {
   const int rpw = WG_THREADS / mb_lpr(e);
   const int64_t partials = (step_rows + rpw - 1) / rpw + (tiles_per_step > 0 ? tiles_per_step : 1) + 8 + 4096;
+  if (!e->rows_pace) {
+    FMX_HIP(hipMalloc(&e->rows_pace, PACE_WORDS * sizeof(uint32_t)));
+    FMX_HIP(hipMemsetAsync(e->rows_pace, 0, PACE_WORDS * sizeof(uint32_t), e->stream));
+  }
   if (s_rows <= e->ws_rows && partials <= e->ws_partials) return FMX_OK;
   FMX_HIP(hipStreamSynchronize(e->stream));
   (void)hipFree(e->S); (void)hipFree(e->amul); (void)hipFree(e->partials);
@@ -695,6 +699,7 @@
   (void)hipFree(e->seq_packed); (void)hipFree(e->seq_conf); (void)hipFree(e->seq_keys); (void)hipFree(e->seq_sort_tmp);
   (void)hipFree(e->long_partial); (void)hipFree(e->probit);
   (void)hipFree(e->S); (void)hipFree(e->amul); (void)hipFree(e->partials); (void)hipFree(e->gbuf);
+  (void)hipFree(e->rows_pace); (void)hipFree(e->rows_pace_trace);
   (void)hipFree(e->crec); (void)hipFree(e->ctail); merge_ws_free(e->merge); (void)hipFree(e->als_qe_new); (void)hipFree(e->als_Q); (void)hipFree(e->als_qe); (void)hipFree(e->als_dyn); (void)hipFree(e->als_backup); (void)hipFree(e->als_tile_ws); (void)hipFree(e->als_lo[0]); (void)hipFree(e->als_lo[1]); (void)hipFree(e->als_hash_word); (void)hipFree(e->als_lam_mu); (void)hipFree(e->als_persist_ctl); (void)hipFree(e->als_rec);
   als_graph_free(e->als_graph_w); als_graph_free(e->als_graph_v);
   if (e->side_fork) (void)hipEventDestroy(e->side_fork);
@@ -2028,6 +2033,30 @@
   debug_rows_sched_launches(out);
   return FMX_OK;
 }
+int fmx_debug_rows_pace_launches(int64_t* out) {
+  FMX_CHECK(out != nullptr, FMX_ERR_INVALID, "out is NULL");
+  debug_rows_pace_launches(out);
+  return FMX_OK;
+}
+int fmx_debug_rows_pace_counters_of(fmx_engine* e, int32_t replica, uint32_t* out) {
+  FMX_CHECK(e != nullptr && out != nullptr, FMX_ERR_INVALID, "NULL engine or out");
+  fmx_engine* r = group_replica(e, replica);
+  FMX_CHECK(r != nullptr, FMX_ERR_INVALID, "no replica %d", (int)replica);
+  FMX_HIP(hipSetDevice(r->cfg.device));
+  const int st = debug_rows_pace_counters(r, out);
+  (void)hipSetDevice(e->cfg.device);
+  return st;
+}
+int fmx_debug_rows_pace_counters(fmx_engine* e, uint32_t* out) { return fmx_debug_rows_pace_counters_of(e, 0, out); }
+int fmx_debug_rows_pace_poison(fmx_engine* e, uint32_t value) {
+  FMX_CHECK(e != nullptr, FMX_ERR_INVALID, "NULL engine");
+  for (int i = 0; group_replica(e, i) != nullptr; ++i) { fmx_engine* r = group_replica(e, i); r->rows_pace_poisoned = 1; r->rows_pace_poison = value; }
+  return FMX_OK;
+}
+int fmx_debug_rows_pace_trace(fmx_engine* e, uint64_t* out, int64_t cap_words, int64_t* waves) {
+  FMX_CHECK(e != nullptr && waves != nullptr, FMX_ERR_INVALID, "NULL engine or waves");
+  return debug_rows_pace_trace(e, out, cap_words, waves);
+}
 int fmx_debug_rows_sched_id_limit(uint32_t limit) { debug_rows_sched_id_limit(limit); return FMX_OK; }
 int fmx_debug_rows_sched_export(const fmx_matrix* m, int64_t tile, int64_t block, uint32_t* out, int64_t cap_words, int64_t* steps, int64_t* info) {
   FMX_CHECK(m != nullptr, FMX_ERR_INVALID, "NULL matrix");
diff --git a/fmwr_amd/csrc/fmx_internal.h b/fmwr_amd/csrc/fmx_internal.h
--- a/fmwr_amd/csrc/fmx_internal.h
+++ b/fmwr_amd/csrc/fmx_internal.h
@@ -239,6 +239,12 @@
   void* amul = nullptr;
   double* partials = nullptr;
   int64_t ws_partials = 0;
+  uint32_t* rows_pace = nullptr;
+  int64_t rows_pace_launches = 0;
+  int rows_pace_poisoned = 0;
+  uint32_t rows_pace_poison = 0;
+  uint64_t* rows_pace_trace = nullptr;
+  int64_t rows_pace_trace_cap = 0, rows_pace_trace_waves = 0;
   double* probit = nullptr;
   double* long_partial = nullptr;
   int64_t long_partial_cap = 0;
@@ -353,6 +359,13 @@
   uint32_t sched_vbytes, sched_wbytes;
   int sched_uniform;
   int sched_deal;
+  uint32_t* pace;
+  int pace_set;
+  int pace_zero;
+  uint32_t pace_inc;
+  uint32_t pace_div, pace_rem;
+  int pace_every, pace_lead, pace_sleep;
+  uint64_t* pace_trace;
   int fixed_schedule;
 };
 constexpr size_t FMX_SERIAL_TABLE_MAX = 1ull << 30;
@@ -382,6 +395,12 @@
 bool rows_sched_wanted(fmx_engine* e, const RowsArgs& a, int* policy, int* rho_q);
 void rows_sched_count_build();
 void debug_rows_sched_launches(int64_t out[3]);
+constexpr int PACE_LINE = 32;
+constexpr int PACE_WORDS = 2 * 8 * PACE_LINE;
+constexpr int PACE_TRACE_WORDS = 16;
+void debug_rows_pace_launches(int64_t out[2]);
+int debug_rows_pace_counters(fmx_engine* e, uint32_t out[16]);
+int debug_rows_pace_trace(fmx_engine* e, uint64_t* out, int64_t cap_words, int64_t* waves);
 int rows_sched_build(fmx_matrix* m, int policy, int rho_q, hipStream_t stream);
 void rows_sched_free(fmx_matrix* m);
 void debug_rows_sched_id_limit(uint32_t limit);
@@ -632,6 +651,7 @@
 int group_set_params(fmx_engine* e, double w0, const double* w, const double* v);
 int group_init_normal(fmx_engine* e, uint64_t seed, double mean, double stdev);
 int group_set_rows(fmx_engine* e, const uint32_t* ids, int64_t n, const double* w, const double* v);
+fmx_engine* group_replica(fmx_engine* e, int r);
 bool group_outside(const fmx_engine* e);
 int group_load(fmx_engine* e, const char* path);
 using GroupStepHook = std::function<int(int64_t first, int64_t last, bool* stop)>;
diff --git a/fmwr_amd/csrc/fmx_test_hooks.h b/fmwr_amd/csrc/fmx_test_hooks.h
--- a/fmwr_amd/csrc/fmx_test_hooks.h
+++ b/fmwr_amd/csrc/fmx_test_hooks.h
@@ -26,6 +26,11 @@
 int fmx_debug_rows_sched_launches(int64_t* out );
 int fmx_debug_rows_sched_id_limit(uint32_t limit);
 int fmx_debug_rows_sched_export(const fmx_matrix* m, int64_t tile, int64_t block, uint32_t* out, int64_t cap_words, int64_t* steps, int64_t* info );
+int fmx_debug_rows_pace_launches(int64_t* out );
+int fmx_debug_rows_pace_counters(fmx_engine* e, uint32_t* out );
+int fmx_debug_rows_pace_counters_of(fmx_engine* e, int32_t replica, uint32_t* out );
+int fmx_debug_rows_pace_poison(fmx_engine* e, uint32_t value);
+int fmx_debug_rows_pace_trace(fmx_engine* e, uint64_t* out, int64_t cap_words, int64_t* waves);
 #ifdef __cplusplus
 }
 #endif
diff --git a/profiles/rows_pace_sim.py b/profiles/rows_pace_sim.py
--- /dev/null
+++ b/profiles/rows_pace_sim.py
@@ -0,0 +1,96 @@
+import argparse
+import os
+import sys
+import time
+
+import numpy as np
+
+sys.path.insert(0, os.path.dirname(os.path.abspath(__file__)))
+import rows_deal_sim as S
+
+STEP_CYCLES = 1870.0
+N_STEPS = S.SLOTS * S.NNZ
+
+
+def arrival_times(rng, rate, start, inside, pace):
+    o = rng.normal(0.0, start, S.BLOCKS)
+    r = rng.normal(0.0, rate, S.BLOCKS)
+    t = np.arange(N_STEPS, dtype=np.float64)
+    held = np.zeros((S.BLOCKS, N_STEPS))
+    slept = 0
+    if pace is not None:
+        every, lead, sleep = pace
+        delay = np.zeros(S.BLOCKS)
+        for k in range(1, (N_STEPS - 1) // every + 1):
+            s = k * every
+            mine = o + s * (1.0 + r) + delay
+            at = (mine[:, None] - o[None, :] - delay[None, :]) / (1.0 + r[None, :])
+            seen = np.clip(np.floor(at / every), 0, (N_STEPS - 1) // every).sum(axis=1)
+            lead_steps = every * (k - seen / S.BLOCKS) - (every - 1) / 2.0
+            level = (lead_steps > lead).astype(int) + (lead_steps > 2 * lead) + (lead_steps > 3 * lead)
+            slept += int((level > 0).sum())
+            delay = delay + level * sleep * 64.0 / STEP_CYCLES
+            held[:, s + 1:] = delay[:, None]
+    wg = o[:, None] + t[None, :] * (1.0 + r[:, None]) + held
+    waves = np.repeat(wg, 4, axis=0) + rng.normal(0.0, inside, S.BLOCKS * 4)[:, None]
+    return waves, slept
+
+
+def lines_fetched(cols, when_wave):
+    when = np.repeat(when_wave, 16, axis=0).ravel()
+    order = np.argsort(when, kind="stable")
+    flat = cols.ravel()[order]
+    v_line, w_line = (flat >> 1).tolist(), ((flat >> 5) + S.W_BASE).tolist()
+    lru, miss_v, miss_w = {}, 0, 0
+    for v, w in zip(v_line, w_line):
+        for key in (v, w):
+            if key in lru:
+                del lru[key]
+            else:
+                if key >= S.W_BASE:
+                    miss_w += 1
+                else:
+                    miss_v += 1
+                if len(lru) >= S.LRU_LINES:
+                    del lru[next(iter(lru))]
+            lru[key] = None
+    return miss_v, miss_w
+
+
+def spread(when_wave):
+    return {s: float(when_wave[:, s].std()) for s in (0, 32, 64, 96, N_STEPS - 1)}
+
+
+def main():
+    ap = argparse.ArgumentParser()
+    ap.add_argument("--rate", type=float, nargs="*", default=[0.0, 0.04, 0.08])
+    ap.add_argument("--start", type=float, default=0.7)
+    ap.add_argument("--inside", type=float, default=0.7)
+    ap.add_argument("--every", type=int, default=8)
+    ap.add_argument("--lead", type=float, nargs="*", default=[1.0, 2.0, 4.0])
+    ap.add_argument("--sleep", type=int, nargs="*", default=[10, 20])
+    ap.add_argument("--seed", type=int, default=1)
+    a = ap.parse_args()
+    t0 = time.time()
+    cols = S.streams(np.random.default_rng(a.seed), "deal")
+    print(f"DEAL streams made in {time.time() - t0:.1f} s")
+    print("M lines per tile (8 XCDs); spread = sd over the XCD's waves of the time a step is reached, in steps")
+    for rate in a.rate:
+        w, _ = arrival_times(np.random.default_rng(a.seed + 1000), rate, a.start, a.inside, None)
+        v, wl = lines_fetched(cols, w)
+        sp = spread(w)
+        print(f"rate {rate:.2f}  no pace              V {S.XCDS * v / 1e6:5.2f}  w {S.XCDS * wl / 1e6:4.2f}  spread " + " ".join(f"{s}:{x:.1f}" for s, x in sp.items()), flush=True)
+        if rate == 0.0:
+            continue
+        for lead in a.lead:
+            for sleep in a.sleep:
+                w, slept = arrival_times(np.random.default_rng(a.seed + 1000), rate, a.start, a.inside, (a.every, lead, sleep))
+                v, wl = lines_fetched(cols, w)
+                sp = spread(w)
+                print(f"rate {rate:.2f}  every {a.every} lead {lead:.0f} sleep {sleep:2d}  V {S.XCDS * v / 1e6:5.2f}  w {S.XCDS * wl / 1e6:4.2f}  spread " +
+                      " ".join(f"{s}:{x:.1f}" for s, x in sp.items()) + f"  sleeps {slept}  end {w.max() - w.min():.1f} steps", flush=True)
+    print(f"{time.time() - t0:.1f} s")
+
+
+if __name__ == "__main__":
+    main()
diff --git a/profiles/rows_pace_trace.py b/profiles/rows_pace_trace.py
--- /dev/null
+++ b/profiles/rows_pace_trace.py
@@ -0,0 +1,116 @@
+import argparse
+import ctypes
+import json
+import os
+import sys
+
+import numpy as np
+
+ROOT = os.path.dirname(os.path.dirname(os.path.abspath(__file__)))
+sys.path.insert(0, ROOT)
+WORDS = 16
+
+
+def reduce_launch(tr):
+    waves = tr.shape[0]
+    xcc = (tr[:, 0] & 15).astype(np.int64)
+    steps = ((tr[:, 0] >> 8) & 0xFFFF).astype(np.int64)
+    slept = ((tr[:, 0] >> 32) & 0xFFFF).astype(np.int64)
+    label = (np.arange(waves) // 4) % 8
+    labels_ok = all(len(np.unique(xcc[label == lb])) == 1 for lb in range(8)) and len(np.unique(xcc)) == 8
+    n = int(steps.min())
+    assert n == int(steps.max()) and n >= 32, "the headline's blocks hold the same number of steps"
+    at = list(range(0, n, 16))
+    stamps = tr[:, 1:1 + len(at) + 1].astype(np.int64)
+    t0 = stamps[:, 0].min()
+    tm = (stamps - t0).astype(np.float64) * 0.01
+    pos = np.array(at + [n], np.float64)
+    step_us = float(np.mean((tm[:, -1] - tm[:, 0]) / n))
+    out = {"waves": waves, "steps": n, "labels_are_xcds": bool(labels_ok), "launch_us": float(tm[:, -1].max()), "first_step_spread_us": float(tm[:, 0].max()),
+           "step_us": step_us, "sleeps": int(slept.sum()), "waves_that_slept": int((slept > 0).sum())}
+    drift = np.zeros((8, len(pos)))
+    for x in range(8):
+        sel = tm[label == x]
+        drift[x] = sel.std(axis=0) / step_us
+    out["drift_steps_by_step"] = {str(int(s)): float(v) for s, v in zip(pos, drift.mean(axis=0))}
+    out["drift_steps_by_step_per_xcd_end"] = [float(v) for v in drift[:, -1]]
+    b, a = np.polyfit(pos, (drift ** 2).mean(axis=0), 1)
+    out["variance_fit"] = {"at_step_0": float(a), "per_step": float(b), "fixed_share_at_end": float(a / max(a + b * n, 1e-12))}
+    frac = [0.1, 0.25, 0.5, 0.75, 0.9]
+    lo, hi = float(np.median(tm[:, 0])), float(np.median(tm[:, -1]))
+    reached = {}
+    for f in frac:
+        t = lo + f * (hi - lo)
+        sd = []
+        for x in range(8):
+            sel = tm[label == x]
+            sd.append(float(np.std([np.interp(t, w, pos) for w in sel])))
+        reached[str(f)] = float(np.mean(sd))
+    out["sd_of_step_reached_at_time"] = reached
+    for name, j in (("middle", len(pos) // 2), ("end", len(pos) - 1)):
+        inside, between = [], []
+        for x in range(8):
+            sel = tm[label == x][:, j].reshape(-1, 4)
+            inside.append(float(np.mean(sel.var(axis=1))))
+            between.append(float(sel.mean(axis=1).var()))
+        out[f"sd_inside_workgroup_steps_{name}"] = float(np.sqrt(np.mean(inside)) / step_us)
+        out[f"sd_between_workgroups_steps_{name}"] = float(np.sqrt(np.mean(between)) / step_us)
+    return out
+
+
+def main():
+    ap = argparse.ArgumentParser()
+    ap.add_argument("--pace", default="0")
+    ap.add_argument("--tune", default=None)
+    ap.add_argument("--launches", type=int, default=5)
+    ap.add_argument("--rows", type=int, default=262144)
+    ap.add_argument("--json", default=None)
+    ap.add_argument("--raw", default=None, help="save the last launch's stamps as .npy")
+    a = ap.parse_args()
+    os.environ["FMX_ROWS_PACE_TRACE"] = "1"
+    os.environ["FMX_ROWS_PACE"] = a.pace
+    if a.tune:
+        os.environ["FMX_ROWS_PACE_TUNE"] = a.tune
+    from fmwr_amd import _lib as L
+    from fmwr_amd import engine
+    lib = L.lib()
+    p, z, k, B = 1_000_000, 30, 16, a.rows
+    m = engine.Matrix.synthetic_iid(2 * B, p, z, 20240001, law=L.COLUMNS_UNIFORM)
+    e = engine.Engine(p, task=L.TASK_CLASSIFICATION, solver=L.SOLVER_SGD, num_factor=k, learn_rate=0.01, l2_w1=1e-4, l2_v=1e-4, mode=L.MODE_MINIBATCH, batch_rows=B)
+    e.init_normal(1, 0.0, 0.01)
+    for i in range(40):
+        e.step(m, i % 2)
+    e.sync()
+    per = []
+    for i in range(a.launches):
+        e.step(m, i % 2)
+        e.sync()
+        waves = ctypes.c_int64(0)
+        L.check(lib.fmx_debug_rows_pace_trace(e.h, None, ctypes.c_int64(0), ctypes.byref(waves)))
+        if waves.value == 0:
+            raise SystemExit("no traced launch: the step did not take the MERGE or DEAL walk of the scheduled form")
+        buf = np.zeros(waves.value * WORDS, np.uint64)
+        L.check(lib.fmx_debug_rows_pace_trace(e.h, buf.ctypes.data_as(ctypes.c_void_p), ctypes.c_int64(len(buf)), ctypes.byref(waves)))
+        per.append(reduce_launch(buf.reshape(-1, WORDS)))
+        if a.raw and i == a.launches - 1:
+            np.save(a.raw, buf.reshape(-1, WORDS))
+    pl = (ctypes.c_int64 * 2)()
+    L.check(lib.fmx_debug_rows_pace_launches(pl))
+    keys = ["launch_us", "step_us", "first_step_spread_us", "sleeps", "waves_that_slept", "sd_inside_workgroup_steps_middle", "sd_between_workgroups_steps_middle",
+            "sd_inside_workgroup_steps_end", "sd_between_workgroups_steps_end"]
+    med = {q: float(np.median([r[q] for r in per])) for q in keys}
+    med["drift_steps_by_step"] = {s: float(np.median([r["drift_steps_by_step"][s] for r in per])) for s in per[0]["drift_steps_by_step"]}
+    med["sd_of_step_reached_at_time"] = {s: float(np.median([r["sd_of_step_reached_at_time"][s] for r in per])) for s in per[0]["sd_of_step_reached_at_time"]}
+    med["variance_fit"] = {s: float(np.median([r["variance_fit"][s] for r in per])) for s in per[0]["variance_fit"]}
+    out = {"pace": a.pace, "tune": a.tune, "paced_launches": int(pl[0]), "unpaced_launches": int(pl[1]), "labels_are_xcds": all(r["labels_are_xcds"] for r in per),
+           "median": med, "launches": per}
+    print(json.dumps({q: out[q] for q in ("pace", "tune", "paced_launches", "unpaced_launches", "labels_are_xcds", "median")}, indent=1))
+    if a.json:
+        with open(a.json, "w") as f:
+            json.dump(out, f, indent=1)
+    e.close()
+    m.close()
+
+
+if __name__ == "__main__":
+    main()
```
